# BoyBaykiller/IDKEngine

Hardware: AMD Instinct MI355X
Metric: Mray/s (primary+1 bounce) at 1920x1080, 1M-tri scene (higher is better)
Workload: dtype f32

## Files before the change

idkengine_amd/csrc/host_context.hpp:

```cpp
#pragma once


struct DevBuf {
    void* p = nullptr; size_t bytes = 0;
    hipError_t ensure(size_t n) { if (n <= bytes && p) return hipSuccess; if (p) (void)hipFree(p); p = nullptr; bytes = 0; if (n == 0) return hipSuccess; hipError_t e = hipMalloc(&p, n); if (e == hipSuccess) bytes = n; return e; }
    void release() { if (p) (void)hipFree(p); p = nullptr; bytes = 0; }
    template <class T> T* as() const { return (T*)p; }
};

struct PinnedStage {
    char* host = nullptr; hipEvent_t ev[2] = {nullptr, nullptr}; int half = 0;
    template <class Fill> hipError_t stage(DevBuf& dst, size_t capacity, size_t bytes, hipStream_t st, Fill&& fill)
    {
        hipError_t e;
        if (!host) {
            if ((e = hipHostMalloc((void**)&host, 2 * capacity, hipHostMallocDefault)) != hipSuccess) return e;
            for (int i = 0; i < 2; i++) if ((e = hipEventCreateWithFlags(&ev[i], hipEventDisableTiming)) != hipSuccess) return e;
            half = 0;
        } else if ((e = hipEventSynchronize(ev[half])) != hipSuccess) return e;
        char* h = host + (size_t)half * capacity;
        fill(h);
        if ((e = dst.ensure(capacity)) != hipSuccess) return e;
        if ((e = hipMemcpyAsync(dst.p, h, bytes, hipMemcpyHostToDevice, st)) != hipSuccess) return e;
        if ((e = hipEventRecord(ev[half], st)) != hipSuccess) return e;
// ... 37 lines not shown
    void release() { mem.release(); bytes = 0; }
    template <class T> T* as() const { return (T*)mem.p; }
};

struct DisplaySlot {
    GuardedBuf image; int format = -1;
    void release() { image.release(); format = -1; }
};

struct BloomSlot {
    GuardedBuf down, up, out;
    int levels = 0, w0 = 0, h0 = 0; bool valid = false;
    bool direct = false;
    void release() { down.release(); up.release(); out.release(); valid = false; }
};

struct DenoiseSlot {
    GuardedBuf out, ping[2];
    bool valid = false;
    int iterations = 0; uint8_t route[8] = {0};
    void release() { out.release(); ping[0].release(); ping[1].release(); valid = false; iterations = 0; }
};

struct NoiseSlot {
    GuardedBuf tiles, summary;
    int tilesX = 0, tilesY = 0; bool valid = false;
    void release() { tiles.release(); summary.release(); valid = false; }
};

static bool slot_holds(const DisplaySlot& s) { return s.format >= 0; }
template <class S> static bool slot_holds(const S& s) { return s.valid; }

struct FrameProducts {
    std::vector<DisplaySlot> display; std::vector<BloomSlot> bloom; std::vector<DenoiseSlot> denoise; std::vector<NoiseSlot> noise;
    DevBuf moments;
    template <class S> static void drop(std::vector<S>& v) { for (S& s : v) s.release(); v.clear(); }
    void release_noise() { drop(noise); moments.release(); }
    void release_presentation_sized() { drop(display); drop(bloom); }
    void release_all() { release_presentation_sized(); drop(denoise); release_noise(); }
    template <class S> static S& slot(std::vector<S>& v, int ringSize, int slot) { if (v.size() != (size_t)ringSize) { drop(v); v.resize(ringSize); } return v[slot]; }
};

struct DevOptions {
    int forceGeneric = 0;
    int noTileCull = 0;
    int noLeanPrimary = 0;
    int leafMin = 0;
    int grabUnitLog2 = 10, grabFixed = 0;
    int ldsPad = 0;
    int traceWaves = 0;
    int gridHint = 2;
    int deferLast = 1;
    int lastOcclusion = 1;
    int graphProbe = 0;
    int gridMidWaves = 20;
    int gridRaysX4 = 6;
    int traceVariant = 0;
    int bvhTiming = 0, bvhSmall = 32;
    int advMin = 0;
    int poolMin = 12;
    int leafPool = -1;
    int splitScatter = 6;
    int queryScheduler = 1;
    int groupThreads = -1;
    int fused = 1;
    int fusedShadeMin = 16;
    int splitPeek = 64;
    int splitDonor = 1;
    int split = 1;
    int wide = 0;
    int wideCap = 0;
    int wideCount = 0;
    int genPixelMajor = 8;
    int bouncePixelMajor = 1;
    int genGroupMax = 16;
    int instSieve = 8;
    int instSieveOverlap = 50;
    int instTlas = 8;
    int instTlasOverlap = 10;
    int instBraid = 0;
    int instUnify = 4096;
    int instGeneral = 0;
    int uniRefill = 32;
    int instUnifyRadius = 15;
    int pairNodes = 1;
    int packet = 1;
    int packetMinLive = 60;
    int packetWaves = 0;
    int bvhStackOptHost = 0;
};

enum { VB_NODES = 0, VB_TRIVERTS, VB_VERTICES, VB_TLAS, VB_XFORMS, VB_COUNT };
struct PendingSample { uint32_t accum; int slot; float cam[36]; uint8_t vs[VB_COUNT]; };

struct dev_ctx {
    int device = 0;
    hipStream_t stream = nullptr; bool ownStream = true;
    std::string lastError;
    idkpt_error_fn errFn = nullptr; void* errUser = nullptr;
    int numCUs = 256;
    idkpt_settings st;
    idkpt_settings stCaller;
    int W = 0, H = 0, rowMod = 1, rowRem = 0, rows = 0, rowBandLog2 = 0;
    float invProj[16], invView[16], viewPos[3];
    int ringSize = 1, curSlot = 0; bool ringStarted = false; std::vector<uint32_t> accum = std::vector<uint32_t>(1, 0u);
    bool counters = false, timing = false, capturePrimary = false;
    DevOptions opt;
    uint32_t seqFirst = 0, seqStride = 1;
    bool haveScene = false, frameOk = false;
    DevBuf nodes, tris, triVerts, descs, instances, tlas, parents, leaves, positions, prevPositions, vertices, meshes, materials, xforms, lights, sky, texDescs, unskinned, joints, levelNodes, tlasScratch, queryIn, queryOut, queryRec, queryList, tileClass, gbases;
    std::vector<DevBuf> texData; std::vector<std::pair<int, int>> texDims; std::vector<uint32_t> texState;
    DevBuf texStage;
    DevBuf srgbLut;
    std::vector<GpuBlasDesc> hDescs;
    std::vector<std::vector<uint32_t>> levelOffsets;
    std::vector<uint32_t> levelBase;
    std::vector<char> refitCoversAll;
    int nodeCount = 0, triCount = 0, instanceCount = 0, tlasCount = 0, vertexCount = 0, meshCount = 0, materialCount = 0, xformCount = 0, lightCount = 0, skySize = 0, textureCount = 0, unskinnedCount = 0;
    int sceneStack = 1;
    int hInst0Blas = 0;
    DevBuf wnodes, wleaf, wids, wpair, wcounts, wtotals; std::vector<uint32_t> wNodeOff, wLeafOff; bool wideTopoValid = false, wideFillValid = false;
    DevBuf pairNodes; bool pairValid = false;
    DevBuf instRec; bool instRecValid = false;
    DevBuf itlas, imarks, ichunks; int itlasNeed = 1; uint32_t ichunkCount = 0; bool itlasValid = false, imarksValid = false;
    int uniMode = 0; uint32_t uniBaseB = 0, uniRestoreIdx = 0;
    DevBuf unodes, utlas, uTabs, uniBuf, uniEntRec; bool uniValid = false, uniEligible = false, uniTabsValid = false; int uniCap = 0, uniEntries = 0, uniDepth = 0; float* hUni = nullptr; float* dUni = nullptr;
    std::vector<GpuBlasInstance> hInstances; std::vector<char> hXforms; uint64_t uniLaunches = 0;
    DevBuf entRec, braidBuf; bool itlasBraided = false; int itlasDepth = 0, itlasEntries = 0;
    int pkState = 0, pkBatchesSinceProbe = 0; unsigned long long* hPkStats = nullptr; unsigned long long* dPkStats = nullptr; unsigned long long pkSeen[6] = {0, 0, 0, 0, 0, 0}; float pkCam[36] = {0}; int pkW = 0, pkRows = 0, pkBatch = 0; float pkLastLive = -1.0f;
    float* hInstOverlap = nullptr; float* dInstOverlap = nullptr; bool instOverlapKnown = false, itlasBuilt = false, isieveWorth = false;
    int verSlots = 1; size_t vbytes[VB_COUNT] = {0}, vstride[VB_COUNT] = {0}; int valloc[VB_COUNT] = {1, 1, 1, 1, 1}, vcur[VB_COUNT] = {0};
    uint64_t lastMask[VB_COUNT] = {0};
    uint8_t lastSlots[VB_COUNT] = {0}; bool lastMulti = false;
    DevBuf verTab; PinnedStage verStage;
    char* hStage = nullptr; hipEvent_t evStage[4] = {nullptr, nullptr, nullptr, nullptr}; int stageNext = 0;
    PinnedUpload skyStage;
    hipEvent_t evSky = nullptr;
    int (*groupFlushAll)(void* user) = nullptr;
    DevBuf pmList;
    DevBuf trRec, contFlag, blockSums, rayO, rayT, rayR, aovA, aovN, hit, hitCost, primHit, queue[2], keys[2], keysTmp, sortKeys, sortVals, contMask, waveCounts, counts, work, sortHist, counters64;
    DevBuf img[3];
    FrameProducts products;
    int presW = 0, presH = 0;
    int resultSource = 0;
    PinnedUpload denoiseStage;
    int noiseOn = 0;
    DevBuf camTab;
    int rowLimit = 0x7fffffff;
    idkpt_bounce_exchange_fn exchangeFn = nullptr; void* exchangeUser = nullptr;
    idkpt_band_exchange_fn bandExchangeFn = nullptr; void* bandExchangeUser = nullptr; DevBuf bandTab;
    idkpt_band_exchange_device_fn bandExchangeDevFn = nullptr; void* bandExchangeDevUser = nullptr;
    idkpt_stats stats;
    uint32_t* hCounts = nullptr; uint32_t* dCountsMirror = nullptr;
    bool sceneNested = false;
    bool sceneNoEmission = false;
    struct { bool valid = false, allHits = false; int j = 0, side = 0, B = 0; uint32_t total = 0, Npad = 0;
             bool occl = false, pm = false; size_t ldsBytes = 0; uint32_t grid = 0; } defer;
    uint64_t occlLaunches = 0;
    DevBuf radSave, deferCount;
    bool countersDirty = true;
    uint32_t* hOverflow = nullptr; uint32_t* dOverflow = nullptr;
    int tlasNeed = 1;
    hipEvent_t evFrame[2] = {nullptr, nullptr};
    std::vector<hipEvent_t> evPool; size_t evUsed = 0;
    double traceMsAcc = 0.0; uint64_t traceLaunchesAcc = 0;
    int lastQueueSide = 0; int lastQueueCountSlot = 0; bool lastFast = false, lastNeedsRegen = false, lastTileClass = false ; int lastBatch = 1; Frame lastFrame;
    int maxBatch = 1; uint32_t Npad = 0; std::vector<PendingSample> pending; DevBuf bases, qwork; uint32_t* hBases = nullptr; uint32_t* dBasesMirror = nullptr;
    PinnedStage camStage;
    bool grouped = false, inGroupFlush = false; int groupIndex = 0;
    hipEvent_t* evBounce = nullptr;
    int (*groupExchange)(void* user, dev_ctx* member, int bounce, int samples, const uint32_t** outBases) = nullptr; void* groupUser = nullptr;
    struct BuilderScratch* bscratch = nullptr;
    struct PeerPolicy* peer = nullptr;
};

static hipEvent_t next_event(dev_ctx* ctx)
{
    if (ctx->evUsed == ctx->evPool.size()) { hipEvent_t e = nullptr; if (hipEventCreate(&e) != hipSuccess) return nullptr; ctx->evPool.push_back(e); }
    return ctx->evPool[ctx->evUsed++];
}
static void resolve_trace_events(dev_ctx* ctx)
{
    for (size_t i = 0; i + 1 < ctx->evUsed; i += 2) { float ms = 0.0f; if (hipEventElapsedTime(&ms, ctx->evPool[i], ctx->evPool[i + 1]) == hipSuccess) { ctx->traceMsAcc += ms; ctx->traceLaunchesAcc++; } }
    ctx->evUsed = 0;
}
#define TRACE_T0() do { if (ctx->timing) { hipEvent_t _e = next_event(ctx); if (_e) (void)hipEventRecord(_e, st); } } while (0)
#define TRACE_T1() do { if (ctx->timing) { hipEvent_t _e = next_event(ctx); if (_e) (void)hipEventRecord(_e, st); } } while (0)

static int fail(dev_ctx* c, int code, const std::string& msg) { if (c) { c->lastError = msg; if (c->errFn) c->errFn(c->errUser, (int32_t)code, c->lastError.c_str()); } return code; }
#define HIPC(expr) do { hipError_t _e = (expr); if (_e != hipSuccess) { (void)hipGetLastError(); return fail(ctx, IDKPT_ERR_HIP, std::string(#expr) + ": " + hipGetErrorString(_e)); } } while (0)
#define REQUIRE(cond, msg) do { if (!(cond)) return fail(ctx, IDKPT_ERR_INVALID_ARGUMENT, msg); } while (0)

static bool holds_whole_frame(const dev_ctx* ctx) { return ctx->rowMod == 1 && ctx->rowRem == 0 && ctx->rows == ctx->H; }
static bool owns_whole_frame(const dev_ctx* ctx) { return !ctx->grouped && holds_whole_frame(ctx); }
static int pres_w(const dev_ctx* ctx) { return ctx->presW ? ctx->presW : ctx->W; }
static int pres_h(const dev_ctx* ctx) { return ctx->presW ? ctx->presH : ctx->H; }
static bool present_scaled(const dev_ctx* ctx) { return ctx->presW && (ctx->presW != ctx->W || ctx->presH != ctx->H); }
static size_t display_texel_bytes(int format) { return format == IDKPT_DISPLAY_RGBA32F ? 16 : 4; }
static size_t display_texels(const dev_ctx* ctx) { return present_scaled(ctx) ? (size_t)ctx->presW * ctx->presH : (size_t)ctx->W * ctx->rows; }

template <class S> static int32_t slot_of(dev_ctx* ctx, std::vector<S>& v, const char* who, int32_t slot, const char* none, S** out)
{
    REQUIRE(slot >= -1 && slot < ctx->ringSize, std::string(who) + ": slot outside the frame ring (-1: the current slot)");
    if (slot < 0) slot = ctx->curSlot;
    if ((size_t)slot >= v.size() || !slot_holds(v[slot])) return fail(ctx, IDKPT_ERR_INVALID_OPERATION, std::string(who) + none);
    *out = &v[slot];
    return IDKPT_OK;
}

static int local_rows(int H, int mod, int rem, int bandLog2 = 0)
{
// ... 6 lines not shown
```

idkengine_amd/csrc/host_frame.hpp:

```cpp
#pragma once

static int alloc_frame_impl(dev_ctx* ctx)
{
    const size_t N = (size_t)ctx->W * ctx->rows;
    ctx->Npad = (uint32_t)((N + 63) / 64 * 64);
    const size_t cap = (size_t)ctx->maxBatch * ctx->Npad;
    ctx->pending.clear();
    ctx->lastFast = false; ctx->lastNeedsRegen = false; ctx->lastBatch = 1;
    HIPC(ctx->rayO.ensure(cap * 16)); HIPC(ctx->rayT.ensure(cap * 16)); HIPC(ctx->rayR.ensure(cap * 16));
    HIPC(ctx->aovA.ensure(cap * 16)); HIPC(ctx->aovN.ensure(cap * 16));
    HIPC(ctx->trRec.ensure(cap * 64)); HIPC(ctx->contFlag.ensure(cap));
    HIPC(ctx->blockSums.ensure(((cap + 63) / 64 + SCAN_WAVES_PER_BLOCK - 1) / SCAN_WAVES_PER_BLOCK * 4 + 16));
    HIPC(ctx->hit.ensure(cap * 32)); HIPC(ctx->hitCost.ensure(cap * 4));
    for (int i = 0; i < 2; i++) { HIPC(ctx->queue[i].ensure(cap * 4)); HIPC(ctx->keys[i].ensure(cap * 4)); }
    HIPC(ctx->keysTmp.ensure(cap * 4)); HIPC(ctx->sortKeys.ensure(cap * 4)); HIPC(ctx->sortVals.ensure(cap * 4));
    size_t nW = (cap + 63) / 64;
    HIPC(ctx->contMask.ensure(nW * 8)); HIPC(ctx->waveCounts.ensure(nW * 4));
    HIPC(ctx->counts.ensure(MAX_DEPTH_SLOTS * 4)); HIPC(ctx->work.ensure(WORK_WORDS * 4)); HIPC(ctx->counters64.ensure(128));
    HIPC(ctx->bases.ensure((size_t)MAX_DEPTH_SLOTS * (MAX_BATCH + 1) * 4));
    size_t nTiles = (cap + SORT_TILE - 1) / SORT_TILE;
    HIPC(ctx->sortHist.ensure((SORT_RADIX * nTiles + SORT_RADIX) * 4));
    for (int i = 0; i < 3; i++) { HIPC(ctx->img[i].ensure(N * 16 * ctx->ringSize)); HIPC(hipMemsetAsync(ctx->img[i].p, 0, N * 16 * ctx->ringSize, ctx->stream)); }
    HIPC(hipMemsetAsync(ctx->counters64.p, 0, 128, ctx->stream));
    ctx->defer.valid = false;
    ctx->countersDirty = true;
    HIPC(hipMemsetAsync(ctx->aovA.p, 0, cap * 16, ctx->stream)); HIPC(hipMemsetAsync(ctx->aovN.p, 0, cap * 16, ctx->stream));
    HIPC(hipMemsetAsync(ctx->contFlag.p, 0, cap, ctx->stream));
    ctx->accum.assign(ctx->ringSize, 0u); ctx->curSlot = 0; ctx->ringStarted = false;
    ctx->products.release_all();
    if (!owns_whole_frame(ctx)) ctx->noiseOn = 0;
    return IDKPT_OK;
}

static int alloc_frame(dev_ctx* ctx) { int rc = alloc_frame_impl(ctx); ctx->frameOk = rc == IDKPT_OK; return rc; }

static int alloc_frame_keep_images(dev_ctx* ctx)
{
    const size_t N = (size_t)ctx->W * ctx->rows;
    DevBuf saved[3];
    for (int i = 0; i < 3; i++) { saved[i] = ctx->img[i]; ctx->img[i] = DevBuf(); }
    FrameProducts products = std::move(ctx->products); ctx->products = FrameProducts();
    int rc = alloc_frame(ctx);
    ctx->products = std::move(products);
    hipError_t e = hipSuccess;
    for (int i = 0; i < 3 && rc == IDKPT_OK && e == hipSuccess; i++)
        if (saved[i].p) e = hipMemcpyAsync(ctx->img[i].p, saved[i].p, std::min(saved[i].bytes, N * 16 * ctx->ringSize), hipMemcpyDeviceToDevice, ctx->stream);
    if (rc == IDKPT_OK && e == hipSuccess) e = hipStreamSynchronize(ctx->stream);
    for (int i = 0; i < 3; i++) saved[i].release();
    if (rc == IDKPT_OK && e != hipSuccess) { (void)hipGetLastError(); ctx->frameOk = false; return fail(ctx, IDKPT_ERR_HIP, std::string("alloc_frame_keep_images: ") + hipGetErrorString(e)); }
    return rc;
}

static int flush_batch(dev_ctx* ctx);
static int check_overflow(dev_ctx* ctx)
{
    if (!ctx->hOverflow || *(volatile uint32_t*)ctx->hOverflow == 0u) return IDKPT_OK;
    *(volatile uint32_t*)ctx->hOverflow = 0u;
    return fail(ctx, IDKPT_ERR_INVALID_OPERATION, "traversal stack overflow: a BLAS/TLAS is deeper than the traversal stack (BlasStackSize / TLAS_STACK_SIZE); results since the last synchronisation are invalid");
}
#define SYNC_CHECKED() do { HIPC(hipStreamSynchronize(ctx->stream)); int _rc = check_overflow(ctx); if (_rc) return _rc; } while (0)
static int finish_deferred(dev_ctx* ctx);
static int flush_any(dev_ctx* ctx);
#define FLUSH() do { int _rc = flush_any(ctx); if (_rc) return _rc; _rc = finish_deferred(ctx); if (_rc) return _rc; } while (0)
#define FLUSH_KEEP() do { int _rc = flush_any(ctx); if (_rc) return _rc; } while (0)
static int32_t download_behind_queue(dev_ctx* ctx, void* dst, const void* src, size_t bytes)
{
    HIPC(hipSetDevice(ctx->device));
    FLUSH_KEEP();
    HIPC(hipMemcpyAsync(dst, src, bytes, hipMemcpyDeviceToHost, ctx->stream));
    SYNC_CHECKED();
    return IDKPT_OK;
}

static int flush_any(dev_ctx* ctx)
{
    if (ctx->pending.empty()) return IDKPT_OK;
    if (!(ctx->grouped && !ctx->inGroupFlush && ctx->groupFlushAll)) return flush_batch(ctx);
    const int rc = ctx->groupFlushAll(ctx->groupUser);
    const hipError_t e = hipSetDevice(ctx->device);
    if (rc) return rc;
// ... 97 lines not shown
```

idkengine_amd/csrc/host_options.hpp:

```cpp
#pragma once

static int32_t dev_SetOption(dev_ctx* ctx, const char* name, int32_t value)
{
    if (!ctx || !name) return IDKPT_ERR_INVALID_ARGUMENT;
    HIPC(hipSetDevice(ctx->device));
    FLUSH();
    DevOptions& o = ctx->opt;
    const std::string n(name);
    if (n == "force_generic") o.forceGeneric = value != 0;
    else if (n == "no_tile_cull") o.noTileCull = value != 0;
    else if (n == "no_lean_primary") o.noLeanPrimary = value != 0;
    else if (n == "leaf_min") o.leafMin = std::max(0, value);
    else if (n == "grab_unit_log2") o.grabUnitLog2 = value;
    else if (n == "grab_fixed") o.grabFixed = value;
    else if (n == "lds_pad") o.ldsPad = value;
    else if (n == "trace_waves") o.traceWaves = std::max(0, value);
    else if (n == "grid_hint") o.gridHint = std::max(0, value);
    else if (n == "grid_rays_x4") o.gridRaysX4 = std::max(0, value);
    else if (n == "grid_mid_waves") o.gridMidWaves = std::max(0, value);
    else if (n == "defer_last") o.deferLast = value != 0;
    else if (n == "last_occlusion") o.lastOcclusion = value != 0;
    else if (n == "split") { REQUIRE(value >= 0 && value <= 3, "idkptSetDeveloperOption: split is 0..3"); o.split = value; }
    else if (n == "split_donor") o.splitDonor = value != 0;
    else if (n == "split_peek") o.splitPeek = std::max(1, value);
    else if (n == "split_scatter") o.splitScatter = std::min(6, std::max(0, value));
    else if (n == "query_scheduler") o.queryScheduler = value != 0;
    else if (n == "group_threads") o.groupThreads = value;
    else if (n == "fused") { REQUIRE(value >= 0 && value <= 2, "idkptSetDeveloperOption: fused is 0..2"); o.fused = value; }
    else if (n == "fused_shade_min") o.fusedShadeMin = std::min(64, std::max(1, value));
    else if (n == "leaf_pool") { REQUIRE(value >= -1 && value <= 7, "idkptSetDeveloperOption: leaf_pool is -1 (automatic) or a mask 0..7 (1: primary launches, 2: the first bounce, 4: later bounces)"); o.leafPool = value; }
    else if (n == "pool_min") o.poolMin = std::max(0, value);
    else if (n == "adv_min") o.advMin = std::min(64, std::max(0, value));
#ifdef IDKPT_DEVELOPER
    else if (n == "graph_probe") o.graphProbe = std::max(0, value);
#endif
    else if (n == "inst_tlas_overlap") { REQUIRE(value >= 0 && value <= 100, "idkptSetDeveloperOption: inst_tlas_overlap is a percentage"); FLUSH(); o.instTlasOverlap = value; ctx->itlasValid = false; }
    else if (n == "bounce_pixel_major") { REQUIRE(value >= 0 && value <= 2, "idkptSetDeveloperOption: bounce_pixel_major is 0..2"); o.bouncePixelMajor = value; }
    else if (n == "gen_group_max") { REQUIRE(value >= 1 && value <= 16, "idkptSetDeveloperOption: gen_group_max is 1..16"); o.genGroupMax = value; }
    else if (n == "gen_pixel_major") { REQUIRE(value >= 0, "idkptSetDeveloperOption: gen_pixel_major is >= 0"); o.genPixelMajor = value; }
    else if (n == "inst_sieve_overlap") { REQUIRE(value >= 0 && value <= 100, "idkptSetDeveloperOption: inst_sieve_overlap is a percentage"); FLUSH(); o.instSieveOverlap = value; ctx->itlasValid = false; }
    else if (n == "inst_sieve") { REQUIRE(value >= 0, "idkptSetDeveloperOption: inst_sieve is >= 0"); FLUSH(); o.instSieve = value; ctx->itlasValid = false; }
    else if (n == "inst_braid") { REQUIRE(value >= 0, "idkptSetDeveloperOption: inst_braid is >= 0"); FLUSH(); o.instBraid = value; ctx->itlasValid = false; }
    else if (n == "pair_nodes") { REQUIRE(value == 0 || value == 1, "idkptSetDeveloperOption: pair_nodes is 0 or 1"); o.pairNodes = value; }
    else if (n == "inst_general") { REQUIRE(value >= 0, "idkptSetDeveloperOption: inst_general is >= 0"); FLUSH(); o.instGeneral = value; ctx->itlasValid = false; }
    else if (n == "uni_refill") { REQUIRE(value == 16 || value == 32, "idkptSetDeveloperOption: uni_refill is 16 or 32"); o.uniRefill = value; }
    else if (n == "inst_unify_radius") { REQUIRE(value >= 1 && value <= 512, "idkptSetDeveloperOption: inst_unify_radius is 1-512"); FLUSH(); o.instUnifyRadius = value; ctx->itlasValid = false; }
    else if (n == "inst_unify") { REQUIRE(value >= 0, "idkptSetDeveloperOption: inst_unify is >= 0"); FLUSH(); o.instUnify = value; ctx->itlasValid = false; }
    else if (n == "inst_tlas") { REQUIRE(value >= 0, "idkptSetDeveloperOption: inst_tlas is >= 0"); FLUSH(); o.instTlas = value; ctx->itlasValid = false; }
    else if (n == "packet") { REQUIRE(value >= 0 && value <= 2, "idkptSetDeveloperOption: packet is 0..2"); o.packet = value; ctx->pkState = 0; ctx->pkBatchesSinceProbe = 0; }
    else if (n == "packet_min_live") { REQUIRE(value >= 0 && value <= 100, "idkptSetDeveloperOption: packet_min_live is a percentage"); o.packetMinLive = value; ctx->pkState = 0; ctx->pkBatchesSinceProbe = 0; }
    else if (n == "packet_waves") { REQUIRE(value >= 0 && value <= 32, "idkptSetDeveloperOption: packet_waves is 0 (default) or 1..32"); o.packetWaves = value; }
    else if (n == "wide") { REQUIRE(value >= 0 && value <= 1, "idkptSetDeveloperOption: wide is 0 or 1"); FLUSH(); o.wide = value; }
    else if (n == "wide_cap") { REQUIRE(value >= 0 && value <= 96, "idkptSetDeveloperOption: wide_cap is 0 (default) or 4..96 rows"); o.wideCap = value; }
    else if (n == "wide_count") o.wideCount = value != 0;
    else if (n == "bvh_timing") o.bvhTiming = value != 0;
    else if (n == "bvh_small") o.bvhSmall = value;
    else if (n == "bvh_stackopt_host") o.bvhStackOptHost = value != 0;
    else if (n == "force_no_peer") { }
    else if (n == "trace_variant") {
#ifdef IDKPT_DEVELOPER
        o.traceVariant = value;
#else
        REQUIRE(value == 0 || value == 100, "idkptSetDeveloperOption: trace_variant needs the developer build of the library (libidkpt_dev.so)");
#endif
    }
    else return fail(ctx, IDKPT_ERR_INVALID_ARGUMENT, "idkptSetDeveloperOption: unknown option '" + n + "'");
    return IDKPT_OK;
}
```

idkengine_amd/csrc/host_readback.hpp:

```cpp
#pragma once

static int32_t dev_DownloadFrame(dev_ctx* ctx, int32_t slot, int32_t image, float* rgba, size_t bytes)
{
    if (!ctx || !rgba) return IDKPT_ERR_INVALID_ARGUMENT;
    REQUIRE(image >= 0 && image < 3, "idkptDownloadFrame: bad image id");
    REQUIRE(slot >= 0 && slot < ctx->ringSize, "idkptDownloadFrame: slot outside the frame ring");
    size_t need = (size_t)ctx->W * ctx->rows * 16;
    REQUIRE(bytes == need && need > 0, "idkptDownloadFrame: bytes must equal localRows*width*16");
    HIPC(hipSetDevice(ctx->device));
    FLUSH_KEEP();
    HIPC(hipMemcpyAsync(rgba, image_ptr(ctx, image, slot), need, hipMemcpyDeviceToHost, ctx->stream));
    SYNC_CHECKED();
    return IDKPT_OK;
}

static int32_t dev_GetFrameDevicePtr(dev_ctx* ctx, int32_t slot, int32_t image, void** outPtr, size_t* outBytes)
{
    if (!ctx || !outPtr) return IDKPT_ERR_INVALID_ARGUMENT;
    REQUIRE(image >= 0 && image < 3, "idkptGetFrameDevicePtr: bad image id");
    REQUIRE(slot >= 0 && slot < ctx->ringSize, "idkptGetFrameDevicePtr: slot outside the frame ring");
    HIPC(hipSetDevice(ctx->device));
    FLUSH_KEEP();
    { int rc = check_overflow(ctx); if (rc) return rc; }
    *outPtr = image_ptr(ctx, image, slot);
// ... 60 lines not shown
static int32_t dev_DownloadPrimaryHits(dev_ctx* ctx, float* t, uint32_t* triangleId, float* baryXY, size_t pixelCount)
{
    if (!ctx || !t || !triangleId || !baryXY) return IDKPT_ERR_INVALID_ARGUMENT;
    size_t N = (size_t)ctx->W * ctx->rows;
    REQUIRE(pixelCount == N, "idkptDownloadPrimaryHits: pixelCount mismatch");
    HIPC(hipSetDevice(ctx->device));
    FLUSH_KEEP();
    if (!ctx->capturePrimary || ctx->primHit.bytes < N * 16) return fail(ctx, IDKPT_ERR_INVALID_OPERATION, "idkptDownloadPrimaryHits: call idkptEnablePrimaryHitCapture(ctx,1) before idkptRender");
    std::vector<float4> h(N);
    HIPC(hipMemcpyAsync(h.data(), ctx->primHit.p, N * 16, hipMemcpyDeviceToHost, ctx->stream));
    HIPC(hipStreamSynchronize(ctx->stream));
    for (size_t i = 0; i < N; i++) { t[i] = h[i].x; baryXY[2 * i] = h[i].y; baryXY[2 * i + 1] = h[i].z; memcpy(&triangleId[i], &h[i].w, 4); }
    return IDKPT_OK;
}

static int32_t dev_DownloadTileClasses(dev_ctx* ctx, uint8_t* out, size_t bytes, int32_t* tilesX, int32_t* tilesY, int32_t* sets)
{
    if (!ctx || !tilesX || !tilesY || !sets) return IDKPT_ERR_INVALID_ARGUMENT;
    HIPC(hipSetDevice(ctx->device));
    FLUSH_KEEP();
    const bool have = ctx->lastFast && ctx->lastTileClass;
    const int32_t tx = have ? (ctx->lastFrame.W + 7) / 8 : 0, ty = have ? (ctx->lastFrame.rows + 7) / 8 : 0;
    const int32_t n = have ? (ctx->lastFrame.tilePerSample ? ctx->lastBatch : 1) : 0;
    *tilesX = tx; *tilesY = ty; *sets = n;
    if (!out) return IDKPT_OK;
    const size_t need = (size_t)n * tx * ty;
    REQUIRE(bytes == need, "idkptDownloadTileClasses: bytes must equal sets*tilesX*tilesY (call with out = NULL for the three numbers)");
    if (need) { REQUIRE(ctx->tileClass.bytes >= need, "idkptDownloadTileClasses: no classification is resident"); HIPC(hipMemcpyAsync(out, ctx->tileClass.p, need, hipMemcpyDeviceToHost, ctx->stream)); }
    SYNC_CHECKED();
    return IDKPT_OK;
}

static int32_t dev_GetStats(dev_ctx* ctx, idkpt_stats* out)
{
    if (!ctx || !out) return IDKPT_ERR_INVALID_ARGUMENT;
    HIPC(hipSetDevice(ctx->device));
    FLUSH_KEEP();
    SYNC_CHECKED();
    idkpt_stats s = ctx->stats;
    for (int j = 0; j < 16; j++) { const uint32_t* hb = ctx->hBases + (size_t)j * (MAX_BATCH + 1); s.LastAliveCounts[j] = (j >= 1 && j < ctx->st.RayDepth) ? hb[ctx->lastBatch] - hb[ctx->lastBatch - 1] : 0; }
    s.LastAliveCounts[0] = s.Frames ? (ctx->lastFast ? ctx->hCounts[MAX_DEPTH_SLOTS - 1] : (uint32_t)((size_t)ctx->W * ctx->rows)) : 0;
    s.LastFrameMs = 0.0f; s.LastTraceMs = 0.0f;
    if (ctx->timing && s.Frames > 0) { float ms = 0.0f; if (hipEventElapsedTime(&ms, ctx->evFrame[0], ctx->evFrame[1]) == hipSuccess) s.LastFrameMs = ms; }
    resolve_trace_events(ctx);
    s.TraceMsTotal = ctx->traceMsAcc; s.TraceLaunches = ctx->traceLaunchesAcc;
    s.LastTraceMs = s.TraceLaunches ? (float)(s.TraceMsTotal / (double)s.TraceLaunches) : 0.0f;
    uint64_t c[4] = {0, 0, 0, 0};
    HIPC(hipMemcpyAsync(c, ctx->counters64.p, 32, hipMemcpyDeviceToHost, ctx->stream)); HIPC(hipStreamSynchronize(ctx->stream));
    s.NodePairVisits = c[0]; s.TriangleTests = c[1];
    if (ctx->opt.traceVariant == 107 || ctx->opt.traceVariant == 113 || ctx->opt.traceVariant == 116 || ctx->opt.traceVariant == 213) { uint64_t d[16]; HIPC(hipMemcpyAsync(d, ctx->counters64.p, 128, hipMemcpyDeviceToHost, ctx->stream)); HIPC(hipStreamSynchronize(ctx->stream)); fprintf(stderr, "[idkpt prof] cycles refill %llu node %llu leaf %llu other %llu | refills %llu lanes %llu | nodeSteps %llu lanes %llu | leafPhases %llu lanes %llu | leafTests %llu leafTrips %llu\n", (unsigned long long)d[4], (unsigned long long)d[5], (unsigned long long)d[6], (unsigned long long)d[7], (unsigned long long)d[8], (unsigned long long)d[9], (unsigned long long)d[10], (unsigned long long)d[11], (unsigned long long)d[12], (unsigned long long)d[13], (unsigned long long)d[14], (unsigned long long)d[15]); }
    s.RaysTraced = s.PrimaryRays + c[2];
    if (ctx->wtotals.p) { uint64_t w[16]; HIPC(hipMemcpyAsync(w, ctx->wtotals.p, TOTALS_BYTES, hipMemcpyDeviceToHost, ctx->stream)); HIPC(hipStreamSynchronize(ctx->stream)); s.WideFlaggedRays = w[0]; s.WideNodeVisits = w[1]; s.WideLeafRecords = w[2]; s.WideTriangleTests = w[3]; s.InstTlasFlaggedRays = w[4];
        s.PacketFlaggedRays = w[8]; s.PacketPackets = w[9]; s.PacketNodeSteps = w[10]; s.PacketLiveLanes = w[11]; s.PacketRaysEntered = w[12]; s.PacketTriangleRounds = w[13]; }
    s.LastOcclusionLaunches = ctx->occlLaunches;
    s.InstUnifiedLaunches = ctx->uniLaunches; s.InstUnifiedEntries = ctx->uniValid ? (uint32_t)ctx->uniEntries : 0u; s.InstUnifiedTopDepth = ctx->uniValid ? (uint32_t)ctx->uniDepth : 0u;
    *out = s;
    return IDKPT_OK;
}

static int32_t dev_ResetStats(dev_ctx* ctx)
{
    if (!ctx) return IDKPT_ERR_INVALID_ARGUMENT;
    HIPC(hipSetDevice(ctx->device));
    FLUSH_KEEP();
    HIPC(hipStreamSynchronize(ctx->stream));
    memset(&ctx->stats, 0, sizeof(ctx->stats)); ctx->uniLaunches = 0; ctx->occlLaunches = 0;
    if (ctx->hPkStats) memset(ctx->hPkStats, 0, 64);
    for (int i = 0; i < 6; i++) ctx->pkSeen[i] = 0;
    ctx->evUsed = 0; ctx->traceMsAcc = 0.0; ctx->traceLaunchesAcc = 0;
    memset(ctx->hCounts, 0, (MAX_DEPTH_SLOTS - 1) * 4);
    HIPC(hipMemsetAsync(ctx->counters64.p, 0, 128, ctx->stream)); if (ctx->wtotals.p) HIPC(hipMemsetAsync(ctx->wtotals.p, 0, TOTALS_BYTES, ctx->stream)); HIPC(hipStreamSynchronize(ctx->stream));
    return IDKPT_OK;
}

static int32_t dev_EnableCounters(dev_ctx* ctx, int32_t enable) { if (!ctx) return IDKPT_ERR_INVALID_ARGUMENT; ctx->counters = enable != 0; return IDKPT_OK; }
static int32_t dev_EnableTiming(dev_ctx* ctx, int32_t enable) { if (!ctx) return IDKPT_ERR_INVALID_ARGUMENT; ctx->timing = enable != 0; return IDKPT_OK; }

static int32_t dev_GetImageDevicePtr(dev_ctx* ctx, int32_t image, void** outPtr, size_t* outBytes)
{
    if (!ctx || !outPtr) return IDKPT_ERR_INVALID_ARGUMENT;
    REQUIRE(image >= 0 && image < 3 && ctx->W > 0, "idkptGetImageDevicePtr: bad image / no size");
    HIPC(hipSetDevice(ctx->device));
    FLUSH_KEEP();
    { int rc = check_overflow(ctx); if (rc) return rc; }
    *outPtr = image_ptr(ctx, image, ctx->curSlot);
    if (outBytes) *outBytes = (size_t)ctx->W * ctx->rows * 16;
    return IDKPT_OK;
}

static int32_t dev_SetStream(dev_ctx* ctx, void* hipStream)
{
    if (!ctx) return IDKPT_ERR_INVALID_ARGUMENT;
    HIPC(hipSetDevice(ctx->device));
    FLUSH();
    HIPC(hipStreamSynchronize(ctx->stream));
    if (hipStream) { if (ctx->ownStream && ctx->stream) (void)hipStreamDestroy(ctx->stream); ctx->stream = (hipStream_t)hipStream; ctx->ownStream = false; }
    else if (!ctx->ownStream) { HIPC(hipStreamCreateWithFlags(&ctx->stream, hipStreamNonBlocking)); ctx->ownStream = true; }
    return IDKPT_OK;
}
static int32_t dev_GetStream(dev_ctx* ctx, void** out) { if (!ctx || !out) return IDKPT_ERR_INVALID_ARGUMENT; *out = (void*)ctx->stream; return IDKPT_OK; }

static int32_t dev_SetPresentationSize(dev_ctx* ctx, int32_t width, int32_t height)
{
    if (!ctx) return IDKPT_ERR_INVALID_ARGUMENT;
    REQUIRE((width == 0 && height == 0) || (width > 0 && height > 0 && width <= 65536 && height <= 65536), "idkptSetPresentationSize: width and height must both be 0 (the render size) or both be 1..65536");
    if (width == ctx->presW && height == ctx->presH) return IDKPT_OK;
    HIPC(hipSetDevice(ctx->device));
    ctx->products.release_presentation_sized();
    ctx->presW = width; ctx->presH = height;
    return IDKPT_OK;
}
static int32_t dev_GetPresentationSize(dev_ctx* ctx, int32_t* width, int32_t* height)
{
    if (!ctx) return IDKPT_ERR_INVALID_ARGUMENT;
    if (width) *width = pres_w(ctx);
    if (height) *height = pres_h(ctx);
    return IDKPT_OK;
}
static bool source_denoised(const dev_ctx* ctx, int image) { return ctx->resultSource == IDKPT_RESULT_DENOISED && image == IDKPT_IMAGE_RESULT; }
// ... 63 lines not shown
```

idkengine_amd/csrc/host_schedule.hpp:

```cpp
#pragma once

static DScene make_dscene(dev_ctx* ctx, const uint8_t* slots, bool multi)
{
    DScene s;
    auto at = [&](int b) -> char* { return multi ? (char*)vb_buf(ctx, b).p : vb_ptr(ctx, b, slots ? slots[b] : ctx->vcur[b]); };
    s.nodes = (const float4*)at(VB_NODES); s.tris = ctx->tris.as<uint4>(); s.triVerts = (const float4*)at(VB_TRIVERTS);
    s.descs = ctx->descs.as<GpuBlasDesc>(); s.instances = ctx->instances.as<GpuBlasInstance>(); s.instanceCount = ctx->instanceCount;
    s.tlas = (const float4*)at(VB_TLAS); s.tlasCount = ctx->tlasCount; s.vertices = (const uint4*)at(VB_VERTICES);
    s.instRec = nullptr;
    s.pairNodes = nullptr;
    s.meshes = ctx->meshes.as<GpuMesh>(); s.materials = ctx->materials.as<GpuMaterial>(); s.xforms = (const float4*)at(VB_XFORMS);
    s.lights = ctx->lights.as<GpuLight>(); s.lightCount = ctx->lightCount; s.sky = ctx->sky.as<float4>(); s.skySize = ctx->skySize;
    s.textures = ctx->texDescs.as<TexDesc>(); s.textureCount = ctx->textureCount; s.srgbLut = ctx->srgbLut.as<float>();
    s.overflow = ctx->dOverflow;
    s.ver = multi ? ctx->verTab.as<uint32_t>() : nullptr;
    return s;
}
static DScene make_dscene(dev_ctx* ctx) { return make_dscene(ctx, nullptr, false); }
static DScene make_dscene_last(dev_ctx* ctx) { return make_dscene(ctx, ctx->lastSlots, ctx->lastMulti); }

static float4* image_ptr(dev_ctx* ctx, int i, int slot) { return ctx->img[i].as<float4>() + (size_t)slot * ((size_t)ctx->W * ctx->rows); }

#define GRID_MID_RAYS 14000000u
#define SPLIT_MAX_RAYS 1500000u
static bool want_split(const dev_ctx* ctx, uint32_t prev, bool known, int samples)
{
    if (ctx->opt.split == 0) return false;
    if (ctx->opt.split >= 2) return true;
    return known && sparse_view(ctx, samples) && prev > 0u && prev < SPLIT_MAX_RAYS;
}
#define FUSED_MAX_RAYS 600000u
static bool want_fused(const dev_ctx* ctx, uint32_t prev, bool known, int samples)
{
    if (ctx->opt.fused == 0) return false;
    if (ctx->opt.fused >= 2) return true;
    return known && prev > 0u && prev < FUSED_MAX_RAYS && few_traversed(ctx, prev, std::max(1, samples));
}
static bool want_occlusion(const dev_ctx* ctx, const TracePlan& plan, bool readsOnlyHitOrMiss, bool split)
{
    return readsOnlyHitOrMiss && ctx->opt.lastOcclusion != 0 && !plan.fused && (plan.walk == Walk::Plain || plan.walk == Walk::Fast) && !(split && plan.splitOk)
           && !plan.multiVer && !plan.counting && !ctx->counters && (ctx->opt.traceVariant == 0 || ctx->opt.traceVariant == 100);
}
static uint32_t small_launch_grid(uint32_t fullGrid, uint32_t prev, int hintMul, int raysX4, uint32_t midGrid)
{
    if (prev == 0u || hintMul <= 0) return fullGrid;
    const uint32_t cap = std::max<uint32_t>(256u, (uint32_t)(((uint64_t)hintMul * prev + 63) / 64));
    uint32_t g = cap;
    if (raysX4 > 0) g = std::max<uint32_t>((uint32_t)(((uint64_t)prev * 4u / (uint32_t)raysX4 + 63) / 64), std::min<uint32_t>(cap, 1024u));
    if (midGrid > 0u && prev < GRID_MID_RAYS) g = std::min(g, midGrid);
    return std::min(fullGrid, std::min(g, cap));
}

struct Batch {
    dev_ctx* ctx; hipStream_t st; int B, depth; uint32_t N, Npad, total, gridTotal, scanBlocks;
    bool multiVer, fast, debug, capturing;
    Frame f; DScene s; TracePlan plan;
    RayBufs rays; HitBufs hits; TraceBufs tr, trNone;
    uint32_t* counts; uint32_t* bases ; uint32_t* work; uint64_t* counters; uint32_t* hostCounts; uint32_t* hostBases;
    unsigned long long* contMask; uint32_t* waveLocal ; uint32_t* blockSums; uint32_t* keysTmp;
    uint32_t* activeList; uint32_t* activeCount;
    uint32_t* pmList; uint32_t* pmCount; bool pmBounce;
    const uint8_t* tileClass; uint32_t midGrid, traceGrid;
    int side;
};
static const int BS = MAX_BATCH + 1;

static void batch_views(dev_ctx* ctx, Batch& b, int B, uint32_t Npad)
{
    b.ctx = ctx; b.st = ctx->stream; b.B = B; b.depth = ctx->st.RayDepth; b.N = (uint32_t)((size_t)ctx->W * ctx->rows); b.Npad = Npad; b.total = (uint32_t)B * Npad;
    b.gridTotal = (b.total + 255) / 256; b.scanBlocks = ((b.total + 63) / 64 + SCAN_WAVES_PER_BLOCK - 1) / SCAN_WAVES_PER_BLOCK;
    b.rays = {ctx->rayO.as<float4>(), ctx->rayT.as<float4>(), ctx->rayR.as<float4>(), ctx->aovA.as<float4>(), ctx->aovN.as<float4>()}; b.hits = {ctx->hit.as<float4>(), ctx->hitCost.as<float>()};
    b.tr = {ctx->trRec.as<float4>(), nullptr, nullptr}; b.trNone = {nullptr, nullptr, nullptr};
    b.counts = ctx->counts.as<uint32_t>(); b.bases = ctx->bases.as<uint32_t>(); b.work = ctx->work.as<uint32_t>(); b.counters = ctx->counters64.as<uint64_t>(); b.hostCounts = ctx->dCountsMirror; b.hostBases = ctx->dBasesMirror;
    b.contMask = ctx->contMask.as<unsigned long long>(); b.waveLocal = ctx->waveCounts.as<uint32_t>(); b.blockSums = ctx->blockSums.as<uint32_t>(); b.keysTmp = ctx->keysTmp.as<uint32_t>();
    b.activeList = ctx->sortVals.as<uint32_t>(); b.activeCount = b.counts + (MAX_DEPTH_SLOTS - 1);
    b.pmList = nullptr; b.pmCount = b.counts + (MAX_DEPTH_SLOTS - 2); b.pmBounce = false; b.tileClass = nullptr; b.side = 1; b.capturing = false;
}

static int bounce_tail(Batch& b, int j, const uint32_t* q, const uint32_t* cnt, const uint32_t* gbase, unsigned long long* traced, bool record, const TraceBufs& tr)
{
    dev_ctx* ctx = b.ctx; hipStream_t st = b.st; const int side = b.side;
    with_flag(b.multiVer, [&](auto VER) { launch(k_shade<false, VER>, dim3(b.gridTotal), dim3(256), 0, st, b.s, b.f, b.rays, tr, b.hits, q, cnt, 0u, b.bases + j * BS, gbase, b.contMask, b.waveLocal, b.keysTmp); });
    launch(k_scan_local<false>, dim3(b.scanBlocks), dim3(SCAN_WAVES_PER_BLOCK), 0, st, cnt, 0u, nullptr, b.contMask, b.waveLocal, b.blockSums);
    launch(k_scan_blocks, dim3(1), dim3(1024), 0, st, cnt, 0u, b.blockSums, b.waveLocal, b.counts + j + 1, traced, b.contMask, b.bases + j * BS, b.Npad, b.B, b.bases + (j + 1) * BS, b.hostCounts + j + 1, b.hostBases + (size_t)(j + 1) * BS, nullptr, nullptr);
    if (record) HIPC(hipEventRecord(ctx->evBounce[j + 1], st));
    launch(k_compact<false>, dim3(b.gridTotal), dim3(256), 0, st, q, cnt, 0u, b.contMask, b.waveLocal, b.blockSums, b.keysTmp, ctx->queue[1 - side].as<uint32_t>(), ctx->keys[1 - side].as<uint32_t>());
    return IDKPT_OK;
}

static int finish_deferred(dev_ctx* ctx)
{
    if (!ctx->defer.valid) return IDKPT_OK;
    ctx->defer.valid = false;
    Batch b; batch_views(ctx, b, ctx->defer.B, ctx->defer.Npad);
    b.side = ctx->defer.side; b.f = ctx->lastFrame; b.s = make_dscene_last(ctx); b.multiVer = ctx->lastMulti;
    const uint32_t* q = ctx->queue[b.side].as<uint32_t>(); const uint32_t* cnt = ctx->deferCount.as<uint32_t>();
    if (ctx->defer.occl) {
        const int j = ctx->defer.j;
        if (ctx->countersDirty) HIPC(hipMemsetAsync(b.work, 0, WORK_WORDS * 4, b.st));
        TracePlan p{}; p.walk = Walk::Plain; p.ldsBytes = ctx->defer.ldsBytes; p.grid = ctx->defer.grid;
        Frame ft = b.f; if (ctx->defer.pm) ft.hitsByRid = 0;
        if (ctx->defer.pm) launch_trace2<true>(ctx, p, p.grid, b.st, b.s, ft, b.rays, b.tr, b.hits, ctx->pmList.as<uint32_t>(), cnt, b.work + j, b.counters, false, j);
        else launch_trace2<false>(ctx, p, p.grid, b.st, b.s, ft, b.rays, b.tr, b.hits, q, cnt, b.work + j, b.counters, false, j);
        ctx->defer.occl = false;
    }
    with_flag(ctx->defer.allHits, [&](auto ALL) { launch(k_restore_last<ALL>, dim3(b.gridTotal), dim3(256), 0, b.st, b.rays, b.hits, q, cnt, ctx->radSave.as<float4>(), b.f.hitsByRid); });
    { int rc = bounce_tail(b, ctx->defer.j, q, cnt, nullptr, nullptr, false, b.tr); if (rc) return rc; }
    HIPC(hipGetLastError());
    ctx->lastQueueSide = 1 - b.side; ctx->countersDirty = true;
    return IDKPT_OK;
}

static int stage_versions_cameras(Batch& b)
{
    dev_ctx* ctx = b.ctx; const int B = b.B;
    bool multiVer = false; for (int k = 1; k < B && !multiVer; k++) multiVer = memcmp(ctx->pending[k].vs, ctx->pending[0].vs, VB_COUNT) != 0;
    for (int v = 0; v < VB_COUNT; v++) { uint64_t m = 0; for (int k = 0; k < B; k++) m |= 1ull << ctx->pending[k].vs[v]; ctx->lastMask[v] = m; ctx->lastSlots[v] = ctx->pending[0].vs[v]; }
    ctx->lastMulti = b.multiVer = multiVer;
    auto fillVersions = [&](char* half) {
        for (int k = 0; k < B; k++) {
            const uint8_t* vs = ctx->pending[k].vs; uint32_t* row = (uint32_t*)half + (size_t)k * SCENE_VER_WORDS;
            for (int v = 0; v < VB_COUNT; v++) row[v] = (uint32_t)(((size_t)vs[v] * ctx->vstride[v]) / 16);
            for (int v = VB_COUNT; v < SCENE_VER_WORDS; v++) row[v] = 0u;
        } };
    if (multiVer) HIPC(ctx->verStage.stage(ctx->verTab, (size_t)MAX_BATCH * SCENE_VER_WORDS * 4, (size_t)B * SCENE_VER_WORDS * 4, b.st, fillVersions));
    b.s = make_dscene_last(ctx);
    memset(&b.f, 0, sizeof(b.f));
    if (ctx->ringSize > 1) {
        auto fillCameras = [&](char* half) { for (int k = 0; k < B; k++) memcpy(half + (size_t)k * 36 * 4, ctx->pending[k].cam, 36 * 4); };
        HIPC(ctx->camStage.stage(ctx->camTab, (size_t)MAX_BATCH * 36 * 4, (size_t)B * 36 * 4, b.st, fillCameras));
        b.f.cams = ctx->camTab.as<float>();
    }
    return IDKPT_OK;
}

#ifdef IDKPT_DEVELOPER
static void graph_probe_begin(Batch& b) { if (b.ctx->opt.graphProbe > 0 && !b.ctx->timing) b.capturing = hipStreamBeginCapture(b.st, hipStreamCaptureModeThreadLocal) == hipSuccess; }
static void graph_probe_end(Batch& b)
{
    if (!b.capturing) return;
    dev_ctx* ctx = b.ctx; hipStream_t st = b.st;
    hipGraph_t g = nullptr; hipGraphExec_t ex = nullptr; const int K = ctx->opt.graphProbe; ctx->opt.graphProbe = 0;
    if (hipStreamEndCapture(st, &g) == hipSuccess && g && hipGraphInstantiate(&ex, g, nullptr, nullptr, 0) == hipSuccess) {
        hipEvent_t e0 = nullptr, e1 = nullptr; (void)hipEventCreate(&e0); (void)hipEventCreate(&e1);
        (void)hipGraphLaunch(ex, st); (void)hipStreamSynchronize(st);
        (void)hipEventRecord(e0, st);
        for (int k = 0; k < K; k++) (void)hipGraphLaunch(ex, st);
        (void)hipEventRecord(e1, st); (void)hipStreamSynchronize(st);
        float ms = 0.0f; (void)hipEventElapsedTime(&ms, e0, e1);
        size_t nodes = 0; (void)hipGraphGetNodes(g, nullptr, &nodes);
        fprintf(stderr, "[idkpt graph] batch of %d sample(s) captured: %zu graph nodes; %d replays: %.1f us per batch\n", b.B, nodes, K, ms * 1000.0f / (float)K);
        (void)hipEventDestroy(e0); (void)hipEventDestroy(e1); (void)hipGraphExecDestroy(ex);
    } else fprintf(stderr, "[idkpt graph] capture or instantiation failed: %s\n", hipGetErrorString(hipGetLastError()));
    if (g) (void)hipGraphDestroy(g);
}
#else
static void graph_probe_begin(Batch&) {}
static void graph_probe_end(Batch&) {}
#endif

static int frame_setup(Batch& b)
{
    dev_ctx* ctx = b.ctx; hipStream_t st = b.st; Frame& f = b.f; const int B = b.B;
    memcpy(f.invProj, ctx->pending[0].cam, 64); memcpy(f.invView, ctx->pending[0].cam + 16, 64); memcpy(f.viewPos, ctx->pending[0].cam + 32, 12);
    f.W = ctx->W; f.H = ctx->H; f.rowMod = ctx->rowMod; f.rowRem = ctx->rowRem; f.rows = ctx->rows; f.rowBandLog2 = ctx->rowBandLog2;
    f.g = ctx->st.Gpu; f.useTlas = ctx->st.UseTlas; f.stackCap = std::max(1, ctx->st.BlasStackSize > 0 ? ctx->st.BlasStackSize : ctx->sceneStack);
    f.outputAovs = ctx->st.OutputAOVs; f.batch = B; f.Npad = b.Npad;
    HIPC(ctx->trRec.ensure((size_t)ctx->maxBatch * b.Npad * 64)); b.tr.rec = ctx->trRec.as<float4>();
    for (int k = 0; k < MAX_BATCH; k++) { f.accum[k] = k < B ? ctx->pending[k].accum : 0u; f.slotOf[k] = (uint32_t)(k < B ? ctx->pending[k].slot : 0); }
    f.seqFirst = ctx->seqFirst; f.seqStride = ctx->seqStride; f.accumulated = f.seqFirst + f.accum[0] * f.seqStride;
    f.tilePerSample = (f.cams != nullptr || b.multiVer) ? 1 : 0;
    graph_probe_begin(b);
    if (ctx->timing) HIPC(hipEventRecord(ctx->evFrame[0], st));
    ctx->defer.valid = false;
    if (ctx->countersDirty) { HIPC(hipMemsetAsync(b.work, 0, WORK_WORDS * 4, st)); HIPC(hipMemsetAsync(b.counts, 0, MAX_DEPTH_SLOTS * 4, st)); }
    ctx->countersDirty = true;
    f.tlasCap = std::min(TLAS_STACK_SIZE, std::max(1, ctx->tlasNeed));
    f.grabUnitLog2 = std::min(24, std::max(6, ctx->opt.grabUnitLog2)); f.grabFixed = std::max(0, ctx->opt.grabFixed);
    f.leafMin = ctx->opt.leafMin > 0 ? ctx->opt.leafMin : (B >= 4 ? 16 : 12);
    b.fast = fast_path(ctx);
    f.genPixelMajor = (b.fast && ctx->opt.genPixelMajor > 0 && B >= ctx->opt.genPixelMajor && !f.tilePerSample) ? 1 : 0;
    { int rc = trace_plan(ctx, f, b.s, b.multiVer, false, false, b.plan); if (rc) { ctx->pending.clear(); return rc; } }
    b.traceGrid = std::min<uint32_t>(b.plan.grid, std::max<uint32_t>(1u, (uint32_t)(((size_t)B * b.N + 63) / 64)));
    b.midGrid = (ctx->opt.gridMidWaves > 0 && ctx->opt.traceWaves == 0) ? (uint32_t)(ctx->numCUs * std::min(b.plan.wavesPerCU, ctx->opt.gridMidWaves)) : 0u;
    f.gridRaysX4 = (uint32_t)std::max(0, ctx->opt.gridRaysX4); f.gridMid = b.midGrid; f.gridMidRays = GRID_MID_RAYS; f.splitMode = (ctx->opt.split == 3 ? 2 : 1) | (ctx->opt.splitDonor ? 4 : 0); f.poolMin = ctx->opt.poolMin; f.advMin = ctx->opt.advMin > 0 ? ctx->opt.advMin : (B >= 4 ? 8 : 1); f.splitPeek = ctx->opt.splitPeek;
    b.debug = f.g.DoDebugBVHTraversal != 0; f.shadeMin = ctx->opt.fusedShadeMin; f.scatterLog2 = ctx->opt.splitScatter;
    if (!b.fast && (B != 1 || b.multiVer)) { ctx->pending.clear(); return fail(ctx, IDKPT_ERR_UNKNOWN, "internal: generic path is never batched"); }
    return IDKPT_OK;
}

static int first_hit_compact(Batch& b)
{
    dev_ctx* ctx = b.ctx; hipStream_t st = b.st;
    launch(k_scan_blocks, dim3(1), dim3(1024), 0, st, nullptr, b.total, b.blockSums, b.waveLocal, b.counts + 1, (unsigned long long*)(1 < b.depth ? b.counters + 2 : nullptr), b.contMask, nullptr, b.Npad, b.B, b.bases + 1 * BS, b.hostCounts + 1, b.hostBases + 1 * BS, b.counts + MAX_DEPTH_SLOTS - 1, b.hostCounts + MAX_DEPTH_SLOTS - 1);
    if (ctx->evBounce) HIPC(hipEventRecord(ctx->evBounce[1], st));
    launch(k_compact<true>, dim3(b.gridTotal), dim3(256), 0, st, nullptr, nullptr, b.total, b.contMask, b.waveLocal, b.blockSums, b.keysTmp, ctx->queue[1].as<uint32_t>(), ctx->keys[1].as<uint32_t>());
    return IDKPT_OK;
}

static int first_hit_fast(Batch& b)
{
    dev_ctx* ctx = b.ctx; hipStream_t st = b.st; Frame& f = b.f; const DScene& s = b.s; const int B = b.B; const uint32_t N = b.N;
    const uint32_t tilesX = ((uint32_t)f.W + 7) / 8, tilesY = ((uint32_t)f.rows + 7) / 8; const uint32_t genWaves = tilesX * tilesY;
    const int cull = f.g.DoTraceLights ? 0 : 1;
    const int lean = (cull && !f.useTlas && s.instanceCount == 1 && ctx->opt.noLeanPrimary == 0) ? 1 : 0;
    uint8_t* contFlag = ctx->contFlag.as<uint8_t>();
    if (ctx->capturePrimary) launch(k_fill_miss, dim3((N + 255) / 256), dim3(256), 0, st, b.hits, (size_t)(B - 1) * b.Npad, N);
    if (cull && !ctx->opt.noTileCull) {
        const uint32_t classSets = f.tilePerSample ? (uint32_t)B : 1u;
        HIPC(ctx->tileClass.ensure((size_t)genWaves * classSets));
        with_flag(b.multiVer, [&](auto VER) { launch(k_classify_tiles<VER>, dim3((genWaves + 255) / 256, classSets), dim3(256), 0, st, s, f, ctx->tileClass.as<uint8_t>(), tilesX, tilesY); });
        b.tileClass = ctx->tileClass.as<uint8_t>();
    }
    const int genMax = std::min(16, std::max(1, ctx->opt.genGroupMax)), genGroups = (B + genMax - 1) / genMax, genPer = (B + genGroups - 1) / genGroups;
    const dim3 genGrid = f.genPixelMajor ? dim3(genGroups, genWaves) : dim3(B, (genWaves + 15) / 16), genBlock = f.genPixelMajor ? dim3(64 * genPer) : dim3(1024);
    with_flag(b.multiVer, [&](auto VER) { launch(k_gen_primary<VER>, genGrid, genBlock, 0, st, s, f, b.rays, b.tr, cull, b.activeList, b.activeCount, b.keysTmp, contFlag, b.tileClass, lean); });
    TRACE_T0();
    const bool known = ctx->lastFast && ctx->lastBatch == B;
    uint32_t grid0 = b.traceGrid;
    if (ctx->opt.gridRaysX4 > 0 && known) grid0 = small_launch_grid(b.traceGrid, ctx->hCounts[MAX_DEPTH_SLOTS - 1], 2, ctx->opt.gridRaysX4, b.midGrid);
    if (b.plan.fused) launch(k_trace_fused<32>, dim3(grid0), dim3(WAVE), b.plan.ldsBytes, st, s, f, b.rays, b.tr, b.hits, b.activeList, b.activeCount, b.work + 0, contFlag, b.keysTmp, lean);
    else launch_trace2<true>(ctx, b.plan, grid0, st, s, f, b.rays, b.tr, b.hits, b.activeList, b.activeCount, b.work + 0, b.counters, want_split(ctx, ctx->hCounts[MAX_DEPTH_SLOTS - 1], known, B), 0);
    TRACE_T1();
    if (ctx->capturePrimary) { HIPC(ctx->primHit.ensure((size_t)N * 16)); launch(k_capture_primary, dim3((N + 255) / 256), dim3(256), 0, st, b.hits, (size_t)(B - 1) * b.Npad, N, ctx->primHit.as<float4>()); }
    if (!b.plan.fused) {
        const bool sparseView = ctx->lastFast && ctx->lastBatch >= 1 && few_traversed(ctx, ctx->hCounts[MAX_DEPTH_SLOTS - 1], ctx->lastBatch);
        b.pmBounce = f.genPixelMajor && (ctx->opt.bouncePixelMajor >= 2 || (ctx->opt.bouncePixelMajor == 1 && sparseView)) && b.depth >= 2 && !b.multiVer;
        if (b.pmBounce) { HIPC(ctx->pmList.ensure((size_t)b.total * 4)); b.pmList = ctx->pmList.as<uint32_t>(); }
// ... 32 lines not shown
        HIPC(hipMemcpyAsync(ctx->gbases.p, outBases.data(), (size_t)B * 4, hipMemcpyHostToDevice, st)); HIPC(hipStreamSynchronize(st));
        gbase = ctx->gbases.as<uint32_t>();
    }
    if (!bandExchange) return IDKPT_OK;
    const int bandRows = 1 << ctx->rowBandLog2, LB = (ctx->rows + bandRows - 1) / bandRows;
    HIPC(ctx->bandTab.ensure((size_t)4 * MAX_BATCH * ((size_t)LB + 1) * 4));
    uint32_t* dStarts = ctx->bandTab.as<uint32_t>(); uint32_t* dTab = dStarts + (size_t)MAX_BATCH * (LB + 1);
    launch(k_band_starts, dim3((uint32_t)(((size_t)B * (LB + 1) + 255) / 256)), dim3(256), 0, st, q, b.bases + j * BS, B, LB, (uint32_t)ctx->W * (uint32_t)bandRows, b.Npad, dStarts);
    if (ctx->bandExchangeDevFn) {
        uint32_t* dCounts = dTab + (size_t)MAX_BATCH * (LB + 1); uint32_t* dBases = dCounts + (size_t)MAX_BATCH * (LB + 1);
        const uint32_t nb = (uint32_t)(((size_t)B * LB + 255) / 256);
        launch(k_band_counts, dim3(nb), dim3(256), 0, st, dStarts, B, LB, dCounts);
        HIPC(hipGetLastError());
        ctx->bandExchangeDevFn(ctx->bandExchangeDevUser, j, B, LB, dCounts, dBases, (void*)st);
        launch(k_band_tab, dim3(nb), dim3(256), 0, st, dStarts, dBases, B, LB, dTab);
    } else {
        std::vector<uint32_t> starts((size_t)B * (LB + 1)), local((size_t)B * LB), outBases((size_t)B * LB, 0u), tab((size_t)B * LB);
        HIPC(hipMemcpyAsync(starts.data(), dStarts, starts.size() * 4, hipMemcpyDeviceToHost, st)); HIPC(hipStreamSynchronize(st));
        for (int k2 = 0; k2 < B; k2++) for (int b2 = 0; b2 < LB; b2++) local[(size_t)k2 * LB + b2] = starts[(size_t)k2 * (LB + 1) + b2 + 1] - starts[(size_t)k2 * (LB + 1) + b2];
        ctx->bandExchangeFn(ctx->bandExchangeUser, j, B, LB, local.data(), outBases.data());
        for (int k2 = 0; k2 < B; k2++) for (int b2 = 0; b2 < LB; b2++) tab[(size_t)k2 * LB + b2] = outBases[(size_t)k2 * LB + b2] - starts[(size_t)k2 * (LB + 1) + b2];
        HIPC(hipMemcpyAsync(dTab, tab.data(), tab.size() * 4, hipMemcpyHostToDevice, st)); HIPC(hipStreamSynchronize(st));
    }
    gbase = dTab; f.gbStride = LB; f.gbBands = 1;
    return IDKPT_OK;
}

static int sort_queue(Batch& b, uint32_t* q, uint32_t* k, const uint32_t* cnt)
{
    dev_ctx* ctx = b.ctx; hipStream_t st = b.st;
    const uint32_t nTiles = (b.total + SORT_TILE - 1) / SORT_TILE;
    int sampleBits = 0; while ((1 << sampleBits) < b.B) sampleBits++;
    const int passes = (IDKPT_SORT_KEY_BITS + sampleBits + 6) / 7;
    uint32_t* hist = ctx->sortHist.as<uint32_t>(); uint32_t* digitTotals = hist + (size_t)SORT_RADIX * nTiles;
    uint32_t* ka = k; uint32_t* va = q; uint32_t* kb = ctx->sortKeys.as<uint32_t>(); uint32_t* vb = ctx->sortVals.as<uint32_t>();
    for (int pass = 0; pass < passes; pass++) {
        launch(k_sort_hist, dim3(nTiles), dim3(SORT_BLOCK), 0, st, ka, cnt, (uint32_t)(7 * pass), hist, nTiles);
        launch(k_sort_scan, dim3(SORT_RADIX), dim3(1024), 0, st, cnt, hist, nTiles, digitTotals);
        launch(k_sort_scatter, dim3(nTiles), dim3(SORT_BLOCK), 0, st, ka, va, cnt, (uint32_t)(7 * pass), hist, nTiles, digitTotals, kb, vb);
        std::swap(ka, kb); std::swap(va, vb);
    }
    if (va != q) HIPC(hipMemcpyAsync(q, va, (size_t)b.total * 4, hipMemcpyDeviceToDevice, st));
    return IDKPT_OK;
}

static bool trace_bounce(Batch& b, int j, const uint32_t* q, const uint32_t* cnt, bool readsOnlyHitOrMiss)
{
    dev_ctx* ctx = b.ctx; hipStream_t st = b.st; const int B = b.B;
    TRACE_T0();
    const bool known = ctx->lastFast && ctx->lastBatch == B && ctx->hBases != nullptr; const uint32_t prev = ctx->hBases ? ctx->hBases[(size_t)j * BS + B] : 0u;
    uint32_t gridj = b.traceGrid;
    const bool split = want_split(ctx, prev, known, B), occl = b.fast && want_occlusion(ctx, b.plan, readsOnlyHitOrMiss, split);
    if (occl) ctx->occlLaunches++;
    if (ctx->opt.gridHint > 0 && ctx->lastBatch == B && ctx->hBases) gridj = small_launch_grid(b.traceGrid, ctx->hBases[(size_t)j * BS + B], ctx->opt.gridHint, ctx->opt.gridRaysX4, b.midGrid);
    if (b.fast && b.pmBounce && j == 1) {
        Frame ft = b.f; ft.hitsByRid = 0;
        launch_trace2<true>(ctx, b.plan, gridj, st, b.s, ft, b.rays, b.tr, b.hits, b.pmList, b.pmCount, b.work + j, b.counters, split, j, occl);
    } else if (b.fast) launch_trace2<false>(ctx, b.plan, gridj, st, b.s, b.f, b.rays, b.tr, b.hits, q, cnt, b.work + j, b.counters, split, j, occl);
    else with_flag(ctx->counters, [&](auto COUNT) { launch(k_trace_queue<COUNT>, dim3(b.traceGrid), dim3(WAVE), b.plan.ldsBytes, st, b.s, b.f, b.rays, b.hits, q, cnt, b.work + j, b.counters); });
    TRACE_T1();
    return occl;
}

static int defer_last_bounce(Batch& b, int j, const uint32_t* q, const uint32_t* cnt, bool allHits, bool occl)
{
    dev_ctx* ctx = b.ctx;
    HIPC(ctx->radSave.ensure((size_t)ctx->maxBatch * ctx->Npad * 16)); HIPC(ctx->deferCount.ensure(64));
    auto shade_last = [&](auto ALL, auto VER) { launch(k_shade_last<ALL, VER>, dim3(b.gridTotal), dim3(256), 0, b.st, b.s, b.f, b.rays, b.hits, q, cnt, b.bases + j * BS, ctx->radSave.as<float4>(), ctx->deferCount.as<uint32_t>()); };
    if (allHits) with_flag(b.multiVer, [&](auto VER) { shade_last(std::true_type{}, VER); });
    else shade_last(std::false_type{}, std::false_type{});
    ctx->defer.allHits = allHits; ctx->defer.valid = true; ctx->defer.j = j; ctx->defer.side = b.side; ctx->defer.B = b.B; ctx->defer.total = b.total; ctx->defer.Npad = b.Npad;
    ctx->defer.occl = occl; ctx->defer.pm = b.pmBounce && j == 1; ctx->defer.ldsBytes = b.plan.ldsBytes; ctx->defer.grid = b.traceGrid;
    return IDKPT_OK;
}

static int final_draw(Batch& b)
{
    dev_ctx* ctx = b.ctx; hipStream_t st = b.st;
    ctx->lastQueueSide = b.side; ctx->lastQueueCountSlot = b.depth; ctx->lastFast = b.fast; ctx->lastNeedsRegen = b.fast; ctx->lastTileClass = b.tileClass != nullptr; ctx->lastBatch = b.B; ctx->lastFrame = b.f;
    if (ctx->noiseOn) {
        launch(k_final_draw_noise, dim3((b.N + 255) / 256), dim3(256), 0, st, b.s, b.f, b.rays, image_ptr(ctx, 0, 0), image_ptr(ctx, 1, 0), image_ptr(ctx, 2, 0), b.N, b.tileClass, b.work, (uint32_t)WORK_WORDS, b.counts, (uint32_t)MAX_DEPTH_SLOTS,
               noise_moments_ptr(ctx, 0), noise_mom_stride(ctx));
    } else
    launch(k_final_draw, dim3((b.N + 255) / 256), dim3(256), 0, st, b.s, b.f, b.rays, image_ptr(ctx, 0, 0), image_ptr(ctx, 1, 0), image_ptr(ctx, 2, 0), b.N, b.tileClass, b.work, (uint32_t)WORK_WORDS, b.counts, (uint32_t)MAX_DEPTH_SLOTS);
    HIPC(hipGetLastError()); ctx->countersDirty = false;
    graph_probe_end(b);
    if (ctx->timing) HIPC(hipEventRecord(ctx->evFrame[1], st));
    ctx->stats.Frames += (uint64_t)b.B; ctx->stats.PrimaryRays += (uint64_t)b.N * (uint64_t)b.B;
    ctx->pending.clear();
    return IDKPT_OK;
}

static int flush_batch(dev_ctx* ctx)
{
    if (ctx->pending.empty()) return IDKPT_OK;
    if (ctx->grouped && !ctx->inGroupFlush) return fail(ctx, IDKPT_ERR_UNKNOWN, "internal: a member of a multi-device context was flushed on its own");
    if (ctx->noiseOn) { int rc = noise_moments_ensure(ctx); if (rc) return rc; }
    Batch b; batch_views(ctx, b, (int)ctx->pending.size(), ctx->Npad); int rc;
    if ((rc = stage_versions_cameras(b))) return rc;
    if ((rc = frame_setup(b))) return rc;
    if ((rc = b.fast ? first_hit_fast(b) : first_hit_generic(b))) return rc;
    const bool deferLast = b.fast && b.depth >= 2 && ctx->opt.deferLast != 0 && !b.f.outputAovs && !b.debug;
    const bool deferAllHits = !(ctx->sceneNoEmission && !(b.f.g.DoTraceLights && b.s.lightCount > 0));
    for (int j = 1; j < b.depth; j++) {
        uint32_t* q = ctx->queue[b.side].as<uint32_t>(); uint32_t* k = ctx->keys[b.side].as<uint32_t>();
        const uint32_t* cnt = b.counts + j; const uint32_t* gbase;
        b.f.hitsByRid = (b.plan.fused || (b.pmBounce && j == 1)) ? 1 : 0;
        if ((rc = exchange_bases(b, j, q, gbase))) return rc;
        if (ctx->st.DoRaySorting && j > 1) if ((rc = sort_queue(b, q, k, cnt))) return rc;
        const bool deferThis = deferLast && j == b.depth - 1 && gbase == nullptr;
        bool tookOccl = false;
        if (!b.plan.fused) tookOccl = trace_bounce(b, j, q, cnt, deferThis && !deferAllHits);
        if (deferThis) { if ((rc = defer_last_bounce(b, j, q, cnt, deferAllHits, tookOccl))) return rc; break; }
        if ((rc = bounce_tail(b, j, q, cnt, gbase, (unsigned long long*)(j + 1 < b.depth ? b.counters + 2 : nullptr), ctx->evBounce != nullptr, b.fast ? b.tr : b.trNone))) return rc;
        b.side = 1 - b.side;
    }
    return final_draw(b);
}


static int32_t dev_Render(dev_ctx* ctx)
{
    if (!ctx) return IDKPT_ERR_INVALID_ARGUMENT;
    if (!ctx->haveScene) return fail(ctx, IDKPT_ERR_INVALID_OPERATION, "idkptRender: no scene uploaded");
    if (ctx->W <= 0 || !ctx->frameOk) return fail(ctx, IDKPT_ERR_INVALID_OPERATION, "idkptRender: no frame buffers (idkptSetSize not called, or its allocation failed)");
    if (ctx->st.UseTlas && ctx->tlasCount == 0) return fail(ctx, IDKPT_ERR_INVALID_OPERATION, "idkptRender: UseTlas set but no TLAS nodes uploaded");
    HIPC(hipSetDevice(ctx->device));
    if (ctx->timing && ctx->evUsed > 4096) { HIPC(hipStreamSynchronize(ctx->stream)); resolve_trace_events(ctx); }
    const int limit = fast_path(ctx) ? ctx->maxBatch : 1;
    for (int i = 0; i < ctx->st.SamplesPerPixel; i++) {
        PendingSample ps; ps.accum = ctx->accum[ctx->curSlot]++; ps.slot = ctx->curSlot;
        memcpy(ps.cam, ctx->invProj, 64); memcpy(ps.cam + 16, ctx->invView, 64); memcpy(ps.cam + 32, ctx->viewPos, 12); ps.cam[35] = 0.0f;
        for (int b = 0; b < VB_COUNT; b++) ps.vs[b] = (uint8_t)ctx->vcur[b];
        ctx->pending.push_back(ps);
        if (!ctx->grouped && (int)ctx->pending.size() >= limit) { int rc = flush_batch(ctx); if (rc) return rc; }
    }
    return IDKPT_OK;
}

static int32_t dev_Synchronize(dev_ctx* ctx) { if (!ctx) return IDKPT_ERR_INVALID_ARGUMENT; HIPC(hipSetDevice(ctx->device)); FLUSH_KEEP(); SYNC_CHECKED(); return IDKPT_OK; }

static int32_t dev_Flush(dev_ctx* ctx) { if (!ctx) return IDKPT_ERR_INVALID_ARGUMENT; HIPC(hipSetDevice(ctx->device)); FLUSH_KEEP(); return IDKPT_OK; }

static int32_t dev_SetMaxBatch(dev_ctx* ctx, int32_t maxBatch)
{
    if (!ctx) return IDKPT_ERR_INVALID_ARGUMENT;
    REQUIRE(maxBatch >= 1 && maxBatch <= MAX_BATCH, "idkptSetMaxBatch: 1..256");
    HIPC(hipSetDevice(ctx->device));
    FLUSH();
    HIPC(hipStreamSynchronize(ctx->stream));
    if (maxBatch == ctx->maxBatch) return IDKPT_OK;
    const int previous = ctx->maxBatch;
    ctx->maxBatch = maxBatch;
    if (ctx->W > 0) {
        std::vector<uint32_t> acc = ctx->accum; int slot = ctx->curSlot; const bool started = ctx->ringStarted;
        int rc = alloc_frame_keep_images(ctx);
        if (rc) {
            const std::string why = ctx->lastError;
            ctx->maxBatch = previous;
            (void)alloc_frame(ctx);
            return fail(ctx, rc, "idkptSetMaxBatch: could not allocate the wavefront buffers for " + std::to_string(maxBatch) + " samples in flight (" + why + "); kept " + std::to_string(previous));
        }
        ctx->accum = acc; ctx->curSlot = slot; ctx->ringStarted = started;
    }
    return IDKPT_OK;
}
// ... 43 lines not shown
```

idkengine_amd/csrc/idkpt_api.hpp:

```cpp
#pragma once
#include <array>
#include <thread>
#include <mutex>
#include <condition_variable>
#include <functional>

struct GroupBarrier {
    std::mutex m; std::condition_variable cv; int n = 0, arrived = 0; unsigned gen = 0; bool aborted = false;
    void reset(int members) { std::lock_guard<std::mutex> l(m); n = members; arrived = 0; aborted = false; }
    bool wait()
    {
        std::unique_lock<std::mutex> l(m);
        if (aborted) return false;
        const unsigned g = gen;
        if (++arrived == n) { arrived = 0; gen++; cv.notify_all(); return true; }
        cv.wait(l, [&] { return gen != g || aborted; });
        return !aborted;
    }
    void abort() { std::lock_guard<std::mutex> l(m); aborted = true; cv.notify_all(); }
};
struct GroupWorkers {
    std::vector<std::thread> th;
    std::mutex m; std::condition_variable cvGo, cvDone;
    unsigned epoch = 0; int remaining = 0; bool quit = false;
// ... 891 lines not shown
    ONE(dev_DownloadAliveQueue(m, indices, capacityElems, outCount));
    GFLUSH();
    if (c->st.DoRaySorting && c->st.RayDepth > 2) return gfail(c, IDKPT_ERR_INVALID_OPERATION, "idkptDownloadAliveQueue: with DoRaySorting every device sorts its own queue; there is no single queue to return");
    std::vector<uint32_t> all;
    for (size_t d = 0; d < c->n(); d++) {
        uint32_t cnt = 0;
        int rc = dev_DownloadAliveQueue(c->dev[d], nullptr, 0, &cnt); if (rc) return mfail(c, c->dev[d], rc);
        std::vector<uint32_t> q(cnt);
        if (cnt) { rc = dev_DownloadAliveQueue(c->dev[d], q.data(), cnt, &cnt); if (rc) return mfail(c, c->dev[d], rc); }
        for (uint32_t v : q) all.push_back(global_pixel(c, (int)d, v));
    }
    if (!c->strips) std::sort(all.begin(), all.end());
    *outCount = (uint32_t)all.size();
    if (indices && !all.empty()) { GREQ(capacityElems >= all.size(), "idkptDownloadAliveQueue: capacity too small"); memcpy(indices, all.data(), all.size() * 4); }
    return IDKPT_OK;
}
int32_t idkptEnablePrimaryHitCapture(idkpt_ctx* c, int32_t enable) { if (!c) return IDKPT_ERR_INVALID_ARGUMENT; for (dev_ctx* m : c->dev) dev_EnablePrimaryHitCapture(m, enable); return IDKPT_OK; }
int32_t idkptDownloadTileClasses(idkpt_ctx* c, uint8_t* out, size_t bytes, int32_t* tilesX, int32_t* tilesY, int32_t* sets)
{
    if (!c || !tilesX || !tilesY || !sets) return IDKPT_ERR_INVALID_ARGUMENT;
    ONE(dev_DownloadTileClasses(m, out, bytes, tilesX, tilesY, sets));
    GFLUSH();
    dev_ctx* m = c->dev[0];
    const int rc = dev_DownloadTileClasses(m, out, bytes, tilesX, tilesY, sets);
    return rc ? mfail(c, m, rc) : IDKPT_OK;
}
int32_t idkptDownloadPrimaryHits(idkpt_ctx* c, float* t, uint32_t* triangleId, float* baryXY, size_t pixelCount)
{
    if (!c || !t || !triangleId || !baryXY) return IDKPT_ERR_INVALID_ARGUMENT;
    ONE(dev_DownloadPrimaryHits(m, t, triangleId, baryXY, pixelCount));
    GREQ(pixelCount == (size_t)c->W * c->H, "idkptDownloadPrimaryHits: pixelCount mismatch");
    GFLUSH();
    for (size_t d = 0; d < c->n(); d++) {
        dev_ctx* m = c->dev[d];
        const size_t N = (size_t)c->W * m->rows;
        std::vector<float> tt(N), bb(2 * N); std::vector<uint32_t> ii(N);
        int rc = dev_DownloadPrimaryHits(m, tt.data(), ii.data(), bb.data(), N); if (rc) return mfail(c, m, rc);
        for (size_t i = 0; i < N; i++) { const uint32_t g = global_pixel(c, (int)d, (uint32_t)i); t[g] = tt[i]; triangleId[g] = ii[i]; baryXY[2 * (size_t)g] = bb[2 * i]; baryXY[2 * (size_t)g + 1] = bb[2 * i + 1]; }
    }
    return IDKPT_OK;
}

int32_t idkptGetStats(idkpt_ctx* c, idkpt_stats* out)
{
    if (!c || !out) return IDKPT_ERR_INVALID_ARGUMENT;
    ONE(dev_GetStats(m, out));
    GFLUSH();
    idkpt_stats sum; memset(&sum, 0, sizeof(sum));
    for (size_t d = 0; d < c->n(); d++) {
        idkpt_stats s; int rc = dev_GetStats(c->dev[d], &s); if (rc) return mfail(c, c->dev[d], rc);
        sum.RaysTraced += s.RaysTraced; sum.PrimaryRays += s.PrimaryRays; sum.NodePairVisits += s.NodePairVisits; sum.TriangleTests += s.TriangleTests;
        sum.WideFlaggedRays += s.WideFlaggedRays; sum.WideNodeVisits += s.WideNodeVisits; sum.WideLeafRecords += s.WideLeafRecords; sum.WideTriangleTests += s.WideTriangleTests; sum.InstTlasFlaggedRays += s.InstTlasFlaggedRays;
        sum.PacketFlaggedRays += s.PacketFlaggedRays; sum.PacketPackets += s.PacketPackets; sum.PacketNodeSteps += s.PacketNodeSteps; sum.PacketLiveLanes += s.PacketLiveLanes; sum.PacketRaysEntered += s.PacketRaysEntered; sum.PacketTriangleRounds += s.PacketTriangleRounds;
        sum.LastOcclusionLaunches += s.LastOcclusionLaunches;
        sum.InstUnifiedLaunches += s.InstUnifiedLaunches; if (d == 0) { sum.InstUnifiedEntries = s.InstUnifiedEntries; sum.InstUnifiedTopDepth = s.InstUnifiedTopDepth; }
        for (int j = 0; j < 16; j++) sum.LastAliveCounts[j] += s.LastAliveCounts[j];
        sum.LastFrameMs = std::max(sum.LastFrameMs, s.LastFrameMs); sum.LastTraceMs = std::max(sum.LastTraceMs, s.LastTraceMs);
        sum.TraceMsTotal = std::max(sum.TraceMsTotal, s.TraceMsTotal);
        if (d == 0) { sum.Frames = s.Frames; sum.TraceLaunches = s.TraceLaunches; }
    }
    *out = sum;
    return IDKPT_OK;
}
int32_t idkptGetStatsSized(idkpt_ctx* c, void* out, size_t bytes)
{
    if (!c || !out) return IDKPT_ERR_INVALID_ARGUMENT;
    idkpt_stats s; const int32_t rc = idkptGetStats(c, &s); if (rc) return rc;
    memcpy(out, &s, std::min(bytes, sizeof(s)));
    return IDKPT_OK;
}
int32_t idkptResetStats(idkpt_ctx* c) { REPLICATE(ResetStats); }
int32_t idkptEnableCounters(idkpt_ctx* c, int32_t enable) { if (!c) return IDKPT_ERR_INVALID_ARGUMENT; ONE(dev_EnableCounters(m, enable)); GFLUSH(); for (dev_ctx* m : c->dev) dev_EnableCounters(m, enable); return IDKPT_OK; }
int32_t idkptEnableTiming(idkpt_ctx* c, int32_t enable) { if (!c) return IDKPT_ERR_INVALID_ARGUMENT; for (dev_ctx* m : c->dev) dev_EnableTiming(m, enable); return IDKPT_OK; }

int32_t idkptSetStream(idkpt_ctx* c, void* hipStream)
{
    if (!c) return IDKPT_ERR_INVALID_ARGUMENT;
    ONE(dev_SetStream(m, hipStream));
    return gfail(c, IDKPT_ERR_INVALID_OPERATION, "idkptSetStream: a multi-device context owns one stream per device");
}
int32_t idkptGetStream(idkpt_ctx* c, void** out) { if (!c || !out) return IDKPT_ERR_INVALID_ARGUMENT; return dev_GetStream(c->dev[0], out); }

}
```

idkengine_amd/csrc/kernels_frame.hpp:

```cpp
#pragma once
#include "noise_texel.hpp"

DEV f3 TurboColormap(float x)
{
    x = gclamp(x, 0.0f, 1.0f);
    float v0 = 1.0f, v1 = x, v2 = x * x, v3 = x * x * x;
    float w0 = v2 * v2, w1 = v3 * v2;
    float r = (((v0 * 0.13572138f + v1 * 4.61539260f) + v2 * -42.66032258f) + v3 * 132.13108234f) + (w0 * -152.94239396f + w1 * 59.28637943f);
    float g = (((v0 * 0.09140261f + v1 * 2.19418839f) + v2 * 4.84296658f) + v3 * -14.18503333f) + (w0 * 4.27729857f + w1 * 2.82956604f);
    float b = (((v0 * 0.10667330f + v1 * 12.64194608f) + v2 * -60.58204836f) + v3 * 110.36276771f) + (w0 * -89.90310912f + w1 * 27.34824973f);
    return mk3(r, g, b);
}
template <bool NOISE>
__device__ __forceinline__ void final_draw_body(const DScene& s, const Frame& f, const RayBufs& rays, float4* imgResult, float4* imgAlbedo, float4* imgNormal, uint32_t N, const uint8_t* tileClass,
                                                uint32_t i, float4* imgMoments, size_t momStride)
{
    uint32_t slot = f.slotOf[0];
    float4 o = imgResult[(size_t)slot * N + i];
    f3 r = mk3(o.x, o.y, o.z), ra = splat3(0.0f), rn = splat3(0.0f);
    if (f.outputAovs) { float4 oa = imgAlbedo[(size_t)slot * N + i], on = imgNormal[(size_t)slot * N + i]; ra = mk3(oa.x, oa.y, oa.z); rn = mk3(on.x, on.y, on.z); }
    float m1 = 0.0f, m2 = 0.0f;
    if constexpr (NOISE) { const float4 om = imgMoments[(size_t)slot * momStride + i]; m1 = om.x; m2 = om.y; }
    const uint32_t px = i % (uint32_t)f.W, py = i / (uint32_t)f.W, tilesX = ((uint32_t)f.W + 7) / 8;
    const uint32_t tile = (py >> 3) * tilesX + (px >> 3), nTilesAll = tilesX * (((uint32_t)f.rows + 7) / 8);
    const uint32_t sharedCls = (tileClass && !f.tilePerSample) ? tileClass[tile] : 0u;
    for (int k = 0; k < f.batch; k++) {
        if (f.slotOf[k] != slot) {
            imgResult[(size_t)slot * N + i] = make_float4(r.x, r.y, r.z, 1.0f);
            if (f.outputAovs) { imgAlbedo[(size_t)slot * N + i] = make_float4(ra.x, ra.y, ra.z, 1.0f); imgNormal[(size_t)slot * N + i] = make_float4(rn.x, rn.y, rn.z, 1.0f); }
            if constexpr (NOISE) imgMoments[(size_t)slot * momStride + i] = make_float4(m1, m2, 0.0f, 1.0f);
            slot = f.slotOf[k];
            o = imgResult[(size_t)slot * N + i]; r = mk3(o.x, o.y, o.z);
            if (f.outputAovs) { float4 oa = imgAlbedo[(size_t)slot * N + i], on = imgNormal[(size_t)slot * N + i]; ra = mk3(oa.x, oa.y, oa.z); rn = mk3(on.x, on.y, on.z); }
            if constexpr (NOISE) { const float4 om = imgMoments[(size_t)slot * momStride + i]; m1 = om.x; m2 = om.y; }
        }
        const size_t rid = (size_t)k * f.Npad + i;
        float w = 1.0f / ((float)f.accum[k] + 1.0f);
        const uint32_t cls = !tileClass ? 0u : (f.tilePerSample ? tileClass[(size_t)k * nTilesAll + tile] : sharedCls);
        f3 nr = splat3(0.0f);
        if (cls == 0u) { float4 c = rays.rad_py[rid]; nr = mk3(c.x, c.y, c.z); }
        else if (cls <= 6u) { const float4 p = s.sky[cls - 1u]; nr = splat3(0.0f) + mk3(p.x, p.y, p.z) * splat3(1.0f); }
        else if (cls == 8u) {
            f3 origin; f2 pd; uint32_t seed;
            gen_primary(f, (uint32_t)k, i, sample_index(f, (uint32_t)k), origin, pd, seed);
            const f3 albedo = SampleSky(s, DecodeUnitVec(pd.x, pd.y));
            nr = splat3(0.0f) + albedo * splat3(1.0f);
        }
        if (f.g.DoDebugBVHTraversal) nr = TurboColormap(rays.o_ior[rid].w / 150.0f);
        r = gmix(r, nr, w);
        if constexpr (NOISE) noiset::fold(&m1, &m2, noiset::luminance(nr.x, nr.y, nr.z), w);
        if (f.outputAovs) { float4 a = rays.aovA[rid], n = rays.aovN[rid]; ra = gmix(ra, mk3(a.x, a.y, a.z), w); rn = gmix(rn, mk3(n.x, n.y, n.z), w); }
    }
    imgResult[(size_t)slot * N + i] = make_float4(r.x, r.y, r.z, 1.0f);
    if (f.outputAovs) { imgAlbedo[(size_t)slot * N + i] = make_float4(ra.x, ra.y, ra.z, 1.0f); imgNormal[(size_t)slot * N + i] = make_float4(rn.x, rn.y, rn.z, 1.0f); }
    if constexpr (NOISE) imgMoments[(size_t)slot * momStride + i] = make_float4(m1, m2, 0.0f, 1.0f);
}
__global__ __launch_bounds__(256) void k_final_draw(DScene s, Frame f, RayBufs rays, float4* imgResult, float4* imgAlbedo, float4* imgNormal, uint32_t N, const uint8_t* tileClass,
                                                    uint32_t* zeroWork, uint32_t nWork, uint32_t* zeroCounts, uint32_t nCounts)
{
    if (blockIdx.x == 0) { for (uint32_t k = threadIdx.x; k < nWork; k += blockDim.x) zeroWork[k] = 0u; for (uint32_t k = threadIdx.x; k < nCounts; k += blockDim.x) zeroCounts[k] = 0u; }
    uint32_t i = blockIdx.x * blockDim.x + threadIdx.x;
    if (i >= N) return;
    final_draw_body<false>(s, f, rays, imgResult, imgAlbedo, imgNormal, N, tileClass, i, nullptr, 0);
}
__global__ __launch_bounds__(256) void k_final_draw_noise(DScene s, Frame f, RayBufs rays, float4* imgResult, float4* imgAlbedo, float4* imgNormal, uint32_t N, const uint8_t* tileClass,
                                                          uint32_t* zeroWork, uint32_t nWork, uint32_t* zeroCounts, uint32_t nCounts, float4* imgMoments, size_t momStride)
{
    if (blockIdx.x == 0) { for (uint32_t k = threadIdx.x; k < nWork; k += blockDim.x) zeroWork[k] = 0u; for (uint32_t k = threadIdx.x; k < nCounts; k += blockDim.x) zeroCounts[k] = 0u; }
    uint32_t i = blockIdx.x * blockDim.x + threadIdx.x;
    if (i >= N) return;
    final_draw_body<true>(s, f, rays, imgResult, imgAlbedo, imgNormal, N, tileClass, i, imgMoments, momStride);
}

__global__ __launch_bounds__(256) void k_regen_culled(DScene s, Frame f, RayBufs rays, const uint8_t* contFlag, const uint8_t* tileClass, uint32_t smp, uint32_t N)
{
    const uint32_t pix = blockIdx.x * blockDim.x + threadIdx.x;
    if (pix >= N) return;
    const size_t rid = (size_t)smp * f.Npad + pix;
    uint8_t flag = contFlag[rid];
    if (tileClass) {
        const uint32_t px = pix % (uint32_t)f.W, py = pix / (uint32_t)f.W, tilesX = ((uint32_t)f.W + 7) / 8, nTilesAll = tilesX * (((uint32_t)f.rows + 7) / 8);
        if (tileClass[(f.tilePerSample ? (size_t)smp * nTilesAll : 0) + (py >> 3) * tilesX + (px >> 3)] != 0u) flag = 4;
    }
    if (flag != 2 && flag != 4) return;
    f3 origin; f2 pd; uint32_t seed;
    gen_primary(f, smp, pix, sample_index(f, smp), origin, pd, seed);
    rays.o_ior[rid] = make_float4(origin.x, origin.y, origin.z, 1.0f);
    rays.thr_px[rid] = make_float4(1.0f, 1.0f, 1.0f, pd.x);
    if (flag == 4) {
        const f3 albedo = SampleSky(s, DecodeUnitVec(pd.x, pd.y));
        const f3 radiance = splat3(0.0f) + albedo * splat3(1.0f);
        rays.rad_py[rid] = make_float4(radiance.x, radiance.y, radiance.z, pd.y);
    }
}

__global__ void k_fill_miss(HitBufs hits, size_t first, uint32_t n)
{
    uint32_t i = blockIdx.x * blockDim.x + threadIdx.x;
    if (i < n) store_hit(hits, first + i, PT_FLOAT_MAX, 0.0f, 0.0f, ~0u, 0u);
}

__global__ void k_gather_triverts(const uint4* tris, const float* positions, float4* triVerts, uint32_t first, uint32_t count)
{
    uint32_t i = blockIdx.x * blockDim.x + threadIdx.x;
    if (i >= count) return;
    uint4 t = tris[first + i];
    const float* a = positions + 3 * (size_t)t.x; const float* b = positions + 3 * (size_t)t.y; const float* c = positions + 3 * (size_t)t.z;
    float4* o = triVerts + 3 * (size_t)(first + i);
    o[0] = make_float4(a[0], a[1], a[2], 0.0f); o[1] = make_float4(b[0], b[1], b[2], 0.0f); o[2] = make_float4(c[0], c[1], c[2], 0.0f);
}

__global__ void k_capture_primary(HitBufs hits, size_t first, uint32_t n, float4* out)
{
    uint32_t i = blockIdx.x * blockDim.x + threadIdx.x;
    if (i < n) out[i] = hits.hit[2 * (first + i)];
}
```

idkengine_amd/csrc/kernels_shade.hpp:

```cpp
#pragma once

DEV void write_trace_ready(const DScene& s, const Frame& f, const TraceBufs& tr, uint32_t rid, const RayState& r)
{
    f3 rd = DecodeUnitVec(r.pdx, r.pdy);
    if (f.useTlas || s.instanceCount > 1) {
        tr.rec[4 * (size_t)rid] = make_float4(r.origin.x, r.origin.y, r.origin.z, 0.0f); tr.rec[4 * (size_t)rid + 1] = make_float4(rd.x, rd.y, rd.z, 0.0f);
        if (f.useTlas || f.instTlas) tr.rec[4 * (size_t)rid + 2] = make_float4(1.0f / rd.x, 1.0f / rd.y, 1.0f / rd.z, 0.0f);
        return;
    }
    GpuBlasInstance inst = s.instances[0];
    M34 inv = load_inv_model(s, inst.MeshTransformId);
    f3 lo = xform34(inv, r.origin, 1.0f), ld = xform34(inv, rd, 0.0f);
    const f3 iv = mk3(1.0f / ld.x, 1.0f / ld.y, 1.0f / ld.z);
    const float4* root = s.nodes + 2 * (size_t)s.descs[inst.BlasId].NodeOffset + 2;
    float t1;
    const float rootT = RayBoxIntersect(lo, iv, root[0], root[1], &t1) ? t1 : __builtin_inff();
    const float wantClosest = (__builtin_isfinite(r.throughput.x) && __builtin_isfinite(r.throughput.y) && __builtin_isfinite(r.throughput.z)) ? 0.0f : 1.0f;
    tr.rec[4 * (size_t)rid] = make_float4(lo.x, lo.y, lo.z, rootT); tr.rec[4 * (size_t)rid + 1] = make_float4(ld.x, ld.y, ld.z, wantClosest);
    tr.rec[4 * (size_t)rid + 2] = make_float4(iv.x, iv.y, iv.z, 0.0f);
}

template <bool VER >
__global__ __launch_bounds__(256) void k_shade_first(DScene s0, Frame f, RayBufs rays, TraceBufs tr, HitBufs hits, const uint32_t* activeList, const uint32_t* activeCount,
                                                     uint8_t* contFlag, uint32_t* seedsAndKeys, int lean ,
                                                     uint32_t* pmList , uint32_t* pmCount)
{
    __shared__ uint32_t waveCont[4]; __shared__ uint32_t blockBase;
    const uint32_t item = blockIdx.x * blockDim.x + threadIdx.x;
    const uint32_t nActive = *activeCount;
    if (blockIdx.x * blockDim.x >= nActive) return;
    const bool live = item < nActive;
    if (!pmList && !live) return;
    bool cont = false; uint32_t rid = 0;
    if (live) {
        rid = activeList[item];
        const uint32_t smp = rid / f.Npad, pix = rid - smp * f.Npad;
        const DScene s = VER ? scene_of_sample(s0, smp) : s0;
        const uint32_t acc = sample_index(f, smp);
        const HitRec hit = load_hit(hits, rid);
        RayState r; uint32_t rng, key = 0;
        if (lean) {
            f2 pd; gen_primary(f, smp, pix, acc, r.origin, pd, rng);
            r.prevIor = 1.0f; r.throughput = splat3(1.0f); r.pdx = pd.x; r.radiance = splat3(0.0f); r.pdy = pd.y;
        } else {
            float4 a = rays.o_ior[rid], b = rays.thr_px[rid], c = rays.rad_py[rid];
            r.origin = mk3(a.x, a.y, a.z); r.prevIor = a.w; r.throughput = mk3(b.x, b.y, b.z); r.pdx = b.w; r.radiance = mk3(c.x, c.y, c.z); r.pdy = c.w;
            rng = seedsAndKeys[rid];
        }
        AovState aov; aov.albedo = splat3(0.0f); aov.normal = splat3(0.0f); aov.newWeight = 1.0f;
        int lx = (int)(pix % (uint32_t)f.W), ly = (int)(pix / (uint32_t)f.W);
        uint32_t gidSeed = first_hit_gid_seed(f.W, f.H, lx, global_row(f, ly));
        f3 rd = DecodeUnitVec(r.pdx, r.pdy);
        cont = ShadeHit<true>(s, f, acc, hit, hit.T != PT_FLOAT_MAX, rd, r, aov, rng, gidSeed, key);
        rays.o_ior[rid] = make_float4(r.origin.x, r.origin.y, r.origin.z, r.prevIor);
        rays.thr_px[rid] = make_float4(r.throughput.x, r.throughput.y, r.throughput.z, r.pdx);
        rays.rad_py[rid] = make_float4(r.radiance.x, r.radiance.y, r.radiance.z, r.pdy);
        if (f.outputAovs) { rays.aovA[rid] = make_float4(aov.albedo.x, aov.albedo.y, aov.albedo.z, aov.newWeight); rays.aovN[rid] = make_float4(aov.normal.x, aov.normal.y, aov.normal.z, 0.0f); }
        seedsAndKeys[rid] = (key & ((1u << IDKPT_SORT_KEY_BITS) - 1u)) | (smp << IDKPT_SORT_KEY_BITS);
        if (cont) { contFlag[rid] = 1; write_trace_ready(s, f, tr, rid, r); }
    }
    if (pmList) {
        const unsigned long long m = __ballot(cont);
        const uint32_t wv = threadIdx.x >> 6, lane = threadIdx.x & 63;
        if (lane == 0) waveCont[wv] = (uint32_t)__popcll(m);
        __syncthreads();
        if (threadIdx.x == 0) { uint32_t tot = 0; for (int i = 0; i < 4; i++) { const uint32_t c = waveCont[i]; waveCont[i] = tot; tot += c; } blockBase = tot ? atomicAdd(pmCount, tot) : 0u; }
        __syncthreads();
        if (cont) pmList[blockBase + waveCont[wv] + (uint32_t)__popcll(m & ((1ull << lane) - 1ull))] = rid;
    }
}

template <bool FIRST, bool VER = false>
__global__ __launch_bounds__(256) void k_shade(DScene s0, Frame f, RayBufs rays, TraceBufs tr, HitBufs hits, const uint32_t* queue, const uint32_t* countPtr, uint32_t countImm,
                                               const uint32_t* qbase, const uint32_t* gbase , unsigned long long* contMask, uint32_t* waveCounts, uint32_t* keysTmp)
{
    const uint32_t N = FIRST ? countImm : *countPtr;
    const uint32_t slot = blockIdx.x * blockDim.x + threadIdx.x;
    if ((slot & ~63u) >= N) return;
    bool cont = false;
    uint32_t key = 0;
    bool inRange = slot < N;
    uint32_t smp = 0, pix = 0, idx = 0;
    if (inRange) {
        idx = FIRST ? slot : queue[slot];
        smp = idx / f.Npad; pix = idx - smp * f.Npad;
        if (FIRST && pix >= (uint32_t)f.W * (uint32_t)f.rows) inRange = false;
    }
    if (inRange) {
        const DScene s = VER ? scene_of_sample(s0, smp) : s0;
        const uint32_t acc = sample_index(f, smp);
        float4 a = rays.o_ior[idx], b = rays.thr_px[idx], c = rays.rad_py[idx];
        const HitRec hit = load_hit(hits, (!FIRST && f.hitsByRid) ? idx : slot);
        if (FIRST && f.g.DoDebugBVHTraversal) {
            rays.o_ior[idx] = make_float4(a.x, a.y, a.z, hits.cost[slot]);
        } else {
            RayState r; r.origin = mk3(a.x, a.y, a.z); r.prevIor = a.w; r.throughput = mk3(b.x, b.y, b.z); r.pdx = b.w; r.radiance = mk3(c.x, c.y, c.z); r.pdy = c.w;
            AovState aov; aov.albedo = splat3(0.0f); aov.normal = splat3(0.0f); aov.newWeight = 1.0f;
            if (!FIRST && f.outputAovs) { float4 aa = rays.aovA[idx], an = rays.aovN[idx]; aov.albedo = mk3(aa.x, aa.y, aa.z); aov.newWeight = aa.w; aov.normal = mk3(an.x, an.y, an.z); }
            uint32_t rng, gidSeed;
            if (FIRST) {
                f3 o2; f2 pd2; gen_primary(f, smp, pix, acc, o2, pd2, rng);
                int lx = (int)(pix % (uint32_t)f.W), ly = (int)(pix / (uint32_t)f.W);
                gidSeed = first_hit_gid_seed(f.W, f.H, lx, global_row(f, ly));
            } else {
                uint32_t gslot = (gbase ? gbase[f.gbBands ? smp * (uint32_t)f.gbStride + ((pix / (uint32_t)f.W) >> f.rowBandLog2) : smp] : 0u) + (slot - qbase[smp]);
                rng = gslot * 4096u + acc;
                gidSeed = gslot;
            }
            f3 rd = DecodeUnitVec(r.pdx, r.pdy);
            bool hitScene = hit.T != PT_FLOAT_MAX;
            cont = ShadeHit<FIRST>(s, f, acc, hit, hitScene, rd, r, aov, rng, gidSeed, key);
            rays.o_ior[idx] = make_float4(r.origin.x, r.origin.y, r.origin.z, r.prevIor);
            rays.thr_px[idx] = make_float4(r.throughput.x, r.throughput.y, r.throughput.z, r.pdx);
            rays.rad_py[idx] = make_float4(r.radiance.x, r.radiance.y, r.radiance.z, r.pdy);
            if (f.outputAovs) { rays.aovA[idx] = make_float4(aov.albedo.x, aov.albedo.y, aov.albedo.z, aov.newWeight); rays.aovN[idx] = make_float4(aov.normal.x, aov.normal.y, aov.normal.z, 0.0f); }
            if (cont && tr.rec) write_trace_ready(s, f, tr, idx, r);
        }
        keysTmp[slot] = (key & ((1u << IDKPT_SORT_KEY_BITS) - 1u)) | (smp << IDKPT_SORT_KEY_BITS);
    }
    unsigned long long m = __ballot(cont);
    if ((threadIdx.x & 63) == 0) contMask[slot >> 6] = m;
    (void)waveCounts;
}

template <bool ALL_HITS , bool VER = false>
__global__ __launch_bounds__(256) void k_shade_last(DScene s0, Frame f, RayBufs rays, HitBufs hits, const uint32_t* queue, const uint32_t* countPtr, const uint32_t* qbase,
                                                    float4* radSave, uint32_t* deferCount)
{
    const uint32_t N = *countPtr;
    const uint32_t slot = blockIdx.x * blockDim.x + threadIdx.x;
    if (slot == 0u) *deferCount = N;
    if (slot >= N) return;
    const uint32_t idx = queue[slot];
    const HitRec hit = load_hit(hits, f.hitsByRid ? idx : slot);
    const float4 b = rays.thr_px[idx];
    const bool miss = hit.T == PT_FLOAT_MAX;
    const bool odd = ALL_HITS || !(__builtin_isfinite(b.x) && __builtin_isfinite(b.y) && __builtin_isfinite(b.z));
    if (!miss && !odd) return;
    const float4 c = rays.rad_py[idx];
    radSave[slot] = c;
    if (miss) {
        const f3 albedo = SampleSky(s0, DecodeUnitVec(b.w, c.w));
        const f3 rad = mk3(c.x, c.y, c.z) + albedo * mk3(b.x, b.y, b.z);
        rays.rad_py[idx] = make_float4(rad.x, rad.y, rad.z, c.w);
    } else {
        const uint32_t smp = idx / f.Npad;
        const DScene s = VER ? scene_of_sample(s0, smp) : s0;
        const uint32_t acc = sample_index(f, smp);
        const float4 a = rays.o_ior[idx];
        RayState r; r.origin = mk3(a.x, a.y, a.z); r.prevIor = a.w; r.throughput = mk3(b.x, b.y, b.z); r.pdx = b.w; r.radiance = mk3(c.x, c.y, c.z); r.pdy = c.w;
        AovState aov; aov.albedo = splat3(0.0f); aov.normal = splat3(0.0f); aov.newWeight = 1.0f;
        const uint32_t gslot = slot - qbase[smp];
        uint32_t rng = gslot * 4096u + acc, key = 0;
        (void)ShadeHit<false, true>(s, f, acc, hit, true, DecodeUnitVec(b.w, c.w), r, aov, rng, gslot, key);
        rays.rad_py[idx] = make_float4(r.radiance.x, r.radiance.y, r.radiance.z, c.w);
    }
}
template <bool ALL_HITS>
__global__ __launch_bounds__(256) void k_restore_last(RayBufs rays, HitBufs hits, const uint32_t* queue, const uint32_t* countPtr, const float4* radSave, int hitsByRid)
{
    const uint32_t slot = blockIdx.x * blockDim.x + threadIdx.x;
    if (slot >= *countPtr) return;
    const uint32_t idx = queue[slot];
    const HitRec hit = load_hit(hits, hitsByRid ? idx : slot);
    const float4 b = rays.thr_px[idx];
    if (ALL_HITS || hit.T == PT_FLOAT_MAX || !(__builtin_isfinite(b.x) && __builtin_isfinite(b.y) && __builtin_isfinite(b.z))) rays.rad_py[idx] = radSave[slot];
}
```

idkengine_amd/csrc/kernels_trace.hpp:

```cpp
#pragma once

template <bool COUNT, bool COST>
__global__ __launch_bounds__(WAVE) void k_trace_primary(DScene s, Frame f, RayBufs rays, HitBufs hits, uint32_t N, uint32_t* workCounter, uint64_t* counters)
{
    extern __shared__ uint32_t lds[];
    const int lane = threadIdx.x;
    uint32_t* stk = lds + lane;
    uint32_t nPairs = 0, nTris = 0;
    while (true) {
        uint32_t base = wave_grab(workCounter, WAVE);
        if (base >= N) break;
        uint32_t pix = base + lane;
        if (pix < N) {
            f3 origin; f2 pd; uint32_t seed;
            gen_primary(f, 0u, pix, f.accumulated, origin, pd, seed);
            rays.o_ior[pix] = make_float4(origin.x, origin.y, origin.z, 1.0f);
            rays.thr_px[pix] = make_float4(1.0f, 1.0f, 1.0f, pd.x);
            rays.rad_py[pix] = make_float4(0.0f, 0.0f, 0.0f, pd.y);
            f3 rd = DecodeUnitVec(pd.x, pd.y);
            HitRec hit; float cost;
            TraceRay<COUNT, COST>(s, f, origin, rd, hit, cost, stk, WAVE, nPairs, nTris);
            store_hit(hits, pix, hit.T, hit.bx, hit.by, hit.tri, hit.xform);
            if (COST) hits.cost[pix] = cost;
        }
// ... 86 lines not shown
            bool boxOutside = false;
            for (int i = 0; i < 4; i++) {
                if (!planeOk[i]) continue;
                float dmin = PT_FLOAT_MAX;
                for (int c = 0; c < 8; c++) dmin = gmin(dmin, dot(pn[i], rel[c]));
                if (dmin > margin) boxOutside = true;
            }
            outside = boxOutside;
        }
        if (outside) {
            if (s.skySize <= 0) cls = 7;
            else if (s.skySize > 1) cls = 8;
            else {
                const float eta = 2.0f * (R / F) + 1e-4f;
                int face = -1; bool same = true;
                for (int i = 0; i < 4; i++) {
                    const float ax = gabs(u[i].x), ay = gabs(u[i].y), az = gabs(u[i].z);
                    int fc = -1;
                    if (ax >= gmax(ay, az) + eta) fc = u[i].x > 0.0f ? 0 : 1;
                    else if (ay >= gmax(ax, az) + eta) fc = u[i].y > 0.0f ? 2 : 3;
                    else if (az >= gmax(ax, ay) + eta) fc = u[i].z > 0.0f ? 4 : 5;
                    if (fc < 0 || (face >= 0 && fc != face)) same = false;
                    face = fc;
                }
                if (same && face >= 0) cls = (uint8_t)(1 + face);
            }
        }
    }
    tileClass[(size_t)smp * (tilesX * tilesY) + t] = cls;
}

template <bool VER>
__global__ __launch_bounds__(1024) void k_gen_primary(DScene s0, Frame f, RayBufs rays, TraceBufs tr, int cull, uint32_t* activeList, uint32_t* activeCount, uint32_t* seedOut, uint8_t* contFlag,
                                                     const uint8_t* tileClass ,
                                                     int lean )
{
    __shared__ uint32_t waveKeep[16]; __shared__ uint32_t blockBase; __shared__ unsigned long long keepMask[16];
    const bool pm = f.genPixelMajor != 0;
    if (pm && tileClass && blockIdx.y < ((uint32_t)f.W + 7) / 8 * (((uint32_t)f.rows + 7) / 8) && tileClass[blockIdx.y] != 0u) return;
    const uint32_t G = blockDim.x >> 6;
    const uint32_t smp = pm ? blockIdx.x * G + (threadIdx.x >> 6) : blockIdx.x;
    const DScene s = VER ? scene_of_sample(s0, min(smp, (uint32_t)f.batch - 1u)) : s0;
    const uint32_t wave = pm ? blockIdx.y : (blockIdx.y * blockDim.x + threadIdx.x) >> 6, lane = threadIdx.x & 63;
    const uint32_t tilesX = ((uint32_t)f.W + 7) / 8;
    const uint32_t tx = wave % tilesX, ty = wave / tilesX;
    const uint32_t x = tx * 8 + (lane & 7), y = ty * 8 + (lane >> 3);
    const bool valid = x < (uint32_t)f.W && y < (uint32_t)f.rows && smp < (uint32_t)f.batch;
    const uint32_t pix = y * (uint32_t)f.W + x;
    const uint32_t rid = smp * f.Npad + pix;
    bool keep = false;
    const uint32_t nTilesAll = tilesX * (((uint32_t)f.rows + 7) / 8);
    const uint32_t cls = (tileClass && wave < nTilesAll) ? tileClass[(f.tilePerSample ? (size_t)min(smp, (uint32_t)f.batch - 1u) * nTilesAll : 0) + wave] : 0u;
    if (valid && cls != 0u) {
        contFlag[rid] = 4;
    } else if (valid) {
        f3 origin; f2 pd; uint32_t seed;
        gen_primary(f, smp, pix, sample_index(f, smp), origin, pd, seed);
        f3 rd = DecodeUnitVec(pd.x, pd.y);
        f3 lo = origin, ld = rd, invDir = splat3(0.0f);
        float rootT = __builtin_inff();
        keep = !cull;
        if (f.useTlas || f.instTlas) {
            invDir = mk3(1.0f / rd.x, 1.0f / rd.y, 1.0f / rd.z);
            if (cull) {
                if (s.tlasCount == 0) keep = false;
                else {
                    const uint32_t packed = __float_as_uint(s.tlas[0].w), id = packed & 0x7fffffffu;
                    if ((packed >> 31) == 1u) keep = true;
                    else {
                        float t1, t2;
                        const bool tl = RayBoxIntersect(origin, invDir, s.tlas[2 * (size_t)id], s.tlas[2 * (size_t)id + 1], &t1) && t1 < PT_FLOAT_MAX;
                        const bool tr2 = RayBoxIntersect(origin, invDir, s.tlas[2 * (size_t)id + 2], s.tlas[2 * (size_t)id + 3], &t2) && t2 < PT_FLOAT_MAX;
                        keep = tl || tr2;
                    }
                }
            }
        } else
        for (int ii = 0; ii < s.instanceCount && (ii == 0 || cull); ii++) {
            GpuBlasInstance inst = s.instances[ii];
            M34 inv = load_inv_model(s, inst.MeshTransformId);
            f3 l0 = xform34(inv, origin, 1.0f), l1 = xform34(inv, rd, 0.0f);
            f3 iv = mk3(1.0f / l1.x, 1.0f / l1.y, 1.0f / l1.z);
            if (s.instanceCount == 1) { lo = l0; ld = l1; invDir = iv; }
            if (cull || s.instanceCount == 1) {
                const float4* root = s.nodes + 2 * (size_t)s.descs[inst.BlasId].NodeOffset + 2;
                float t1;
                const bool boxHit = RayBoxIntersect(l0, iv, root[0], root[1], &t1);
                if (s.instanceCount == 1 && boxHit) rootT = t1;
                if (cull && boxHit && t1 < PT_FLOAT_MAX) keep = true;
            }
        }
        f3 radiance = splat3(0.0f);
        if (keep) {
            tr.rec[4 * (size_t)rid] = make_float4(lo.x, lo.y, lo.z, rootT); tr.rec[4 * (size_t)rid + 1] = make_float4(ld.x, ld.y, ld.z, 0.0f); tr.rec[4 * (size_t)rid + 2] = make_float4(invDir.x, invDir.y, invDir.z, 0.0f);
            if (!lean) seedOut[rid] = seed;
        } else {
            f3 albedo = SampleSky(s, rd);
            radiance = radiance + albedo * splat3(1.0f);
            if (f.outputAovs) { f3 fn = CubemapFaceNormal(rd); rays.aovA[rid] = make_float4(albedo.x, albedo.y, albedo.z, 0.0f); rays.aovN[rid] = make_float4(fn.x, fn.y, fn.z, 0.0f); }
        }
        if (keep && !lean) { rays.o_ior[rid] = make_float4(origin.x, origin.y, origin.z, 1.0f); rays.thr_px[rid] = make_float4(1.0f, 1.0f, 1.0f, pd.x); }
        contFlag[rid] = keep ? 0 : 2;
        if (!(keep && lean)) rays.rad_py[rid] = make_float4(radiance.x, radiance.y, radiance.z, pd.y);
    }
    const unsigned long long m = __ballot(keep);
    const uint32_t wv = threadIdx.x >> 6;
    if (pm) {
        if (lane == 0) keepMask[wv] = m;
        __syncthreads();
        uint32_t cnt = 0, before = 0;
        for (uint32_t w = 0; w < G; w++) { const uint32_t b = (uint32_t)(keepMask[w] >> lane) & 1u; cnt += b; before += w < wv ? b : 0u; }
        uint32_t incl = cnt;
        for (int off = 1; off < 64; off <<= 1) { const uint32_t v = (uint32_t)__shfl_up((int)incl, off); incl += lane >= (uint32_t)off ? v : 0u; }
        const uint32_t tot = (uint32_t)__shfl((int)incl, 63);
        if (threadIdx.x == 0) blockBase = tot ? atomicAdd(activeCount, tot) : 0u;
        __syncthreads();
        if (keep) activeList[blockBase + (incl - cnt) + before] = rid;
        return;
    }
    if (lane == 0) waveKeep[wv] = (uint32_t)__popcll(m);
    __syncthreads();
    if (threadIdx.x == 0) { uint32_t tot = 0; for (int i = 0; i < 16; i++) { uint32_t c = waveKeep[i]; waveKeep[i] = tot; tot += c; } blockBase = tot ? atomicAdd(activeCount, tot) : 0u; }
    __syncthreads();
    if (keep) activeList[blockBase + waveKeep[wv] + (uint32_t)__popcll(m & ((1ull << lane) - 1ull))] = rid;
}

#define GRAB_SLICES 8u
#define GRAB_STRIDE 256u
template <bool PRIMARY, bool COUNT, int REFILL_MIN = 32, int OCC = 1, bool PROF = false, int LEAF_MIN = 24, int MODE = 0, int DBG = 0, bool VER = false, bool ANY = false, bool FAST = false, bool OCCL = false>
__global__ __launch_bounds__(WAVE, OCC) void k_trace2(DScene s, Frame f, RayBufs rays, TraceBufs tr, HitBufs hits, const uint32_t* list, const uint32_t* countPtr, uint32_t* workCounter, uint64_t* counters)
{
    static_assert(MODE >= 0 && MODE <= 2 && (DBG == 0 || DBG == 16), "k_trace2: MODE 0-2, DBG 0 or 16 (pooled leaf phase)");
    static_assert(!FAST || (MODE == 0 && !COUNT && !VER && !ANY && !PROF), "k_trace2: FAST is the plain one-BLAS closest-hit walk");
    static_assert(!OCCL || (MODE == 0 && !COUNT && !VER && !ANY && !PROF), "k_trace2: OCCL is the plain one-BLAS walk that stops at the first accepted triangle");
    constexpr bool MULTI = MODE != 0, TLAS = MODE == 2;
    constexpr bool POOL = DBG == 16;
    extern __shared__ uint32_t lds[];
    const uint32_t lane = threadIdx.x;
    typedef __attribute__((address_space(3))) uint32_t lds_u32;
    lds_u32* const stkBase = (lds_u32*)lds + lane + (FAST ? WAVE : 0);
    if (FAST) stkBase[0] = 0u;
    const int cap = f.stackCap;
    lds_u32* const stkFull = stkBase + cap * WAVE;
    uint32_t* tstk = lds + lane + (cap + 2) * WAVE;
    const uint32_t N = *countPtr;
    {
        uint32_t want = gridDim.x;
        if (f.gridRaysX4 > 0u) want = max((uint32_t)(((unsigned long long)N * 4ull / f.gridRaysX4 + 63ull) / 64ull), min(want, 1024u));
        if (f.gridMid > 0u && N < f.gridMidRays) want = min(want, f.gridMid);
        if (blockIdx.x >= max(want, 1u)) return;
    }
    const GpuBlasInstance inst = s.instances[0];
    const int nodeOffset = s.descs[inst.BlasId].NodeOffset;
    const uint32_t triOffset = (uint32_t)s.descs[inst.BlasId].TriangleOffset;
    const float4* nodes = s.nodes + 2 * (size_t)nodeOffset;
// ... 213 lines not shown
                    for (uint32_t k = 0; k < maxCnt; k++) { const uint32_t j = off + k - base; if (k < cnt && j < 64u) tbl[j] = lane | (k << 8); }
                    __builtin_amdgcn_wave_barrier();
                    const bool have = base + lane < total;
                    const uint32_t e = have ? tbl[lane] : lane;
                    const int src = (int)((e & 63u) << 2);
                    const uint32_t kk = e >> 8;
                    const f3 oro = mk3(__int_as_float(__builtin_amdgcn_ds_bpermute(src, __float_as_int(ro.x))), __int_as_float(__builtin_amdgcn_ds_bpermute(src, __float_as_int(ro.y))), __int_as_float(__builtin_amdgcn_ds_bpermute(src, __float_as_int(ro.z))));
                    const f3 ord = mk3(__int_as_float(__builtin_amdgcn_ds_bpermute(src, __float_as_int(rd.x))), __int_as_float(__builtin_amdgcn_ds_bpermute(src, __float_as_int(rd.y))), __int_as_float(__builtin_amdgcn_ds_bpermute(src, __float_as_int(rd.z))));
                    const float oT = __int_as_float(__builtin_amdgcn_ds_bpermute(src, __float_as_int(hitT)));
                    const uint32_t oFirst = (uint32_t)__builtin_amdgcn_ds_bpermute(src, (int)(leafFirst + (MULTI ? triOff : triOffset)));
                    const uint32_t oVer = VER ? (uint32_t)__builtin_amdgcn_ds_bpermute(src, (int)vTri) : 0u;
                    float pt = __builtin_inff(), pby = 0.0f, pbz = 0.0f;
                    if (have) {
                        const float4* tv = s.triVerts + 3 * (size_t)(oFirst + kk) + oVer;
                        const float4 a = tv[0], b = tv[1], c = tv[2];
                        float by, bz, t;
                        if (RayTriangleIntersect(oro, ord, mk3(a.x, a.y, a.z), mk3(b.x, b.y, b.z), mk3(c.x, c.y, c.z), &by, &bz, &t) && t < oT) { pt = t; pby = by; pbz = bz; }
                    }
                    for (uint32_t k = 0; k < maxCnt; k++) {
                        const uint32_t j = off + k - base;
                        const int from = (int)((j & 63u) << 2);
                        const float t = __int_as_float(__builtin_amdgcn_ds_bpermute(from, __float_as_int(pt)));
                        const float by = __int_as_float(__builtin_amdgcn_ds_bpermute(from, __float_as_int(pby))), bz = __int_as_float(__builtin_amdgcn_ds_bpermute(from, __float_as_int(pbz)));
                        if (k < cnt && j < 64u && t < hitT) {
                            hitTri = leafFirst + k + (MULTI ? triOff : triOffset); hbx = 1.0f - by - bz; hby = by; hitT = t; hitXform = MULTI ? xformId : inst.MeshTransformId;
                            if (OCCL && occl) top = 0u;
                        }
                    }
                    __builtin_amdgcn_wave_barrier();
                    if (base + 64u >= total) leafPending = false;
                }
            }
        }
        if (leafPending) {
            const uint32_t tOff = MULTI ? triOff : triOffset;
            for (uint32_t i = leafFirst + tOff, e = leafEnd + tOff; i < e; i++) {
                const float4* tv = s.triVerts + 3 * (size_t)i + (VER ? vTri : 0u);
                float4 a = tv[0], b = tv[1], c = tv[2];
                float by, bz, t;
                if (RayTriangleIntersect(ro, rd, mk3(a.x, a.y, a.z), mk3(b.x, b.y, b.z), mk3(c.x, c.y, c.z), &by, &bz, &t) && t < hitT) {
                    hitTri = i; hbx = 1.0f - by - bz; hby = by; hitT = t; hitXform = MULTI ? xformId : inst.MeshTransformId;
                    if (OCCL && occl) { top = 0u; break; }
                    if (ANY) {
                        top = 0u; sp = stkBase;
                        if (MULTI) { instIdx = (uint32_t)s.instanceCount; moreInst = false; }
                        break;
                    }
                }
            }
            leafPending = false;
        }
        PROF_MARK(2);
        if (active && top == 0u && (!MULTI || (TLAS ? !moreInst : instIdx >= (uint32_t)s.instanceCount))) {
            store_hit(hits, slot, hitT, hbx, hby, hitTri, hitXform);
            active = false;
        }
    }
    if (ovf) *s.overflow = 1u;
    if (COUNT) flush_counters(counters, nPairs, nTris);
    if (PROF && lane == 0) { for (int i = 0; i < 4; i++) atomicAdd((unsigned long long*)&counters[4 + i], pc[i]); for (int i = 0; i < 8; i++) atomicAdd((unsigned long long*)&counters[8 + i], pn[i]); }
#undef PROF_MARK
}
```

idkengine_amd/csrc/kernels_trace_fused.hpp:

```cpp
#pragma once

template <int REFILL_MIN = 32>
__global__ __launch_bounds__(WAVE, 1) void k_trace_fused(DScene s, Frame f, RayBufs rays, TraceBufs tr, HitBufs hits, const uint32_t* list, const uint32_t* countPtr, uint32_t* workCounter,
                                                        uint8_t* contFlag, uint32_t* seedsAndKeys, int lean)
{
    extern __shared__ uint32_t lds[];
    const uint32_t lane = threadIdx.x;
    typedef __attribute__((address_space(3))) uint32_t lds_u32;
    lds_u32* const stkBase = (lds_u32*)lds + lane;
    const int cap = f.stackCap;
    lds_u32* const stkFull = stkBase + cap * WAVE;
    const uint32_t N = *countPtr;
    {
        uint32_t want = gridDim.x;
        if (f.gridRaysX4 > 0u) want = max((uint32_t)(((unsigned long long)N * 4ull / f.gridRaysX4 + 63ull) / 64ull), min(want, 1024u));
        if (f.gridMid > 0u && N < f.gridMidRays) want = min(want, f.gridMid);
        if (blockIdx.x >= max(want, 1u)) return;
    }
    const GpuBlasInstance inst = s.instances[0];
    const int nodeOffset = s.descs[inst.BlasId].NodeOffset;
    const uint32_t triOffset = (uint32_t)s.descs[inst.BlasId].TriangleOffset;
    const float4* nodes = s.nodes + 2 * (size_t)nodeOffset;

    bool active = false, leafPending = false, workLeft = true;
// ... 75 lines not shown
                const uint32_t nearChild = both ? (leftCloser ? lStart : rStart) : (traverseLeft ? lStart : rStart);
                sp[WAVE] = leftCloser ? rStart : lStart;
                const bool full = sp == stkFull, nonEmpty = sp != stkBase;
                ovf = ovf || (both && full);
                top = none ? (nonEmpty ? popped : 0u) : nearChild;
                sp += (both && !full) ? (int)WAVE : ((none && nonEmpty) ? -(int)WAVE : 0);
            }
        }
        if (leafPending) {
            for (uint32_t i = leafFirst + triOffset, e = leafEnd + triOffset; i < e; i++) {
                const float4* tv = s.triVerts + 3 * (size_t)i;
                float4 a = tv[0], b = tv[1], c = tv[2];
                float by, bz, t;
                if (RayTriangleIntersect(ro, rd, mk3(a.x, a.y, a.z), mk3(b.x, b.y, b.z), mk3(c.x, c.y, c.z), &by, &bz, &t) && t < hitT) {
                    hitTri = i; hbx = 1.0f - by - bz; hby = by; hitT = t; hitXform = inst.MeshTransformId;
                }
            }
            leafPending = false;
        }
        if (active && top == 0u) {
            if (bounce) store_hit(hits, rid, hitT, hbx, hby, hitTri, hitXform);
            else shadePend = true;
            active = false;
        }
        {
            const uint32_t nS = (uint32_t)__builtin_popcountll(__builtin_amdgcn_ballot_w64(shadePend)), nA = (uint32_t)__builtin_popcountll(__builtin_amdgcn_ballot_w64(active));
            if (nS == 0u || !(nS >= (uint32_t)f.shadeMin || nS >= nA)) continue;
        }
        if (shadePend) {
            shadePend = false;
            const uint32_t smp = rid / f.Npad, pix = rid - smp * f.Npad;
            const uint32_t acc = sample_index(f, smp);
            HitRec hit; hit.T = hitT; hit.bx = hbx; hit.by = hby; hit.tri = hitTri; hit.xform = hitXform;
            RayState r; uint32_t rng, key = 0;
            if (lean) {
                f2 pd; gen_primary(f, smp, pix, acc, r.origin, pd, rng);
                r.prevIor = 1.0f; r.throughput = splat3(1.0f); r.pdx = pd.x; r.radiance = splat3(0.0f); r.pdy = pd.y;
            } else {
                float4 a = rays.o_ior[rid], b = rays.thr_px[rid], c = rays.rad_py[rid];
                r.origin = mk3(a.x, a.y, a.z); r.prevIor = a.w; r.throughput = mk3(b.x, b.y, b.z); r.pdx = b.w; r.radiance = mk3(c.x, c.y, c.z); r.pdy = c.w;
                rng = seedsAndKeys[rid];
            }
            AovState aov; aov.albedo = splat3(0.0f); aov.normal = splat3(0.0f); aov.newWeight = 1.0f;
            const int lx = (int)(pix % (uint32_t)f.W), ly = (int)(pix / (uint32_t)f.W);
            const uint32_t gidSeed = first_hit_gid_seed(f.W, f.H, lx, global_row(f, ly));
            const f3 rd0 = DecodeUnitVec(r.pdx, r.pdy);
            const bool cont = ShadeHit<true>(s, f, acc, hit, hit.T != PT_FLOAT_MAX, rd0, r, aov, rng, gidSeed, key);
            rays.o_ior[rid] = make_float4(r.origin.x, r.origin.y, r.origin.z, r.prevIor);
            rays.thr_px[rid] = make_float4(r.throughput.x, r.throughput.y, r.throughput.z, r.pdx);
            rays.rad_py[rid] = make_float4(r.radiance.x, r.radiance.y, r.radiance.z, r.pdy);
            if (f.outputAovs) { rays.aovA[rid] = make_float4(aov.albedo.x, aov.albedo.y, aov.albedo.z, aov.newWeight); rays.aovN[rid] = make_float4(aov.normal.x, aov.normal.y, aov.normal.z, 0.0f); }
            seedsAndKeys[rid] = (key & ((1u << IDKPT_SORT_KEY_BITS) - 1u)) | (smp << IDKPT_SORT_KEY_BITS);
            if (cont) {
                contFlag[rid] = 1;
                const f3 wd = DecodeUnitVec(r.pdx, r.pdy);
                const M34 inv = load_inv_model(s, inst.MeshTransformId);
                ro = xform34(inv, r.origin, 1.0f); rd = xform34(inv, wd, 0.0f);
                invDir = mk3(1.0f / rd.x, 1.0f / rd.y, 1.0f / rd.z);
                const float4* root = s.nodes + 2 * (size_t)nodeOffset + 2;
                float t1;
                const float rootT = RayBoxIntersect(ro, invDir, root[0], root[1], &t1) ? t1 : __builtin_inff();
                hitT = PT_FLOAT_MAX; hitTri = ~0u; hitXform = 0; hbx = 0.0f; hby = 0.0f;
                if (f.g.DoTraceLights) {
                    for (int i = 0; i < s.lightCount; i++) {
                        const GpuLight& l = s.lights[i];
                        float tMin, tMax;
                        if (RaySphereIntersect(r.origin, wd, mk3(l.Position[0], l.Position[1], l.Position[2]), l.Radius, &tMin, &tMax) && tMin < hitT) { hitT = tMin < 0.0f ? tMax : tMin; hitXform = (uint32_t)i; hitTri = ~0u; }
                    }
                }
                const bool enter = rootT < hitT;
                active = true; bounce = true; leafPending = false; sp = stkBase; top = enter ? 2u : 0u;
            }
        }
    }
    if (ovf) *s.overflow = 1u;
}
```

idkengine_amd/csrc/pt_kernels.hpp:

```cpp
#pragma once
#include "pt_device.hpp"

namespace ptd {

struct TexDesc { const void* data; int w, h; uint32_t state; uint32_t pad; };

struct DScene {
    const float4* nodes;
    const float4* pairNodes;
    const uint4* tris;
    const float4* triVerts;
    const GpuBlasDesc* descs;
    const GpuBlasInstance* instances; int instanceCount;
    const float4* tlas; int tlasCount;
    const float4* instRec;
    const uint4* vertices;
    const GpuMesh* meshes;
    const GpuMaterial* materials;
    const float4* xforms;
    const GpuLight* lights; int lightCount;
    const float4* sky; int skySize;
    const TexDesc* textures; int textureCount;
    const float* srgbLut;
    uint32_t* overflow;
    const uint32_t* ver;
};
#define SCENE_VER_WORDS 8
DEV DScene scene_of_sample(const DScene& s, uint32_t smp)
{
    DScene v = s;
    const uint32_t* t = s.ver + SCENE_VER_WORDS * (size_t)smp;
    v.nodes = s.nodes + t[0]; v.triVerts = s.triVerts + t[1]; v.vertices = s.vertices + t[2]; v.tlas = s.tlas + t[3]; v.xforms = s.xforms + t[4];
    return v;
}

struct Frame {
    float invProj[16]; float invView[16]; float viewPos[3];
    int W, H, rowMod, rowRem, rows;
    int rowBandLog2;
    GpuSettings g;
    uint32_t accumulated;
    int useTlas, stackCap, outputAovs;
    int tlasCap;
    int leafMin;
    uint32_t gridRaysX4, gridMid, gridMidRays;
    int grabUnitLog2, grabFixed;
    int batch; uint32_t Npad; uint32_t accum[256];
    uint32_t seqFirst, seqStride;
    const float* cams; uint32_t slotOf[256];
    int advMin;
    int poolMin;
    int splitPeek;
    int splitMode;
    int scatterLog2;
    int gbStride, gbBands;
    int queryMode;
    int shadeMin;
    int hitsByRid;
    int genPixelMajor;
    int instSieve;
    int instTlas;
    int packet;
    int tilePerSample;
};
#define MAX_BATCH 256

struct RayBufs {
    float4* o_ior;
    float4* thr_px;
    float4* rad_py;
    float4* aovA;
    float4* aovN;
};
struct TraceBufs {
    float4* rec;
    const uint32_t* order; const uint32_t* orderIdx;
};
struct HitBufs {
    float4* hit;
    float* cost;
};

struct HitRec { float T, bx, by; uint32_t tri, xform; };
DEV void store_hit(const HitBufs& h, size_t slot, float T, float bx, float by, uint32_t tri, uint32_t xform)
{
    h.hit[2 * slot] = make_float4(T, bx, by, __uint_as_float(tri));
    h.hit[2 * slot + 1] = make_float4(__uint_as_float(xform), 0.0f, 0.0f, 0.0f);
}
DEV HitRec load_hit(const HitBufs& h, size_t slot)
{
    const float4 a = h.hit[2 * slot]; const float x = h.hit[2 * slot + 1].x;
    HitRec r; r.T = a.x; r.bx = a.y; r.by = a.z; r.tri = __float_as_uint(a.w); r.xform = __float_as_uint(x);
    return r;
}

#define TLAS_STACK_SIZE 32

template <bool COUNT, bool COST>
DEV bool IntersectBlas(const DScene& s, f3 ro, f3 rd, const GpuBlasDesc& dref, bool useTlas, HitRec& hit, float& debugCost,
                       uint32_t* stk, int stride, int cap, uint32_t& nPairs, uint32_t& nTris)
{
    bool anyHit = false;
    float tMinLeft, tMinRight;
    f3 invDir = mk3(1.0f / rd.x, 1.0f / rd.y, 1.0f / rd.z);
    struct { int NodeOffset, TriangleOffset; } d = {dref.NodeOffset, dref.TriangleOffset};
    const float4* nodes = s.nodes + 2 * (size_t)d.NodeOffset;
    if (!useTlas) {
        float4 rmin = nodes[2], rmax = nodes[3];
        if (!(RayBoxIntersect(ro, invDir, rmin, rmax, &tMinLeft) && tMinLeft < hit.T)) return false;
    }
    int sp = 0;
    uint32_t top = 2;
    while (true) {
        if (COST) debugCost += 1.0f;
        if (COUNT) nPairs++;
        const float4* p = nodes + 2 * (size_t)top;
        float4 lmin = p[0], lmax = p[1], rmin = p[2], rmax = p[3];
        uint32_t lStart = __float_as_uint(lmin.w), lCount = __float_as_uint(lmax.w), rStart = __float_as_uint(rmin.w), rCount = __float_as_uint(rmax.w);
        bool hitLeft = RayBoxIntersect(ro, invDir, lmin, lmax, &tMinLeft) && tMinLeft <= hit.T;
        bool hitRight = RayBoxIntersect(ro, invDir, rmin, rmax, &tMinRight) && tMinRight <= hit.T;
        bool intersectLeft = hitLeft && lCount > 0, intersectRight = hitRight && rCount > 0;
        if (intersectLeft || intersectRight) {
            uint32_t first = intersectLeft ? lStart : rStart;
            uint32_t end = !intersectRight ? (lStart + lCount) : (rStart + rCount);
            first += (uint32_t)d.TriangleOffset; end += (uint32_t)d.TriangleOffset;
            if (COST) debugCost += (float)(end - first) * 1.1f;
            if (COUNT) nTris += end - first;
            for (uint32_t i = first; i < end; i++) {
                const float4* tv = s.triVerts + 3 * (size_t)i;
// ... 492 lines not shown
```

idkengine_amd/gputypes.py:

```python
import ctypes as C
import numpy as np

GpuBlasNode = np.dtype([("Min", "<f4", 3), ("TriStartOrChild", "<u4"), ("Max", "<f4", 3), ("TriCount", "<u4")])
GpuBlasTriangle = np.dtype([("X", "<u4"), ("Y", "<u4"), ("Z", "<u4"), ("MeshId", "<u4")])
GpuBlasDesc = np.dtype([
    ("NodeOffset", "<i4"), ("NodeCount", "<i4"), ("TriangleOffset", "<i4"), ("TriangleCount", "<i4"),
    ("LeafIndicesOffset", "<i4"), ("LeafIndicesCount", "<i4"), ("ParentIndicesOffset", "<i4"), ("ParentIndicesCount", "<i4"),
    ("RequiredStackSize", "<i4"), ("IsRefittable", "u1"), ("_pad", "u1", 3)])
GpuBlasInstance = np.dtype([("BlasId", "<u4"), ("MeshTransformId", "<u4")])
GpuTlasNode = np.dtype([("Min", "<f4", 3), ("IsLeafAndChildOrInstanceId", "<u4"), ("Max", "<f4", 3), ("_pad0", "<f4")])
GpuMeshTransform = np.dtype([("Model", "<f4", (3, 4)), ("InvModel", "<f4", (3, 4)), ("PrevModel", "<f4", (3, 4))])
GpuMesh = np.dtype([
    ("LocalBoundsMin", "<f4", 3), ("MaterialId", "<i4"), ("LocalBoundsMax", "<f4", 3), ("NormalMapStrength", "<f4"),
    ("AbsorbanceBias", "<f4", 3), ("MeshletsOffset", "<i4"), ("MeshletCount", "<i4"), ("EmissiveBias", "<f4"),
    ("SpecularBias", "<f4"), ("RoughnessBias", "<f4"), ("TransmissionBias", "<f4"), ("IORBias", "<f4"),
    ("InstanceCount", "<i4"), ("VertexCount", "<i4"), ("_pad0", "<f4", 3), ("TintOnTransmissive", "u1"), ("_pad1", "u1", 3)])
GpuMaterial = np.dtype([
    ("EmissiveFactor", "<f4", 3), ("BaseColorFactor", "<u4"), ("Absorbance", "<f4", 3), ("IOR", "<f4"),
    ("TransmissionFactor", "<f4"), ("RoughnessFactor", "<f4"), ("MetallicFactor", "<f4"), ("AlphaCutoff", "<f4"),
    ("BaseColorTexture", "<u8"), ("MetallicRoughnessTexture", "<u8"), ("NormalTexture", "<u8"), ("EmissiveTexture", "<u8"),
    ("TransmissionTexture", "<u8"), ("IsVolumetric", "u1"), ("_pad0", "u1", 3), ("IsDoubleSided", "u1"), ("_pad1", "u1", 3)])
GpuVertex = np.dtype([("TexCoord", "<f4", 2), ("Tangent", "<u4"), ("Normal", "<u4")])
GpuLight = np.dtype([("Position", "<f4", 3), ("Radius", "<f4"), ("Color", "<f4", 3), ("PointShadowIndex", "<i4"),
                     ("PrevPosition", "<f4", 3), ("_pad0", "<f4")])
# ... 120 lines not shown
class Atmosphere(C.Structure):
    _fields_ = [("ISteps", C.c_int32), ("JSteps", C.c_int32), ("LightIntensity", C.c_float), ("Azimuth", C.c_float), ("Elevation", C.c_float)]

    def __init__(self, ISteps=40, JSteps=8, LightIntensity=15.0, Azimuth=0.0, Elevation=0.0):
        super().__init__(int(ISteps), int(JSteps), float(LightIntensity), float(Azimuth), float(Elevation))


class TonemapSettings(C.Structure):
    _fields_ = [("Exposure", C.c_float), ("Saturation", C.c_float), ("Linear", C.c_float), ("Peak", C.c_float), ("Compression", C.c_float), ("DoTonemapAndSrgbTransform", C.c_int32)]

    def __init__(self, Exposure=0.45, Saturation=1.06, Linear=0.18, Peak=1.0, Compression=0.1, DoTonemapAndSrgbTransform=True):
        super().__init__(float(Exposure), float(Saturation), float(Linear), float(Peak), float(Compression), 1 if DoTonemapAndSrgbTransform else 0)


IDKPT_DISPLAY_RGBA8, IDKPT_DISPLAY_RGBA32F = 0, 1
IDKPT_BLOOM_ROUTE_TILED, IDKPT_BLOOM_ROUTE_DIRECT = 0, 1


class BloomSettings(C.Structure):
    _fields_ = [("Threshold", C.c_float), ("MaxColor", C.c_float), ("MinusLods", C.c_int32)]

    def __init__(self, Threshold=1.5, MaxColor=3.8, MinusLods=3):
        super().__init__(float(Threshold), float(MaxColor), int(MinusLods))


IDKPT_RESULT_NOISY, IDKPT_RESULT_DENOISED = 0, 1
IDKPT_DENOISE_ROUTE_TILED, IDKPT_DENOISE_ROUTE_DIRECT = 0, 1


class Denoise(C.Structure):
    _fields_ = [("Iterations", C.c_int32), ("ColorSigma", C.c_float), ("AlbedoSigma", C.c_float), ("NormalSigma", C.c_float), ("DemodulateAlbedo", C.c_int32)]

    def __init__(self, Iterations=5, ColorSigma=8.0, AlbedoSigma=0.2, NormalSigma=0.5, DemodulateAlbedo=True):
        super().__init__(int(Iterations), float(ColorSigma), float(AlbedoSigma), float(NormalSigma), int(DemodulateAlbedo))


class Noise(C.Structure):
    _fields_ = [("Epsilon", C.c_float), ("Threshold", C.c_float)]

    def __init__(self, Epsilon=1e-2, Threshold=0.05):
        super().__init__(float(Epsilon), float(Threshold))


class NoiseSummary(C.Structure):
    _fields_ = [("TilesAbove", C.c_uint32), ("MaxTileMean", C.c_float), ("Tiles", C.c_uint32), ("Samples", C.c_uint32)]


class Stats(C.Structure):
    _fields_ = [("RaysTraced", C.c_uint64), ("PrimaryRays", C.c_uint64), ("Frames", C.c_uint64),
                ("LastAliveCounts", C.c_uint32 * 16), ("LastTraceMs", C.c_float), ("LastFrameMs", C.c_float),
                ("NodePairVisits", C.c_uint64), ("TriangleTests", C.c_uint64),
                ("TraceMsTotal", C.c_double), ("TraceLaunches", C.c_uint64),
                ("WideFlaggedRays", C.c_uint64), ("WideNodeVisits", C.c_uint64), ("WideLeafRecords", C.c_uint64), ("WideTriangleTests", C.c_uint64), ("InstTlasFlaggedRays", C.c_uint64),
                ("PacketFlaggedRays", C.c_uint64), ("PacketPackets", C.c_uint64), ("PacketNodeSteps", C.c_uint64), ("PacketLiveLanes", C.c_uint64), ("PacketRaysEntered", C.c_uint64), ("PacketTriangleRounds", C.c_uint64), ("InstUnifiedLaunches", C.c_uint64), ("InstUnifiedEntries", C.c_uint32), ("InstUnifiedTopDepth", C.c_uint32), ("LastOcclusionLaunches", C.c_uint64)]


def _ptr(a):
    return None if a is None or len(a) == 0 else a.ctypes.data


class Scene:

    def __init__(self):
        self.blas_nodes = np.zeros(0, GpuBlasNode)
        self.blas_triangles = np.zeros(0, GpuBlasTriangle)
        self.blas_descs = np.zeros(0, GpuBlasDesc)
        self.blas_instances = np.zeros(0, GpuBlasInstance)
        self.tlas_nodes = np.zeros(0, GpuTlasNode)
        self.blas_parent_indices = np.zeros(0, np.int32)
        self.blas_leaf_indices = np.zeros(0, np.int32)
        self.vertex_positions = np.zeros((0, 3), np.float32)
        self.vertices = np.zeros(0, GpuVertex)
        self.meshes = np.zeros(0, GpuMesh)
        self.materials = np.zeros(0, GpuMaterial)
        self.mesh_transforms = np.zeros(0, GpuMeshTransform)
        self.lights = np.zeros(0, GpuLight)
        self.sky_faces = None
        self.textures = []
        self.blas_stack_size = 0

    def desc(self):
        keep = []

        def c(a, dt=None):
            a = np.ascontiguousarray(a, dtype=dt)
            keep.append(a)
            return a

        d = SceneDesc()
        a = c(self.blas_nodes); d.BlasNodes, d.BlasNodeCount = _ptr(a), len(a)
        a = c(self.blas_triangles); d.BlasTriangles, d.BlasTriangleCount = _ptr(a), len(a)
        a = c(self.blas_descs); d.BlasDescs, d.BlasDescCount = _ptr(a), len(a)
        a = c(self.blas_instances); d.BlasInstances, d.BlasInstanceCount = _ptr(a), len(a)
        a = c(self.tlas_nodes); d.TlasNodes, d.TlasNodeCount = _ptr(a), len(a)
        a = c(self.blas_parent_indices, np.int32); d.BlasParentIndices, d.BlasParentIndexCount = _ptr(a), len(a)
        a = c(self.blas_leaf_indices, np.int32); d.BlasLeafIndices, d.BlasLeafIndexCount = _ptr(a), len(a)
        a = c(self.vertex_positions, np.float32); d.VertexPositions, d.VertexCount = _ptr(a), len(a)
        a = c(self.vertices); d.Vertices = _ptr(a)
        assert len(a) == d.VertexCount
        a = c(self.meshes); d.Meshes, d.MeshCount = _ptr(a), len(a)
        a = c(self.materials); d.Materials, d.MaterialCount = _ptr(a), len(a)
        a = c(self.mesh_transforms); d.MeshTransforms, d.MeshTransformCount = _ptr(a), len(a)
        a = c(self.lights); d.Lights, d.LightCount = _ptr(a), len(a)
        if self.sky_faces is not None:
            a = c(self.sky_faces, np.float32)
            assert a.ndim == 4 and a.shape[0] == 6 and a.shape[1] == a.shape[2] and a.shape[3] == 4
            d.SkyFaces, d.SkyFaceSize = a.ctypes.data, a.shape[1]
# ... 53 lines not shown
```

idkengine_amd/pathtracer.py:

```python
import ctypes as C
import os
import numpy as np
from . import _lib
from . import gputypes as T
from ._lib import IdkPtError


_OPTION_NAMES = ("force_generic", "no_tile_cull", "no_lean_primary", "leaf_min", "grab_unit_log2", "grab_fixed", "lds_pad", "trace_waves", "grid_hint", "grid_rays_x4", "grid_mid_waves", "defer_last", "last_occlusion", "split", "split_donor", "split_peek", "group_threads", "query_scheduler", "split_scatter", "fused", "fused_shade_min", "leaf_pool", "pool_min", "adv_min",
                 "wide", "wide_cap", "wide_count", "packet", "packet_min_live", "packet_waves", "inst_tlas", "inst_tlas_overlap", "inst_braid", "inst_unify", "inst_unify_radius", "uni_refill", "inst_general", "pair_nodes", "inst_sieve", "inst_sieve_overlap", "gen_pixel_major", "gen_group_max", "bounce_pixel_major", "transport", "bvh_timing", "bvh_small", "bvh_stackopt_host", "force_no_peer", "trace_variant")


class PathTracer:
    def __init__(self, width, height, settings=None, device=0, row_modulo=1, row_remainder=0, devices=None, row_band=1):
        self._L = _lib.load()
        n = C.c_int32(0)
        self._L.idkptGetDeviceCount(C.byref(n))
        if n.value <= 0:
            raise IdkPtError("no HIP device visible: the path tracer has no CPU fallback")
        ctx = C.c_void_p()
        ids = list(devices) if devices else [device]
        self.device_count = len(ids); self.device_ids = ids
        if self.device_count > 1 and (row_modulo, row_remainder) != (1, 0):
            raise IdkPtError("a multi-device context deals its rows itself")
        dev = (C.c_int32 * len(ids))(*ids)
        rc = self._L.idkptCreate(len(ids), dev, C.byref(ctx))
        if rc != 0:
            raise IdkPtError(f"idkptCreate failed with status {rc}")
        self._ctx = ctx
        for name in _OPTION_NAMES:
            v = os.environ.get("IDKPT_" + name.upper())
            if v is not None and v != "":
                self.set_option(name, int(v))
        self._settings = settings if settings is not None else T.Settings.default()
        self._cached_ray_depth = self._settings.RayDepth
        self._scene = None
        self.width, self.height = width, height
        self.row_modulo, self.row_remainder, self.row_band = row_modulo, row_remainder, (int(row_band) if row_modulo > 1 else 1)
        self._row_limit = None
        if self.device_count == 1:
            if self.row_band > 1:
                self._check(self._L.idkptSetRowBands(ctx, self.row_band, row_modulo, row_remainder))
            else:
                self._check(self._L.idkptSetRowSharding(ctx, row_modulo, row_remainder))
        self._check(self._L.idkptSetSize(ctx, width, height))
        self._push_settings()

    def _check(self, rc):
        err = getattr(self, "_callback_error", None)
        if err is not None:
            self._callback_error = None
            raise err
        if rc != 0:
            msg = C.c_char_p()
            self._L.idkptGetLastError(self._ctx, C.byref(msg))
            raise IdkPtError(f"idkpt status {rc}: {(msg.value or b'').decode()}")

    def _push_settings(self):
        self._check(self._L.idkptSetSettings(self._ctx, C.addressof(self._settings)))

    def global_rows(self):
        b = self.row_band
# ... 493 lines not shown

    def GetNoiseEstimate(self):
        e = C.c_int32()
        self._check(self._L.idkptGetNoiseEstimate(self._ctx, C.byref(e)))
        return bool(e.value)

    def EstimateNoise(self, settings=None, slot=None):
        if settings is None:
            settings = T.Noise()
        if not isinstance(settings, T.Noise):
            raise TypeError("EstimateNoise: settings must be a gputypes.Noise")
        slot = -1 if slot is None else int(slot)
        self._check(self._L.idkptEstimateNoise(self._ctx, slot, C.addressof(settings)))
        return self.DownloadNoise(slot)

    def DownloadNoise(self, slot=None):
        tiles = np.zeros(((self.height + 7) // 8, (self.width + 7) // 8, 2), np.float32)
        s = T.NoiseSummary()
        self._check(self._L.idkptDownloadNoise(self._ctx, -1 if slot is None else int(slot), tiles.ctypes.data, tiles.nbytes, C.addressof(s)))
        return tiles, {"TilesAbove": s.TilesAbove, "MaxTileMean": s.MaxTileMean, "Tiles": s.Tiles, "Samples": s.Samples}

    def DownloadMoments(self, slot=None):
        out = np.zeros((self.height, self.width, 4), np.float32)
        self._check(self._L.idkptDownloadMoments(self._ctx, -1 if slot is None else int(slot), out.ctypes.data, out.nbytes))
        return out

    def noise_device_ptrs(self, slot=None):
        t = C.c_void_p(); s = C.c_void_p(); n = C.c_size_t()
        self._check(self._L.idkptGetNoiseDevicePtr(self._ctx, -1 if slot is None else int(slot), C.byref(t), C.byref(s), C.byref(n)))
        return t.value, s.value, n.value

    def moments_device_ptr(self, slot=None):
        p = C.c_void_p(); n = C.c_size_t()
        self._check(self._L.idkptGetMomentsDevicePtr(self._ctx, -1 if slot is None else int(slot), C.byref(p), C.byref(n)))
        return p.value, n.value

    def enable_counters(self, on=True):
        self._check(self._L.idkptEnableCounters(self._ctx, 1 if on else 0))

    def enable_timing(self, on=True):
        self._check(self._L.idkptEnableTiming(self._ctx, 1 if on else 0))

    def stats(self):
        s = T.Stats()
        self._check(self._L.idkptGetStatsSized(self._ctx, C.addressof(s), C.sizeof(s)))
        return {"rays_traced": s.RaysTraced, "primary_rays": s.PrimaryRays, "frames": s.Frames, "alive_counts": list(s.LastAliveCounts),
                "last_frame_ms": s.LastFrameMs, "node_pair_visits": s.NodePairVisits, "triangle_tests": s.TriangleTests,
                "trace_ms_total": s.TraceMsTotal, "trace_launches": s.TraceLaunches,
                "wide_flagged_rays": s.WideFlaggedRays, "wide_node_visits": s.WideNodeVisits, "wide_leaf_records": s.WideLeafRecords, "wide_triangle_tests": s.WideTriangleTests,
                "inst_tlas_flagged_rays": s.InstTlasFlaggedRays,
                "packet_flagged_rays": s.PacketFlaggedRays, "packet_packets": s.PacketPackets, "packet_node_steps": s.PacketNodeSteps, "packet_live_lanes": s.PacketLiveLanes,
                "packet_rays_entered": s.PacketRaysEntered, "packet_triangle_rounds": s.PacketTriangleRounds,
                "inst_unified_launches": s.InstUnifiedLaunches, "inst_unified_entries": s.InstUnifiedEntries, "inst_unified_top_depth": s.InstUnifiedTopDepth,
                "last_occlusion_launches": s.LastOcclusionLaunches}

    def reset_stats(self):
        self._check(self._L.idkptResetStats(self._ctx))

    def image_device_ptr(self, which=0):
        p = C.c_void_p(); n = C.c_size_t()
        self._check(self._L.idkptGetImageDevicePtr(self._ctx, which, C.byref(p), C.byref(n)))
        return p.value, n.value

    def SetFrameRing(self, frames):
        self._check(self._L.idkptSetFrameRing(self._ctx, int(frames)))

    def BeginFrame(self):
        slot = C.c_int32()
        self._check(self._L.idkptBeginFrame(self._ctx, C.byref(slot)))
        return slot.value

    def FrameResult(self, slot, which=0):
        out = np.zeros((self.rows, self.width, 4), np.float32)
        self._check(self._L.idkptDownloadFrame(self._ctx, int(slot), which, out.ctypes.data, out.nbytes))
        return out

    def frame_device_ptr(self, slot, which=0):
        p = C.c_void_p(); n = C.c_size_t()
        self._check(self._L.idkptGetFrameDevicePtr(self._ctx, int(slot), which, C.byref(p), C.byref(n)))
        return p.value, n.value

    def set_max_batch(self, n):
        self._check(self._L.idkptSetMaxBatch(self._ctx, n))

    def flush(self):
        self._check(self._L.idkptFlush(self._ctx))

    def set_option(self, name, value):
        self._check(self._L.idkptSetDeveloperOption(self._ctx, name.encode(), int(value)))

    def set_stream(self, hip_stream_handle):
        self._check(self._L.idkptSetStream(self._ctx, C.c_void_p(hip_stream_handle)))
```

include/idkpt.h:

```cpp
#ifndef IDKPT_H
#define IDKPT_H

#include "idkpt_types.h"

#ifdef __cplusplus
extern "C" {
#endif

#define IDKPT_API __attribute__((visibility("default")))

typedef struct idkpt_ctx idkpt_ctx;

enum idkpt_status {
    IDKPT_OK = 0,
    IDKPT_ERR_UNKNOWN = 1,
    IDKPT_ERR_INVALID_ARGUMENT = 2,
    IDKPT_ERR_INVALID_OPERATION = 3,
    IDKPT_ERR_OUT_OF_MEMORY = 4,
    IDKPT_ERR_NO_DEVICE = 5,
    IDKPT_ERR_HIP = 6,
};

enum idkpt_image { IDKPT_IMAGE_RESULT = 0, IDKPT_IMAGE_ALBEDO = 1, IDKPT_IMAGE_NORMAL = 2 };

// ... 77 lines not shown
    const GpuBlasNode*      BlasNodes;        int32_t BlasNodeCount;
    const GpuBlasTriangle*  BlasTriangles;    int32_t BlasTriangleCount;
    const GpuBlasDesc*      BlasDescs;        int32_t BlasDescCount;
    const GpuBlasInstance*  BlasInstances;    int32_t BlasInstanceCount;
    const GpuTlasNode*      TlasNodes;        int32_t TlasNodeCount;
    const int32_t*          BlasParentIndices;int32_t BlasParentIndexCount;
    const int32_t*          BlasLeafIndices;  int32_t BlasLeafIndexCount;
    const float*            VertexPositions;  int32_t VertexCount;
    const GpuVertex*        Vertices;
    const GpuMesh*          Meshes;           int32_t MeshCount;
    const GpuMaterial*      Materials;        int32_t MaterialCount;
    const GpuMeshTransform* MeshTransforms;   int32_t MeshTransformCount;
    const GpuLight*         Lights;           int32_t LightCount;
    const float*            SkyFaces;         int32_t SkyFaceSize;
    const idkpt_texture*    Textures;         int32_t TextureCount;
} idkpt_scene_desc;

typedef struct idkpt_settings {
    GpuSettings Gpu;
    int32_t RayDepth;
    int32_t SamplesPerPixel;
    int32_t DoRaySorting;
    int32_t OutputAOVs;
    int32_t UseTlas;
    int32_t BlasStackSize;
} idkpt_settings;

typedef struct idkpt_stats {
    uint64_t RaysTraced;
    uint64_t PrimaryRays;
    uint64_t Frames;
    uint32_t LastAliveCounts[16];
    float    LastTraceMs;
    float    LastFrameMs;
    uint64_t NodePairVisits;
    uint64_t TriangleTests;
    double   TraceMsTotal;
    uint64_t TraceLaunches;
    uint64_t WideFlaggedRays;
    uint64_t WideNodeVisits;
    uint64_t WideLeafRecords;
    uint64_t WideTriangleTests;
    uint64_t InstTlasFlaggedRays;
    uint64_t PacketFlaggedRays;
    uint64_t PacketPackets;
    uint64_t PacketNodeSteps;
    uint64_t PacketLiveLanes;
    uint64_t PacketRaysEntered;
    uint64_t PacketTriangleRounds;
    uint64_t InstUnifiedLaunches;
    uint32_t InstUnifiedEntries;
    uint32_t InstUnifiedTopDepth;
    uint64_t LastOcclusionLaunches;
} idkpt_stats;
#define IDKPT_ABI_VERSION 12

IDKPT_API int32_t idkptCreate(int32_t deviceCount, const int32_t* deviceIds, idkpt_ctx** outCtx);
IDKPT_API int32_t idkptGetContextDeviceCount(idkpt_ctx* ctx, int32_t* outCount);
enum idkpt_transport { IDKPT_TRANSPORT_NONE = 0, IDKPT_TRANSPORT_PEER_COPY = 1, IDKPT_TRANSPORT_RCCL = 2 };
IDKPT_API int32_t idkptGetTransportInfo(idkpt_ctx* ctx, int32_t* outKind, int32_t* outRanks, int32_t* outRcclVersion, const char** outDetail);
IDKPT_API int32_t idkptTransportSelfTest(int32_t device, int32_t* outRcclVersion, char* outDetail, size_t detailBytes);
enum idkpt_group_sharding { IDKPT_SHARD_AUTO = 0, IDKPT_SHARD_ROWS = 1, IDKPT_SHARD_STRIPS = 2, IDKPT_SHARD_BANDS = 3 };
IDKPT_API int32_t idkptSetGroupSharding(idkpt_ctx* ctx, int32_t mode);
IDKPT_API int32_t idkptDestroy(idkpt_ctx* ctx);
IDKPT_API int32_t idkptGetLastError(idkpt_ctx* ctx, const char** outMessage);
typedef void (*idkpt_error_fn)(void* user, int32_t status, const char* message);
IDKPT_API int32_t idkptSetErrorCallback(idkpt_ctx* ctx, idkpt_error_fn fn, void* user);
IDKPT_API int32_t idkptGetDeviceCount(int32_t* outCount);
IDKPT_API const char* idkptGetVersionString(void);
IDKPT_API int32_t idkptGetAbiVersion(void);

IDKPT_API int32_t idkptSetSize(idkpt_ctx* ctx, int32_t width, int32_t height);
IDKPT_API int32_t idkptSetRowSharding(idkpt_ctx* ctx, int32_t rowModulo, int32_t rowRemainder);
IDKPT_API int32_t idkptSetRowBands(idkpt_ctx* ctx, int32_t bandRows, int32_t rowModulo, int32_t rowRemainder);
IDKPT_API int32_t idkptSetRowRange(idkpt_ctx* ctx, int32_t firstRow, int32_t rowCount);
typedef void (*idkpt_bounce_exchange_fn)(void* user, int32_t bounce, int32_t sampleCount, const uint32_t* localCounts, uint32_t* outBases);
IDKPT_API int32_t idkptSetBounceExchange(idkpt_ctx* ctx, idkpt_bounce_exchange_fn fn, void* user);
typedef void (*idkpt_band_exchange_fn)(void* user, int32_t bounce, int32_t sampleCount, int32_t bandCount, const uint32_t* localCounts, uint32_t* outBases);
IDKPT_API int32_t idkptSetBandExchange(idkpt_ctx* ctx, idkpt_band_exchange_fn fn, void* user);
typedef void (*idkpt_band_exchange_device_fn)(void* user, int32_t bounce, int32_t sampleCount, int32_t bandCount, const uint32_t* dLocalCounts, uint32_t* dOutBases, void* hipStream);
IDKPT_API int32_t idkptSetBandExchangeDevice(idkpt_ctx* ctx, idkpt_band_exchange_device_fn fn, void* user);
IDKPT_API int32_t idkptSetSettings(idkpt_ctx* ctx, const idkpt_settings* settings);
IDKPT_API int32_t idkptGetSettings(idkpt_ctx* ctx, idkpt_settings* outSettings);
IDKPT_API int32_t idkptSetPerFrame(idkpt_ctx* ctx, const float invProjection[16], const float invView[16], const float viewPos[3]);
IDKPT_API int32_t idkptSetPerFrameData(idkpt_ctx* ctx, const GpuPerFrameData* perFrame);

IDKPT_API int32_t idkptUploadScene(idkpt_ctx* ctx, const idkpt_scene_desc* scene);
IDKPT_API int32_t idkptUpdateBuffer(idkpt_ctx* ctx, int32_t which, size_t offsetBytes, size_t bytes, const void* data);
IDKPT_API int32_t idkptUpdateTexture(idkpt_ctx* ctx, int32_t index, const idkpt_texture* texture);
IDKPT_API int32_t idkptDownloadTexture(idkpt_ctx* ctx, int32_t index, int32_t* outResidentFormat, int32_t* outWidth, int32_t* outHeight, void* dst, size_t dstBytes);
typedef struct idkpt_atmosphere { int32_t ISteps, JSteps; float LightIntensity, Azimuth, Elevation; } idkpt_atmosphere;
IDKPT_API int32_t idkptComputeSky(idkpt_ctx* ctx, int32_t faceSize, const idkpt_atmosphere* atmosphere);
IDKPT_API int32_t idkptUpdateSky(idkpt_ctx* ctx, int32_t faceSize, int32_t format, const void* faces);
IDKPT_API int32_t idkptUnprojectSky(idkpt_ctx* ctx, int32_t width, int32_t height, int32_t channels, const float* pixels, int32_t faceSize);
IDKPT_API int32_t idkptDownloadSky(idkpt_ctx* ctx, int32_t* outFaceSize, float* dst, size_t dstBytes);
IDKPT_API int32_t idkptSetLightCount(idkpt_ctx* ctx, int32_t count);
IDKPT_API int32_t idkptBuildTlas(idkpt_ctx* ctx, const GpuTlasNode* nodes, int32_t nodeCount);
IDKPT_API int32_t idkptBuildTlasOnDevice(idkpt_ctx* ctx, int32_t searchRadius);
IDKPT_API int32_t idkptBuildBlasCore(idkpt_ctx* ctx, const float* fragmentBoxes, int32_t fragmentCount, GpuBlasNode* outNodes, int32_t* outSortedIdsX, int32_t* outLevels);
typedef struct idkpt_blas_build_info {
    int32_t NodeCount, TriangleCount, RequiredStackSize, ParentIndexCount, LeafIndexCount, FragmentCount, Levels, _pad;
    double Sah;
    double BuildMs;
} idkpt_blas_build_info;
IDKPT_API int32_t idkptBuildBlas(idkpt_ctx* ctx, const float* positions, int32_t vertexCount, const GpuBlasTriangle* triangles, int32_t triangleCount, int32_t isRefittable,
                                 float preSplitFactor, idkpt_blas_build_info* outInfo);
// ... 104 lines not shown
```

Measured before the change: 7978.

## Fold last-bounce occlusion misses into final draw instead of deferred shading

Adds a 'fold_last' mode for the last bounce when occlusion tracing is used. Rays are marked during the previous bounce, and the occlusion trace writes a per-ray missed flag instead of a hit record. The final draw kernel then adds the sky contribution for flagged rays, and shade_last only processes an 'odd' subset counted by a new counter. This removes the full hit-record store, the shade-last pass and the hit reload in restore. In exchange it adds flag-byte traffic, a sky sample in the final draw, and more coupling between kernels.

```diff
diff --git a/idkengine_amd/csrc/host_context.hpp b/idkengine_amd/csrc/host_context.hpp
--- a/idkengine_amd/csrc/host_context.hpp
+++ b/idkengine_amd/csrc/host_context.hpp
@@ -113,6 +113,7 @@
     int gridHint = 2;
     int deferLast = 1;
     int lastOcclusion = 1;
+    int foldLast = 1;
     int graphProbe = 0;
     int gridMidWaves = 20;
     int gridRaysX4 = 6;
@@ -216,8 +217,9 @@
     bool sceneNested = false;
     bool sceneNoEmission = false;
     struct { bool valid = false, allHits = false; int j = 0, side = 0, B = 0; uint32_t total = 0, Npad = 0;
-             bool occl = false, pm = false; size_t ldsBytes = 0; uint32_t grid = 0; } defer;
+             bool occl = false, pm = false, fold = false; const uint32_t* list = nullptr; size_t ldsBytes = 0; uint32_t grid = 0; } defer;
     uint64_t occlLaunches = 0;
+    uint64_t foldBatches = 0;
     DevBuf radSave, deferCount;
     bool countersDirty = true;
     uint32_t* hOverflow = nullptr; uint32_t* dOverflow = nullptr;
diff --git a/idkengine_amd/csrc/host_frame.hpp b/idkengine_amd/csrc/host_frame.hpp
--- a/idkengine_amd/csrc/host_frame.hpp
+++ b/idkengine_amd/csrc/host_frame.hpp
@@ -26,6 +26,7 @@
     ctx->countersDirty = true;
     HIPC(hipMemsetAsync(ctx->aovA.p, 0, cap * 16, ctx->stream)); HIPC(hipMemsetAsync(ctx->aovN.p, 0, cap * 16, ctx->stream));
     HIPC(hipMemsetAsync(ctx->contFlag.p, 0, cap, ctx->stream));
+    HIPC(ctx->deferCount.ensure(64));
     ctx->accum.assign(ctx->ringSize, 0u); ctx->curSlot = 0; ctx->ringStarted = false;
     ctx->products.release_all();
     if (!owns_whole_frame(ctx)) ctx->noiseOn = 0;
diff --git a/idkengine_amd/csrc/host_options.hpp b/idkengine_amd/csrc/host_options.hpp
--- a/idkengine_amd/csrc/host_options.hpp
+++ b/idkengine_amd/csrc/host_options.hpp
@@ -20,6 +20,7 @@
     else if (n == "grid_mid_waves") o.gridMidWaves = std::max(0, value);
     else if (n == "defer_last") o.deferLast = value != 0;
     else if (n == "last_occlusion") o.lastOcclusion = value != 0;
+    else if (n == "fold_last") o.foldLast = value != 0;
     else if (n == "split") { REQUIRE(value >= 0 && value <= 3, "idkptSetDeveloperOption: split is 0..3"); o.split = value; }
     else if (n == "split_donor") o.splitDonor = value != 0;
     else if (n == "split_peek") o.splitPeek = std::max(1, value);
diff --git a/idkengine_amd/csrc/host_readback.hpp b/idkengine_amd/csrc/host_readback.hpp
--- a/idkengine_amd/csrc/host_readback.hpp
+++ b/idkengine_amd/csrc/host_readback.hpp
@@ -136,7 +136,7 @@
     s.RaysTraced = s.PrimaryRays + c[2];
     if (ctx->wtotals.p) { uint64_t w[16]; HIPC(hipMemcpyAsync(w, ctx->wtotals.p, TOTALS_BYTES, hipMemcpyDeviceToHost, ctx->stream)); HIPC(hipStreamSynchronize(ctx->stream)); s.WideFlaggedRays = w[0]; s.WideNodeVisits = w[1]; s.WideLeafRecords = w[2]; s.WideTriangleTests = w[3]; s.InstTlasFlaggedRays = w[4];
         s.PacketFlaggedRays = w[8]; s.PacketPackets = w[9]; s.PacketNodeSteps = w[10]; s.PacketLiveLanes = w[11]; s.PacketRaysEntered = w[12]; s.PacketTriangleRounds = w[13]; }
-    s.LastOcclusionLaunches = ctx->occlLaunches;
+    s.LastOcclusionLaunches = ctx->occlLaunches; s.LastFoldBatches = ctx->foldBatches;
     s.InstUnifiedLaunches = ctx->uniLaunches; s.InstUnifiedEntries = ctx->uniValid ? (uint32_t)ctx->uniEntries : 0u; s.InstUnifiedTopDepth = ctx->uniValid ? (uint32_t)ctx->uniDepth : 0u;
     *out = s;
     return IDKPT_OK;
@@ -148,7 +148,7 @@
     HIPC(hipSetDevice(ctx->device));
     FLUSH_KEEP();
     HIPC(hipStreamSynchronize(ctx->stream));
-    memset(&ctx->stats, 0, sizeof(ctx->stats)); ctx->uniLaunches = 0; ctx->occlLaunches = 0;
+    memset(&ctx->stats, 0, sizeof(ctx->stats)); ctx->uniLaunches = 0; ctx->occlLaunches = 0; ctx->foldBatches = 0;
     if (ctx->hPkStats) memset(ctx->hPkStats, 0, 64);
     for (int i = 0; i < 6; i++) ctx->pkSeen[i] = 0;
     ctx->evUsed = 0; ctx->traceMsAcc = 0.0; ctx->traceLaunchesAcc = 0;
diff --git a/idkengine_amd/csrc/host_schedule.hpp b/idkengine_amd/csrc/host_schedule.hpp
--- a/idkengine_amd/csrc/host_schedule.hpp
+++ b/idkengine_amd/csrc/host_schedule.hpp
@@ -41,6 +41,8 @@
     return readsOnlyHitOrMiss && ctx->opt.lastOcclusion != 0 && !plan.fused && (plan.walk == Walk::Plain || plan.walk == Walk::Fast) && !(split && plan.splitOk)
            && !plan.multiVer && !plan.counting && !ctx->counters && (ctx->opt.traceVariant == 0 || ctx->opt.traceVariant == 100);
 }
+static bool want_fold(const dev_ctx* ctx, bool tookOccl) { return tookOccl && ctx->opt.foldLast != 0; }
+static bool may_fold(const dev_ctx* ctx, bool deferLast, bool deferAllHits) { return deferLast && !deferAllHits && ctx->opt.lastOcclusion != 0 && ctx->opt.foldLast != 0; }
 static uint32_t small_launch_grid(uint32_t fullGrid, uint32_t prev, int hintMul, int raysX4, uint32_t midGrid)
 {
     if (prev == 0u || hintMul <= 0) return fullGrid;
@@ -69,8 +71,8 @@
 {
     b.ctx = ctx; b.st = ctx->stream; b.B = B; b.depth = ctx->st.RayDepth; b.N = (uint32_t)((size_t)ctx->W * ctx->rows); b.Npad = Npad; b.total = (uint32_t)B * Npad;
     b.gridTotal = (b.total + 255) / 256; b.scanBlocks = ((b.total + 63) / 64 + SCAN_WAVES_PER_BLOCK - 1) / SCAN_WAVES_PER_BLOCK;
-    b.rays = {ctx->rayO.as<float4>(), ctx->rayT.as<float4>(), ctx->rayR.as<float4>(), ctx->aovA.as<float4>(), ctx->aovN.as<float4>()}; b.hits = {ctx->hit.as<float4>(), ctx->hitCost.as<float>()};
-    b.tr = {ctx->trRec.as<float4>(), nullptr, nullptr}; b.trNone = {nullptr, nullptr, nullptr};
+    b.rays = {ctx->rayO.as<float4>(), ctx->rayT.as<float4>(), ctx->rayR.as<float4>(), ctx->aovA.as<float4>(), ctx->aovN.as<float4>(), ctx->contFlag.as<uint8_t>()}; b.hits = {ctx->hit.as<float4>(), ctx->hitCost.as<float>()};
+    b.tr = {ctx->trRec.as<float4>(), nullptr, nullptr, ctx->deferCount.as<uint32_t>() + 1}; b.trNone = {nullptr, nullptr, nullptr, nullptr};
     b.counts = ctx->counts.as<uint32_t>(); b.bases = ctx->bases.as<uint32_t>(); b.work = ctx->work.as<uint32_t>(); b.counters = ctx->counters64.as<uint64_t>(); b.hostCounts = ctx->dCountsMirror; b.hostBases = ctx->dBasesMirror;
     b.contMask = ctx->contMask.as<unsigned long long>(); b.waveLocal = ctx->waveCounts.as<uint32_t>(); b.blockSums = ctx->blockSums.as<uint32_t>(); b.keysTmp = ctx->keysTmp.as<uint32_t>();
     b.activeList = ctx->sortVals.as<uint32_t>(); b.activeCount = b.counts + (MAX_DEPTH_SLOTS - 1);
@@ -93,18 +95,18 @@
     if (!ctx->defer.valid) return IDKPT_OK;
     ctx->defer.valid = false;
     Batch b; batch_views(ctx, b, ctx->defer.B, ctx->defer.Npad);
-    b.side = ctx->defer.side; b.f = ctx->lastFrame; b.s = make_dscene_last(ctx); b.multiVer = ctx->lastMulti;
+    b.side = ctx->defer.side; b.f = ctx->lastFrame; b.f.markLast = 0; b.f.foldLast = 0; b.s = make_dscene_last(ctx); b.multiVer = ctx->lastMulti;
     const uint32_t* q = ctx->queue[b.side].as<uint32_t>(); const uint32_t* cnt = ctx->deferCount.as<uint32_t>();
     if (ctx->defer.occl) {
         const int j = ctx->defer.j;
         if (ctx->countersDirty) HIPC(hipMemsetAsync(b.work, 0, WORK_WORDS * 4, b.st));
         TracePlan p{}; p.walk = Walk::Plain; p.ldsBytes = ctx->defer.ldsBytes; p.grid = ctx->defer.grid;
         Frame ft = b.f; if (ctx->defer.pm) ft.hitsByRid = 0;
-        if (ctx->defer.pm) launch_trace2<true>(ctx, p, p.grid, b.st, b.s, ft, b.rays, b.tr, b.hits, ctx->pmList.as<uint32_t>(), cnt, b.work + j, b.counters, false, j);
+        if (ctx->defer.pm) launch_trace2<true>(ctx, p, p.grid, b.st, b.s, ft, b.rays, b.tr, b.hits, ctx->defer.list, cnt, b.work + j, b.counters, false, j);
         else launch_trace2<false>(ctx, p, p.grid, b.st, b.s, ft, b.rays, b.tr, b.hits, q, cnt, b.work + j, b.counters, false, j);
         ctx->defer.occl = false;
     }
-    with_flag(ctx->defer.allHits, [&](auto ALL) { launch(k_restore_last<ALL>, dim3(b.gridTotal), dim3(256), 0, b.st, b.rays, b.hits, q, cnt, ctx->radSave.as<float4>(), b.f.hitsByRid); });
+    with_flag(ctx->defer.allHits, [&](auto ALL) { launch(k_restore_last<ALL>, dim3(b.gridTotal), dim3(256), 0, b.st, b.rays, b.hits, q, cnt, ctx->radSave.as<float4>(), b.f.hitsByRid, ctx->defer.fold ? 1 : 0); });
     { int rc = bounce_tail(b, ctx->defer.j, q, cnt, nullptr, nullptr, false, b.tr); if (rc) return rc; }
     HIPC(hipGetLastError());
     ctx->lastQueueSide = 1 - b.side; ctx->countersDirty = true;
@@ -173,7 +175,7 @@
     graph_probe_begin(b);
     if (ctx->timing) HIPC(hipEventRecord(ctx->evFrame[0], st));
     ctx->defer.valid = false;
-    if (ctx->countersDirty) { HIPC(hipMemsetAsync(b.work, 0, WORK_WORDS * 4, st)); HIPC(hipMemsetAsync(b.counts, 0, MAX_DEPTH_SLOTS * 4, st)); }
+    if (ctx->countersDirty) { HIPC(hipMemsetAsync(b.work, 0, WORK_WORDS * 4, st)); HIPC(hipMemsetAsync(b.counts, 0, MAX_DEPTH_SLOTS * 4, st)); HIPC(hipMemsetAsync(b.tr.oddCount, 0, 4, st)); }
     ctx->countersDirty = true;
     f.tlasCap = std::min(TLAS_STACK_SIZE, std::max(1, ctx->tlasNeed));
     f.grabUnitLog2 = std::min(24, std::max(6, ctx->opt.grabUnitLog2)); f.grabFixed = std::max(0, ctx->opt.grabFixed);
@@ -312,10 +314,12 @@
     uint32_t gridj = b.traceGrid;
     const bool split = want_split(ctx, prev, known, B), occl = b.fast && want_occlusion(ctx, b.plan, readsOnlyHitOrMiss, split);
     if (occl) ctx->occlLaunches++;
+    if (want_fold(ctx, occl)) { b.f.foldLast = 1; b.f.hitsByRid = 1; }
     if (ctx->opt.gridHint > 0 && ctx->lastBatch == B && ctx->hBases) gridj = small_launch_grid(b.traceGrid, ctx->hBases[(size_t)j * BS + B], ctx->opt.gridHint, ctx->opt.gridRaysX4, b.midGrid);
-    if (b.fast && b.pmBounce && j == 1) {
+    if (b.fast && ((b.pmBounce && j == 1) || b.f.foldLast)) {
+        const bool pm = b.pmBounce && j == 1;
         Frame ft = b.f; ft.hitsByRid = 0;
-        launch_trace2<true>(ctx, b.plan, gridj, st, b.s, ft, b.rays, b.tr, b.hits, b.pmList, b.pmCount, b.work + j, b.counters, split, j, occl);
+        launch_trace2<true>(ctx, b.plan, gridj, st, b.s, ft, b.rays, b.tr, b.hits, pm ? b.pmList : q, pm ? b.pmCount : cnt, b.work + j, b.counters, split, j, occl);
     } else if (b.fast) launch_trace2<false>(ctx, b.plan, gridj, st, b.s, b.f, b.rays, b.tr, b.hits, q, cnt, b.work + j, b.counters, split, j, occl);
     else with_flag(ctx->counters, [&](auto COUNT) { launch(k_trace_queue<COUNT>, dim3(b.traceGrid), dim3(WAVE), b.plan.ldsBytes, st, b.s, b.f, b.rays, b.hits, q, cnt, b.work + j, b.counters); });
     TRACE_T1();
@@ -325,12 +329,15 @@
 static int defer_last_bounce(Batch& b, int j, const uint32_t* q, const uint32_t* cnt, bool allHits, bool occl)
 {
     dev_ctx* ctx = b.ctx;
-    HIPC(ctx->radSave.ensure((size_t)ctx->maxBatch * ctx->Npad * 16)); HIPC(ctx->deferCount.ensure(64));
+    const bool fold = b.f.foldLast != 0, pm = b.pmBounce && j == 1;
+    HIPC(ctx->radSave.ensure((size_t)ctx->maxBatch * ctx->Npad * 16));
     auto shade_last = [&](auto ALL, auto VER) { launch(k_shade_last<ALL, VER>, dim3(b.gridTotal), dim3(256), 0, b.st, b.s, b.f, b.rays, b.hits, q, cnt, b.bases + j * BS, ctx->radSave.as<float4>(), ctx->deferCount.as<uint32_t>()); };
-    if (allHits) with_flag(b.multiVer, [&](auto VER) { shade_last(std::true_type{}, VER); });
+    if (fold) launch(k_shade_last_odd, dim3(std::min<uint32_t>(b.gridTotal, 256u)), dim3(256), 0, b.st, b.s, b.f, b.rays, b.hits, q, cnt, b.bases + j * BS, ctx->radSave.as<float4>(), ctx->deferCount.as<uint32_t>(), (const uint32_t*)b.tr.oddCount);
+    else if (allHits) with_flag(b.multiVer, [&](auto VER) { shade_last(std::true_type{}, VER); });
     else shade_last(std::false_type{}, std::false_type{});
+    if (fold) ctx->foldBatches++;
     ctx->defer.allHits = allHits; ctx->defer.valid = true; ctx->defer.j = j; ctx->defer.side = b.side; ctx->defer.B = b.B; ctx->defer.total = b.total; ctx->defer.Npad = b.Npad;
-    ctx->defer.occl = occl; ctx->defer.pm = b.pmBounce && j == 1; ctx->defer.ldsBytes = b.plan.ldsBytes; ctx->defer.grid = b.traceGrid;
+    ctx->defer.occl = occl; ctx->defer.fold = fold; ctx->defer.pm = pm || fold; ctx->defer.list = pm ? (const uint32_t*)b.pmList : q; ctx->defer.ldsBytes = b.plan.ldsBytes; ctx->defer.grid = b.traceGrid;
     return IDKPT_OK;
 }
 
@@ -339,10 +346,10 @@
     dev_ctx* ctx = b.ctx; hipStream_t st = b.st;
     ctx->lastQueueSide = b.side; ctx->lastQueueCountSlot = b.depth; ctx->lastFast = b.fast; ctx->lastNeedsRegen = b.fast; ctx->lastTileClass = b.tileClass != nullptr; ctx->lastBatch = b.B; ctx->lastFrame = b.f;
     if (ctx->noiseOn) {
-        launch(k_final_draw_noise, dim3((b.N + 255) / 256), dim3(256), 0, st, b.s, b.f, b.rays, image_ptr(ctx, 0, 0), image_ptr(ctx, 1, 0), image_ptr(ctx, 2, 0), b.N, b.tileClass, b.work, (uint32_t)WORK_WORDS, b.counts, (uint32_t)MAX_DEPTH_SLOTS,
+        launch(k_final_draw_noise, dim3((b.N + 255) / 256), dim3(256), 0, st, b.s, b.f, b.rays, image_ptr(ctx, 0, 0), image_ptr(ctx, 1, 0), image_ptr(ctx, 2, 0), b.N, b.tileClass, b.work, (uint32_t)WORK_WORDS, b.counts, (uint32_t)MAX_DEPTH_SLOTS, b.tr.oddCount,
                noise_moments_ptr(ctx, 0), noise_mom_stride(ctx));
     } else
-    launch(k_final_draw, dim3((b.N + 255) / 256), dim3(256), 0, st, b.s, b.f, b.rays, image_ptr(ctx, 0, 0), image_ptr(ctx, 1, 0), image_ptr(ctx, 2, 0), b.N, b.tileClass, b.work, (uint32_t)WORK_WORDS, b.counts, (uint32_t)MAX_DEPTH_SLOTS);
+    launch(k_final_draw, dim3((b.N + 255) / 256), dim3(256), 0, st, b.s, b.f, b.rays, image_ptr(ctx, 0, 0), image_ptr(ctx, 1, 0), image_ptr(ctx, 2, 0), b.N, b.tileClass, b.work, (uint32_t)WORK_WORDS, b.counts, (uint32_t)MAX_DEPTH_SLOTS, b.tr.oddCount);
     HIPC(hipGetLastError()); ctx->countersDirty = false;
     graph_probe_end(b);
     if (ctx->timing) HIPC(hipEventRecord(ctx->evFrame[1], st));
@@ -359,9 +366,11 @@
     Batch b; batch_views(ctx, b, (int)ctx->pending.size(), ctx->Npad); int rc;
     if ((rc = stage_versions_cameras(b))) return rc;
     if ((rc = frame_setup(b))) return rc;
-    if ((rc = b.fast ? first_hit_fast(b) : first_hit_generic(b))) return rc;
     const bool deferLast = b.fast && b.depth >= 2 && ctx->opt.deferLast != 0 && !b.f.outputAovs && !b.debug;
     const bool deferAllHits = !(ctx->sceneNoEmission && !(b.f.g.DoTraceLights && b.s.lightCount > 0));
+    const bool mayFold = may_fold(ctx, deferLast, deferAllHits);
+    b.f.markLast = (mayFold && b.depth == 2) ? 1 : 0;
+    if ((rc = b.fast ? first_hit_fast(b) : first_hit_generic(b))) return rc;
     for (int j = 1; j < b.depth; j++) {
         uint32_t* q = ctx->queue[b.side].as<uint32_t>(); uint32_t* k = ctx->keys[b.side].as<uint32_t>();
         const uint32_t* cnt = b.counts + j; const uint32_t* gbase;
@@ -372,6 +381,7 @@
         bool tookOccl = false;
         if (!b.plan.fused) tookOccl = trace_bounce(b, j, q, cnt, deferThis && !deferAllHits);
         if (deferThis) { if ((rc = defer_last_bounce(b, j, q, cnt, deferAllHits, tookOccl))) return rc; break; }
+        b.f.markLast = (mayFold && j + 1 == b.depth - 1) ? 1 : 0;
         if ((rc = bounce_tail(b, j, q, cnt, gbase, (unsigned long long*)(j + 1 < b.depth ? b.counters + 2 : nullptr), ctx->evBounce != nullptr, b.fast ? b.tr : b.trNone))) return rc;
         b.side = 1 - b.side;
     }
diff --git a/idkengine_amd/csrc/idkpt_api.hpp b/idkengine_amd/csrc/idkpt_api.hpp
--- a/idkengine_amd/csrc/idkpt_api.hpp
+++ b/idkengine_amd/csrc/idkpt_api.hpp
@@ -967,7 +967,7 @@
         sum.RaysTraced += s.RaysTraced; sum.PrimaryRays += s.PrimaryRays; sum.NodePairVisits += s.NodePairVisits; sum.TriangleTests += s.TriangleTests;
         sum.WideFlaggedRays += s.WideFlaggedRays; sum.WideNodeVisits += s.WideNodeVisits; sum.WideLeafRecords += s.WideLeafRecords; sum.WideTriangleTests += s.WideTriangleTests; sum.InstTlasFlaggedRays += s.InstTlasFlaggedRays;
         sum.PacketFlaggedRays += s.PacketFlaggedRays; sum.PacketPackets += s.PacketPackets; sum.PacketNodeSteps += s.PacketNodeSteps; sum.PacketLiveLanes += s.PacketLiveLanes; sum.PacketRaysEntered += s.PacketRaysEntered; sum.PacketTriangleRounds += s.PacketTriangleRounds;
-        sum.LastOcclusionLaunches += s.LastOcclusionLaunches;
+        sum.LastOcclusionLaunches += s.LastOcclusionLaunches; sum.LastFoldBatches += s.LastFoldBatches;
         sum.InstUnifiedLaunches += s.InstUnifiedLaunches; if (d == 0) { sum.InstUnifiedEntries = s.InstUnifiedEntries; sum.InstUnifiedTopDepth = s.InstUnifiedTopDepth; }
         for (int j = 0; j < 16; j++) sum.LastAliveCounts[j] += s.LastAliveCounts[j];
         sum.LastFrameMs = std::max(sum.LastFrameMs, s.LastFrameMs); sum.LastTraceMs = std::max(sum.LastTraceMs, s.LastTraceMs);
diff --git a/idkengine_amd/csrc/kernels_frame.hpp b/idkengine_amd/csrc/kernels_frame.hpp
--- a/idkengine_amd/csrc/kernels_frame.hpp
+++ b/idkengine_amd/csrc/kernels_frame.hpp
@@ -38,7 +38,16 @@
         float w = 1.0f / ((float)f.accum[k] + 1.0f);
         const uint32_t cls = !tileClass ? 0u : (f.tilePerSample ? tileClass[(size_t)k * nTilesAll + tile] : sharedCls);
         f3 nr = splat3(0.0f);
-        if (cls == 0u) { float4 c = rays.rad_py[rid]; nr = mk3(c.x, c.y, c.z); }
+        if (cls == 0u) {
+            const float4 c = rays.rad_py[rid]; nr = mk3(c.x, c.y, c.z);
+            if (f.foldLast && (rays.flag[rid] & CF_LAST_MISSED)) {
+                const float4 b = rays.thr_px[rid];
+                if (__builtin_isfinite(b.x) && __builtin_isfinite(b.y) && __builtin_isfinite(b.z)) {
+                    const f3 albedo = SampleSky(s, DecodeUnitVec(b.w, c.w));
+                    nr = mk3(c.x, c.y, c.z) + albedo * mk3(b.x, b.y, b.z);
+                }
+            }
+        }
         else if (cls <= 6u) { const float4 p = s.sky[cls - 1u]; nr = splat3(0.0f) + mk3(p.x, p.y, p.z) * splat3(1.0f); }
         else if (cls == 8u) {
             f3 origin; f2 pd; uint32_t seed;
@@ -56,17 +65,17 @@
     if constexpr (NOISE) imgMoments[(size_t)slot * momStride + i] = make_float4(m1, m2, 0.0f, 1.0f);
 }
 __global__ __launch_bounds__(256) void k_final_draw(DScene s, Frame f, RayBufs rays, float4* imgResult, float4* imgAlbedo, float4* imgNormal, uint32_t N, const uint8_t* tileClass,
-                                                    uint32_t* zeroWork, uint32_t nWork, uint32_t* zeroCounts, uint32_t nCounts)
+                                                    uint32_t* zeroWork, uint32_t nWork, uint32_t* zeroCounts, uint32_t nCounts, uint32_t* zeroOdd )
 {
-    if (blockIdx.x == 0) { for (uint32_t k = threadIdx.x; k < nWork; k += blockDim.x) zeroWork[k] = 0u; for (uint32_t k = threadIdx.x; k < nCounts; k += blockDim.x) zeroCounts[k] = 0u; }
+    if (blockIdx.x == 0) { for (uint32_t k = threadIdx.x; k < nWork; k += blockDim.x) zeroWork[k] = 0u; for (uint32_t k = threadIdx.x; k < nCounts; k += blockDim.x) zeroCounts[k] = 0u; if (threadIdx.x == 0) *zeroOdd = 0u; }
     uint32_t i = blockIdx.x * blockDim.x + threadIdx.x;
     if (i >= N) return;
     final_draw_body<false>(s, f, rays, imgResult, imgAlbedo, imgNormal, N, tileClass, i, nullptr, 0);
 }
 __global__ __launch_bounds__(256) void k_final_draw_noise(DScene s, Frame f, RayBufs rays, float4* imgResult, float4* imgAlbedo, float4* imgNormal, uint32_t N, const uint8_t* tileClass,
-                                                          uint32_t* zeroWork, uint32_t nWork, uint32_t* zeroCounts, uint32_t nCounts, float4* imgMoments, size_t momStride)
+                                                          uint32_t* zeroWork, uint32_t nWork, uint32_t* zeroCounts, uint32_t nCounts, uint32_t* zeroOdd, float4* imgMoments, size_t momStride)
 {
-    if (blockIdx.x == 0) { for (uint32_t k = threadIdx.x; k < nWork; k += blockDim.x) zeroWork[k] = 0u; for (uint32_t k = threadIdx.x; k < nCounts; k += blockDim.x) zeroCounts[k] = 0u; }
+    if (blockIdx.x == 0) { for (uint32_t k = threadIdx.x; k < nWork; k += blockDim.x) zeroWork[k] = 0u; for (uint32_t k = threadIdx.x; k < nCounts; k += blockDim.x) zeroCounts[k] = 0u; if (threadIdx.x == 0) *zeroOdd = 0u; }
     uint32_t i = blockIdx.x * blockDim.x + threadIdx.x;
     if (i >= N) return;
     final_draw_body<true>(s, f, rays, imgResult, imgAlbedo, imgNormal, N, tileClass, i, imgMoments, momStride);
@@ -80,14 +89,15 @@
     uint8_t flag = contFlag[rid];
     if (tileClass) {
         const uint32_t px = pix % (uint32_t)f.W, py = pix / (uint32_t)f.W, tilesX = ((uint32_t)f.W + 7) / 8, nTilesAll = tilesX * (((uint32_t)f.rows + 7) / 8);
-        if (tileClass[(f.tilePerSample ? (size_t)smp * nTilesAll : 0) + (py >> 3) * tilesX + (px >> 3)] != 0u) flag = 4;
+        if (tileClass[(f.tilePerSample ? (size_t)smp * nTilesAll : 0) + (py >> 3) * tilesX + (px >> 3)] != 0u) flag = CF_CULLED_TILE;
     }
-    if (flag != 2 && flag != 4) return;
+    flag &= (uint8_t)(CF_CULLED_PIXEL | CF_CULLED_TILE);
+    if (flag == 0) return;
     f3 origin; f2 pd; uint32_t seed;
     gen_primary(f, smp, pix, sample_index(f, smp), origin, pd, seed);
     rays.o_ior[rid] = make_float4(origin.x, origin.y, origin.z, 1.0f);
     rays.thr_px[rid] = make_float4(1.0f, 1.0f, 1.0f, pd.x);
-    if (flag == 4) {
+    if (flag == CF_CULLED_TILE) {
         const f3 albedo = SampleSky(s, DecodeUnitVec(pd.x, pd.y));
         const f3 radiance = splat3(0.0f) + albedo * splat3(1.0f);
         rays.rad_py[rid] = make_float4(radiance.x, radiance.y, radiance.z, pd.y);
diff --git a/idkengine_amd/csrc/kernels_shade.hpp b/idkengine_amd/csrc/kernels_shade.hpp
--- a/idkengine_amd/csrc/kernels_shade.hpp
+++ b/idkengine_amd/csrc/kernels_shade.hpp
@@ -16,6 +16,7 @@
     float t1;
     const float rootT = RayBoxIntersect(lo, iv, root[0], root[1], &t1) ? t1 : __builtin_inff();
     const float wantClosest = (__builtin_isfinite(r.throughput.x) && __builtin_isfinite(r.throughput.y) && __builtin_isfinite(r.throughput.z)) ? 0.0f : 1.0f;
+    if (wantClosest != 0.0f && tr.oddCount) atomicAdd(tr.oddCount, 1u);
     tr.rec[4 * (size_t)rid] = make_float4(lo.x, lo.y, lo.z, rootT); tr.rec[4 * (size_t)rid + 1] = make_float4(ld.x, ld.y, ld.z, wantClosest);
     tr.rec[4 * (size_t)rid + 2] = make_float4(iv.x, iv.y, iv.z, 0.0f);
 }
@@ -57,7 +58,7 @@
         rays.rad_py[rid] = make_float4(r.radiance.x, r.radiance.y, r.radiance.z, r.pdy);
         if (f.outputAovs) { rays.aovA[rid] = make_float4(aov.albedo.x, aov.albedo.y, aov.albedo.z, aov.newWeight); rays.aovN[rid] = make_float4(aov.normal.x, aov.normal.y, aov.normal.z, 0.0f); }
         seedsAndKeys[rid] = (key & ((1u << IDKPT_SORT_KEY_BITS) - 1u)) | (smp << IDKPT_SORT_KEY_BITS);
-        if (cont) { contFlag[rid] = 1; write_trace_ready(s, f, tr, rid, r); }
+        if (cont) { contFlag[rid] = (uint8_t)(CF_CONTINUES | (f.markLast ? CF_LAST_ENTERED : 0)); write_trace_ready(s, f, tr, rid, r); }
     }
     if (pmList) {
         const unsigned long long m = __ballot(cont);
@@ -115,6 +116,7 @@
             rays.rad_py[idx] = make_float4(r.radiance.x, r.radiance.y, r.radiance.z, r.pdy);
             if (f.outputAovs) { rays.aovA[idx] = make_float4(aov.albedo.x, aov.albedo.y, aov.albedo.z, aov.newWeight); rays.aovN[idx] = make_float4(aov.normal.x, aov.normal.y, aov.normal.z, 0.0f); }
             if (cont && tr.rec) write_trace_ready(s, f, tr, idx, r);
+            if (!FIRST && cont && f.markLast) rays.flag[idx] = CF_LAST_ENTERED;
         }
         keysTmp[slot] = (key & ((1u << IDKPT_SORT_KEY_BITS) - 1u)) | (smp << IDKPT_SORT_KEY_BITS);
     }
@@ -123,19 +125,15 @@
     (void)waveCounts;
 }
 
-template <bool ALL_HITS , bool VER = false>
-__global__ __launch_bounds__(256) void k_shade_last(DScene s0, Frame f, RayBufs rays, HitBufs hits, const uint32_t* queue, const uint32_t* countPtr, const uint32_t* qbase,
-                                                    float4* radSave, uint32_t* deferCount)
+template <bool ALL_HITS , bool VER, bool ODD_ONLY>
+__device__ __forceinline__ void shade_last_slot(const DScene& s0, const Frame& f, const RayBufs& rays, const HitBufs& hits, const uint32_t* queue, const uint32_t* qbase, float4* radSave, uint32_t slot)
 {
-    const uint32_t N = *countPtr;
-    const uint32_t slot = blockIdx.x * blockDim.x + threadIdx.x;
-    if (slot == 0u) *deferCount = N;
-    if (slot >= N) return;
     const uint32_t idx = queue[slot];
+    const float4 b = rays.thr_px[idx];
+    const bool odd = ALL_HITS || !(__builtin_isfinite(b.x) && __builtin_isfinite(b.y) && __builtin_isfinite(b.z));
+    if (ODD_ONLY && !odd) return;
     const HitRec hit = load_hit(hits, f.hitsByRid ? idx : slot);
-    const float4 b = rays.thr_px[idx];
     const bool miss = hit.T == PT_FLOAT_MAX;
-    const bool odd = ALL_HITS || !(__builtin_isfinite(b.x) && __builtin_isfinite(b.y) && __builtin_isfinite(b.z));
     if (!miss && !odd) return;
     const float4 c = rays.rad_py[idx];
     radSave[slot] = c;
@@ -156,13 +154,33 @@
         rays.rad_py[idx] = make_float4(r.radiance.x, r.radiance.y, r.radiance.z, c.w);
     }
 }
+template <bool ALL_HITS, bool VER = false>
+__global__ __launch_bounds__(256) void k_shade_last(DScene s0, Frame f, RayBufs rays, HitBufs hits, const uint32_t* queue, const uint32_t* countPtr, const uint32_t* qbase,
+                                                    float4* radSave, uint32_t* deferCount)
+{
+    const uint32_t N = *countPtr;
+    const uint32_t slot = blockIdx.x * blockDim.x + threadIdx.x;
+    if (slot == 0u) *deferCount = N;
+    if (slot >= N) return;
+    shade_last_slot<ALL_HITS, VER, false>(s0, f, rays, hits, queue, qbase, radSave, slot);
+}
+__global__ __launch_bounds__(256) void k_shade_last_odd(DScene s0, Frame f, RayBufs rays, HitBufs hits, const uint32_t* queue, const uint32_t* countPtr, const uint32_t* qbase,
+                                                        float4* radSave, uint32_t* deferCount, const uint32_t* oddCount)
+{
+    const uint32_t N = *countPtr;
+    const uint32_t first = blockIdx.x * blockDim.x + threadIdx.x;
+    if (first == 0u) *deferCount = N;
+    if (*oddCount == 0u) return;
+    for (unsigned long long slot = first; slot < N; slot += (unsigned long long)gridDim.x * blockDim.x) shade_last_slot<false, false, true>(s0, f, rays, hits, queue, qbase, radSave, (uint32_t)slot);
+}
 template <bool ALL_HITS>
-__global__ __launch_bounds__(256) void k_restore_last(RayBufs rays, HitBufs hits, const uint32_t* queue, const uint32_t* countPtr, const float4* radSave, int hitsByRid)
+__global__ __launch_bounds__(256) void k_restore_last(RayBufs rays, HitBufs hits, const uint32_t* queue, const uint32_t* countPtr, const float4* radSave, int hitsByRid, int folded)
 {
     const uint32_t slot = blockIdx.x * blockDim.x + threadIdx.x;
     if (slot >= *countPtr) return;
     const uint32_t idx = queue[slot];
-    const HitRec hit = load_hit(hits, hitsByRid ? idx : slot);
     const float4 b = rays.thr_px[idx];
-    if (ALL_HITS || hit.T == PT_FLOAT_MAX || !(__builtin_isfinite(b.x) && __builtin_isfinite(b.y) && __builtin_isfinite(b.z))) rays.rad_py[idx] = radSave[slot];
+    bool restore = ALL_HITS || !(__builtin_isfinite(b.x) && __builtin_isfinite(b.y) && __builtin_isfinite(b.z));
+    if (!restore && !folded) restore = load_hit(hits, hitsByRid ? idx : slot).T == PT_FLOAT_MAX;
+    if (restore) rays.rad_py[idx] = radSave[slot];
 }
diff --git a/idkengine_amd/csrc/kernels_trace.hpp b/idkengine_amd/csrc/kernels_trace.hpp
--- a/idkengine_amd/csrc/kernels_trace.hpp
+++ b/idkengine_amd/csrc/kernels_trace.hpp
@@ -162,7 +162,7 @@
     const uint32_t nTilesAll = tilesX * (((uint32_t)f.rows + 7) / 8);
     const uint32_t cls = (tileClass && wave < nTilesAll) ? tileClass[(f.tilePerSample ? (size_t)min(smp, (uint32_t)f.batch - 1u) * nTilesAll : 0) + wave] : 0u;
     if (valid && cls != 0u) {
-        contFlag[rid] = 4;
+        contFlag[rid] = CF_CULLED_TILE;
     } else if (valid) {
         f3 origin; f2 pd; uint32_t seed;
         gen_primary(f, smp, pix, sample_index(f, smp), origin, pd, seed);
@@ -210,7 +210,7 @@
             if (f.outputAovs) { f3 fn = CubemapFaceNormal(rd); rays.aovA[rid] = make_float4(albedo.x, albedo.y, albedo.z, 0.0f); rays.aovN[rid] = make_float4(fn.x, fn.y, fn.z, 0.0f); }
         }
         if (keep && !lean) { rays.o_ior[rid] = make_float4(origin.x, origin.y, origin.z, 1.0f); rays.thr_px[rid] = make_float4(1.0f, 1.0f, 1.0f, pd.x); }
-        contFlag[rid] = keep ? 0 : 2;
+        contFlag[rid] = keep ? 0 : CF_CULLED_PIXEL;
         if (!(keep && lean)) rays.rad_py[rid] = make_float4(radiance.x, radiance.y, radiance.z, pd.y);
     }
     const unsigned long long m = __ballot(keep);
@@ -530,7 +530,8 @@
         }
         PROF_MARK(2);
         if (active && top == 0u && (!MULTI || (TLAS ? !moreInst : instIdx >= (uint32_t)s.instanceCount))) {
-            store_hit(hits, slot, hitT, hbx, hby, hitTri, hitXform);
+            if (OCCL && occl && f.foldLast) { if (hitT == PT_FLOAT_MAX) rays.flag[slot] = (uint8_t)(CF_LAST_ENTERED | CF_LAST_MISSED); }
+            else store_hit(hits, slot, hitT, hbx, hby, hitTri, hitXform);
             active = false;
         }
     }
diff --git a/idkengine_amd/csrc/kernels_trace_fused.hpp b/idkengine_amd/csrc/kernels_trace_fused.hpp
--- a/idkengine_amd/csrc/kernels_trace_fused.hpp
+++ b/idkengine_amd/csrc/kernels_trace_fused.hpp
@@ -151,7 +151,7 @@
             if (f.outputAovs) { rays.aovA[rid] = make_float4(aov.albedo.x, aov.albedo.y, aov.albedo.z, aov.newWeight); rays.aovN[rid] = make_float4(aov.normal.x, aov.normal.y, aov.normal.z, 0.0f); }
             seedsAndKeys[rid] = (key & ((1u << IDKPT_SORT_KEY_BITS) - 1u)) | (smp << IDKPT_SORT_KEY_BITS);
             if (cont) {
-                contFlag[rid] = 1;
+                contFlag[rid] = CF_CONTINUES;
                 const f3 wd = DecodeUnitVec(r.pdx, r.pdy);
                 const M34 inv = load_inv_model(s, inst.MeshTransformId);
                 ro = xform34(inv, r.origin, 1.0f); rd = xform34(inv, wd, 0.0f);
diff --git a/idkengine_amd/csrc/pt_kernels.hpp b/idkengine_amd/csrc/pt_kernels.hpp
--- a/idkengine_amd/csrc/pt_kernels.hpp
+++ b/idkengine_amd/csrc/pt_kernels.hpp
@@ -62,6 +62,15 @@
     int instTlas;
     int packet;
     int tilePerSample;
+    int markLast;
+    int foldLast;
+};
+enum : uint8_t {
+    CF_CONTINUES = 1,
+    CF_CULLED_PIXEL = 2,
+    CF_CULLED_TILE = 4,
+    CF_LAST_ENTERED = 8,
+    CF_LAST_MISSED = 16,
 };
 #define MAX_BATCH 256
 
@@ -71,10 +80,12 @@
     float4* rad_py;
     float4* aovA;
     float4* aovN;
+    uint8_t* flag;
 };
 struct TraceBufs {
     float4* rec;
     const uint32_t* order; const uint32_t* orderIdx;
+    uint32_t* oddCount;
 };
 struct HitBufs {
     float4* hit;
diff --git a/idkengine_amd/gputypes.py b/idkengine_amd/gputypes.py
--- a/idkengine_amd/gputypes.py
+++ b/idkengine_amd/gputypes.py
@@ -196,7 +196,7 @@
                 ("NodePairVisits", C.c_uint64), ("TriangleTests", C.c_uint64),
                 ("TraceMsTotal", C.c_double), ("TraceLaunches", C.c_uint64),
                 ("WideFlaggedRays", C.c_uint64), ("WideNodeVisits", C.c_uint64), ("WideLeafRecords", C.c_uint64), ("WideTriangleTests", C.c_uint64), ("InstTlasFlaggedRays", C.c_uint64),
-                ("PacketFlaggedRays", C.c_uint64), ("PacketPackets", C.c_uint64), ("PacketNodeSteps", C.c_uint64), ("PacketLiveLanes", C.c_uint64), ("PacketRaysEntered", C.c_uint64), ("PacketTriangleRounds", C.c_uint64), ("InstUnifiedLaunches", C.c_uint64), ("InstUnifiedEntries", C.c_uint32), ("InstUnifiedTopDepth", C.c_uint32), ("LastOcclusionLaunches", C.c_uint64)]
+                ("PacketFlaggedRays", C.c_uint64), ("PacketPackets", C.c_uint64), ("PacketNodeSteps", C.c_uint64), ("PacketLiveLanes", C.c_uint64), ("PacketRaysEntered", C.c_uint64), ("PacketTriangleRounds", C.c_uint64), ("InstUnifiedLaunches", C.c_uint64), ("InstUnifiedEntries", C.c_uint32), ("InstUnifiedTopDepth", C.c_uint32), ("LastOcclusionLaunches", C.c_uint64), ("LastFoldBatches", C.c_uint64)]
 
 
 def _ptr(a):
diff --git a/idkengine_amd/pathtracer.py b/idkengine_amd/pathtracer.py
--- a/idkengine_amd/pathtracer.py
+++ b/idkengine_amd/pathtracer.py
@@ -6,7 +6,7 @@
 from ._lib import IdkPtError
 
 
-_OPTION_NAMES = ("force_generic", "no_tile_cull", "no_lean_primary", "leaf_min", "grab_unit_log2", "grab_fixed", "lds_pad", "trace_waves", "grid_hint", "grid_rays_x4", "grid_mid_waves", "defer_last", "last_occlusion", "split", "split_donor", "split_peek", "group_threads", "query_scheduler", "split_scatter", "fused", "fused_shade_min", "leaf_pool", "pool_min", "adv_min",
+_OPTION_NAMES = ("force_generic", "no_tile_cull", "no_lean_primary", "leaf_min", "grab_unit_log2", "grab_fixed", "lds_pad", "trace_waves", "grid_hint", "grid_rays_x4", "grid_mid_waves", "defer_last", "last_occlusion", "fold_last", "split", "split_donor", "split_peek", "group_threads", "query_scheduler", "split_scatter", "fused", "fused_shade_min", "leaf_pool", "pool_min", "adv_min",
                  "wide", "wide_cap", "wide_count", "packet", "packet_min_live", "packet_waves", "inst_tlas", "inst_tlas_overlap", "inst_braid", "inst_unify", "inst_unify_radius", "uni_refill", "inst_general", "pair_nodes", "inst_sieve", "inst_sieve_overlap", "gen_pixel_major", "gen_group_max", "bounce_pixel_major", "transport", "bvh_timing", "bvh_small", "bvh_stackopt_host", "force_no_peer", "trace_variant")
 
 
@@ -606,7 +606,7 @@
                 "packet_flagged_rays": s.PacketFlaggedRays, "packet_packets": s.PacketPackets, "packet_node_steps": s.PacketNodeSteps, "packet_live_lanes": s.PacketLiveLanes,
                 "packet_rays_entered": s.PacketRaysEntered, "packet_triangle_rounds": s.PacketTriangleRounds,
                 "inst_unified_launches": s.InstUnifiedLaunches, "inst_unified_entries": s.InstUnifiedEntries, "inst_unified_top_depth": s.InstUnifiedTopDepth,
-                "last_occlusion_launches": s.LastOcclusionLaunches}
+                "last_occlusion_launches": s.LastOcclusionLaunches, "last_fold_batches": s.LastFoldBatches}
 
     def reset_stats(self):
         self._check(self._L.idkptResetStats(self._ctx))
diff --git a/include/idkpt.h b/include/idkpt.h
--- a/include/idkpt.h
+++ b/include/idkpt.h
@@ -153,6 +153,7 @@
     uint32_t InstUnifiedEntries;
     uint32_t InstUnifiedTopDepth;
     uint64_t LastOcclusionLaunches;
+    uint64_t LastFoldBatches;
 } idkpt_stats;
 #define IDKPT_ABI_VERSION 12
 
```

After: 8392 (median of 6 runs). 5.2% higher.
